# mees/hulc2

Measured on AMD Instinct MI355X. Metric: play-sequences/sec/node (seq_len=32, 200x200 RGB), higher is better.
Workload: dtype bf16; 1 GPU; BASELINE configs[1]: synthetic CALVIN-shaped batch, Hulc2.training_step fwd+bwd+allreduce+Adam, static CNN 200x200 + gripper CNN 84x84, lang = random (B,384) embeddings, dropout 0.1, gripper_control on; sequences_per_gpu_step=64, seq_len=32, parallelism=dp1, launch=hipGraph replay (fwd+bwd graph, all-reduce, optimizer graph), frames=fp32 NCHW, already transformed (the reference's dataloader output), gradient_allreduce=none (one rank, no process group), exact_forward_sites=encfc,goal,head,txl

## Files before the change

hulc2_amd/csrc/abi.hip:

```cpp
#include "hulc_abi_internal.h"
#include <stdarg.h>
#include <stdio.h>
#include <string.h>

static thread_local char g_err[512] = "";

int hulc_fail(int code, const char* msg) {
    snprintf(g_err, sizeof(g_err), "%s", msg);
    return code;
}

int hulc_check_launch(const char* where) {
    hipError_t e = hipGetLastError();
    if (e == hipSuccess) return 0;
    snprintf(g_err, sizeof(g_err), "%s: launch failed: %s", where, hipGetErrorString(e));
    return -100;
}

extern "C" const char* hulc_last_error(void) { return g_err; }

static thread_local char g_conv_path[256] = "";

void hulc_conv_path_clear(void) { g_conv_path[0] = 0; }
void hulc_conv_path_set(const char* fmt, ...) {
    va_list ap;
    va_start(ap, fmt);
    vsnprintf(g_conv_path, sizeof(g_conv_path), fmt, ap);
    va_end(ap);
}
void hulc_conv_path_append(const char* suffix) {
    const size_t n = strlen(g_conv_path);
    snprintf(g_conv_path + n, sizeof(g_conv_path) - n, "%s", suffix);
}

extern "C" const char* hulc_conv_last_path(void) { return g_conv_path; }
extern "C" int hulc_abi_version(void) { return 7; }

extern "C" int hulc_stream_create(void** out) {
    if (!out) return hulc_fail(-1, "hulc_stream_create: null pointer");
    hipStream_t s = nullptr;
    if (hipStreamCreateWithFlags(&s, hipStreamNonBlocking) != hipSuccess) { *out = nullptr; return hulc_fail(-100, "hulc_stream_create: hipStreamCreateWithFlags failed"); }
    *out = (void*)s;
    return 0;
}
```

hulc2_amd/csrc/hulc_abi_internal.h:

```cpp
#pragma once
#include <hip/hip_runtime.h>
#include "../../include/hulc2_amd.h"

int hulc_fail(int code, const char* msg);
int hulc_check_launch(const char* where);

void hulc_conv_path_clear(void);
void hulc_conv_path_set(const char* fmt, ...) __attribute__((format(printf, 1, 2)));
void hulc_conv_path_append(const char* suffix);

int hulc_wgrad_taps_takes(const hulc_wgrad_item* d);
long hulc_wgrad_taps_workspace(const hulc_wgrad_item* const* items, int n);
int hulc_wgrad_taps_launch(const hulc_wgrad_item* const* items, int n, void* slabs, hipStream_t s);

int hulc_gemm_tn128_try(const hulc_gemm_desc* d, hipStream_t s);
int hulc_gemm_nt128_try(const hulc_gemm_desc* d, hipStream_t s);
```

hulc2_amd/csrc/hulc_common.h:

```cpp
#pragma once
#include <hip/hip_runtime.h>
#include <stdint.h>

#define HULC_F32 0
#define HULC_BF16 1
#define HULC_F16 2

typedef __bf16 bf16_t;
typedef bf16_t bf16x8_t __attribute__((ext_vector_type(8)));
typedef float f32x16_t __attribute__((ext_vector_type(16)));
typedef float f32x4_t __attribute__((ext_vector_type(4)));
typedef float f32x2_t __attribute__((ext_vector_type(2)));

#define HULC_DEVICE __device__ __forceinline__

HULC_DEVICE float bf16_bits_to_f32(uint16_t b) { return __uint_as_float(((uint32_t)b) << 16); }

typedef bf16_t bf16x2_t __attribute__((ext_vector_type(2)));

HULC_DEVICE uint32_t pack_bf16x2(float lo, float hi) {
    f32x2_t f = {lo, hi};
    union { bf16x2_t b; uint32_t u; } x;
    x.b = __builtin_convertvector(f, bf16x2_t);
    return x.u;
// ... 25 lines not shown
}
HULC_DEVICE void store_elem(void* p, int dtype, long idx, float v) {
    if (dtype == HULC_F32) ((float*)p)[idx] = v;
    else ((uint16_t*)p)[idx] = f32_to_bf16_bits(v);
}

struct Chunk8 {
    float v[8];
};

HULC_DEVICE void chunk_zero(Chunk8& c) {
#pragma unroll
    for (int j = 0; j < 8; ++j) c.v[j] = 0.f;
}

HULC_DEVICE void chunk_keep_if(Chunk8& c, bool keep) {
#pragma unroll
    for (int j = 0; j < 8; ++j) c.v[j] = keep ? c.v[j] : 0.f;
}

HULC_DEVICE void chunk_load_contig(Chunk8& c, const void* base, int dtype, long off) {
    if (dtype == HULC_F32) {
        const float4* p = (const float4*)((const float*)base + off);
        float4 a = p[0], b = p[1];
        c.v[0] = a.x; c.v[1] = a.y; c.v[2] = a.z; c.v[3] = a.w;
        c.v[4] = b.x; c.v[5] = b.y; c.v[6] = b.z; c.v[7] = b.w;
    } else if (dtype == HULC_F16) {
        union { uint4 u; _Float16 h[8]; } r; r.u = *(const uint4*)((const uint16_t*)base + off);
#pragma unroll
        for (int j = 0; j < 8; ++j) c.v[j] = (float)r.h[j];
    } else {
        uint4 r = *(const uint4*)((const uint16_t*)base + off);
        c.v[0] = __uint_as_float(r.x << 16); c.v[1] = __uint_as_float(r.x & 0xffff0000u);
        c.v[2] = __uint_as_float(r.y << 16); c.v[3] = __uint_as_float(r.y & 0xffff0000u);
        c.v[4] = __uint_as_float(r.z << 16); c.v[5] = __uint_as_float(r.z & 0xffff0000u);
        c.v[6] = __uint_as_float(r.w << 16); c.v[7] = __uint_as_float(r.w & 0xffff0000u);
    }
}

HULC_DEVICE void chunk_load_strided(Chunk8& c, const void* base, int dtype, long off, long ld, int nvalid) {
#pragma unroll
    for (int j = 0; j < 8; ++j) c.v[j] = (j < nvalid) ? load_elem(base, dtype, off + (long)j * ld) : 0.f;
}

template <typename CT>
HULC_DEVICE void chunk_store_lds(char* dst, const Chunk8& c);

template <>
HULC_DEVICE void chunk_store_lds<bf16_t>(char* dst, const Chunk8& c) {
    uint4 r;
    r.x = pack_bf16x2(c.v[0], c.v[1]);
    r.y = pack_bf16x2(c.v[2], c.v[3]);
    r.z = pack_bf16x2(c.v[4], c.v[5]);
    r.w = pack_bf16x2(c.v[6], c.v[7]);
    *(uint4*)dst = r;
}
template <>
HULC_DEVICE void chunk_store_lds<float>(char* dst, const Chunk8& c) {
    ((float4*)dst)[0] = make_float4(c.v[0], c.v[1], c.v[2], c.v[3]);
    ((float4*)dst)[1] = make_float4(c.v[4], c.v[5], c.v[6], c.v[7]);
}

#define HULC_ROWB 80

template <typename CT> struct MmaTraits;
template <> struct MmaTraits<bf16_t> {
    static constexpr int KT = 32;
    static constexpr int NCH = 4;
    static constexpr int CHB = 16;
};
template <> struct MmaTraits<float> {
    static constexpr int KT = 16;
    static constexpr int NCH = 2;
    static constexpr int CHB = 32;
};

template <typename CT, int TM, int TN>
HULC_DEVICE void mma_tile(const char* a_rows, const char* b_rows, f32x16_t (&acc)[TM][TN], int lane);

template <int TM, int TN>
HULC_DEVICE void mma_tile_bf16(const char* a_rows, const char* b_rows, f32x16_t (&acc)[TM][TN], int lane) {
    const int r = lane & 31, h = lane >> 5;
#pragma unroll
    for (int ks = 0; ks < 2; ++ks) {
        bf16x8_t a[TM], b[TN];
#pragma unroll
        for (int i = 0; i < TM; ++i) a[i] = *(const bf16x8_t*)(a_rows + (i * 32 + r) * HULC_ROWB + (ks * 2 + h) * 16);
#pragma unroll
        for (int j = 0; j < TN; ++j) b[j] = *(const bf16x8_t*)(b_rows + (j * 32 + r) * HULC_ROWB + (ks * 2 + h) * 16);
#pragma unroll
        for (int i = 0; i < TM; ++i)
#pragma unroll
            for (int j = 0; j < TN; ++j)
                acc[i][j] = __builtin_amdgcn_mfma_f32_32x32x16_bf16(a[i], b[j], acc[i][j], 0, 0, 0);
    }
}

template <int TM, int TN>
HULC_DEVICE void mma_tile_f32(const char* a_rows, const char* b_rows, f32x16_t (&acc)[TM][TN], int lane) {
    const int r = lane & 31, h = lane >> 5;
    float a[TM][8], b[TN][8];
#pragma unroll
    for (int i = 0; i < TM; ++i) {
        const float4* p = (const float4*)(a_rows + (i * 32 + r) * HULC_ROWB + h * 32);
        float4 x = p[0], y = p[1];
        a[i][0] = x.x; a[i][1] = x.y; a[i][2] = x.z; a[i][3] = x.w;
        a[i][4] = y.x; a[i][5] = y.y; a[i][6] = y.z; a[i][7] = y.w;
    }
#pragma unroll
    for (int j = 0; j < TN; ++j) {
        const float4* p = (const float4*)(b_rows + (j * 32 + r) * HULC_ROWB + h * 32);
        float4 x = p[0], y = p[1];
        b[j][0] = x.x; b[j][1] = x.y; b[j][2] = x.z; b[j][3] = x.w;
        b[j][4] = y.x; b[j][5] = y.y; b[j][6] = y.z; b[j][7] = y.w;
    }
#pragma unroll
    for (int e = 0; e < 8; ++e)
#pragma unroll
        for (int i = 0; i < TM; ++i)
#pragma unroll
            for (int j = 0; j < TN; ++j)
                acc[i][j] = __builtin_amdgcn_mfma_f32_32x32x2f32(a[i][e], b[j][e], acc[i][j], 0, 0, 0);
}

template <typename CT, int TM, int TN> struct MmaTile;
template <int TM, int TN> struct MmaTile<bf16_t, TM, TN> {
    static HULC_DEVICE void run(const char* a, const char* b, f32x16_t (&acc)[TM][TN], int lane) {
        mma_tile_bf16<TM, TN>(a, b, acc, lane);
    }
};
template <int TM, int TN> struct MmaTile<float, TM, TN> {
    static HULC_DEVICE void run(const char* a, const char* b, f32x16_t (&acc)[TM][TN], int lane) {
        mma_tile_f32<TM, TN>(a, b, acc, lane);
    }
};

HULC_DEVICE int fast_div(int x, float inv) { return (int)(((float)x + 0.5f) * inv); }

HULC_DEVICE float fast_rcp(int d) { return __builtin_amdgcn_rcpf((float)d); }

HULC_DEVICE int acc_row(int reg, int lane) { return (reg & 3) + 8 * (reg >> 2) + 4 * (lane >> 5); }

HULC_DEVICE float wave_sum(float v) {
#pragma unroll
    for (int o = 32; o > 0; o >>= 1) v += __shfl_xor(v, o, 64);
    return v;
}
HULC_DEVICE float wave_max(float v) {
#pragma unroll
    for (int o = 32; o > 0; o >>= 1) v = fmaxf(v, __shfl_xor(v, o, 64));
    return v;
}

HULC_DEVICE uint64_t hulc_rand64(uint64_t seed, uint64_t idx) {
    uint64_t z = idx * 0x9E3779B97F4A7C15ull + seed;
    z = (z ^ (z >> 30)) * 0xBF58476D1CE4E5B9ull;
    z = (z ^ (z >> 27)) * 0x94D049BB133111EBull;
    return z ^ (z >> 31);
}
HULC_DEVICE uint32_t hulc_rand32(uint64_t seed, uint64_t idx) { return (uint32_t)(hulc_rand64(seed, idx) >> 32); }
HULC_DEVICE float dropout_scale(uint64_t seed, uint64_t idx, float p) {
    const uint32_t thr = (uint32_t)(p * 65536.0f);
    const uint32_t u = (uint32_t)(hulc_rand64(seed, idx >> 2) >> (16 * (uint32_t)(idx & 3))) & 0xffffu;
    return u >= thr ? 1.0f / (1.0f - p) : 0.0f;
}
HULC_DEVICE void dropout_scale4(uint64_t seed, uint64_t idx0, float p, float (&s)[4]) {
    const uint32_t thr = (uint32_t)(p * 65536.0f);
    const float keep = 1.0f / (1.0f - p);
    const uint64_t z = hulc_rand64(seed, idx0 >> 2);
    const uint32_t lo = (uint32_t)z, hi = (uint32_t)(z >> 32);
    s[0] = (lo & 0xffffu) >= thr ? keep : 0.f; s[1] = (lo >> 16) >= thr ? keep : 0.f;
    s[2] = (hi & 0xffffu) >= thr ? keep : 0.f; s[3] = (hi >> 16) >= thr ? keep : 0.f;
}
HULC_DEVICE void dropout_scale_acc16(uint64_t seed, uint64_t base, int hf, float p, float (&s)[16]) {
    if ((base & 3) == 0) {
#pragma unroll
        for (int g = 0; g < 4; ++g) {
            float t[4];
            dropout_scale4(seed, base + 8 * g + 4 * hf, p, t);
            s[4 * g] = t[0]; s[4 * g + 1] = t[1]; s[4 * g + 2] = t[2]; s[4 * g + 3] = t[3];
        }
    } else {
#pragma unroll
        for (int e = 0; e < 16; ++e) s[e] = dropout_scale(seed, base + (e & 3) + 8 * (e >> 2) + 4 * hf, p);
    }
}
HULC_DEVICE float hulc_uniform01(uint64_t seed, uint64_t idx) {
    return (hulc_rand32(seed, idx) >> 8) * (1.0f / 16777216.0f);
}
```

hulc2_amd/csrc/losses.hip:

```cpp
#include "hulc_common.h"
#include "hulc_abi_internal.h"
#include <stdio.h>

namespace {

HULC_DEVICE float softplus_t(float x) { return x > 20.f ? x : log1pf(expf(x)); }
HULC_DEVICE float sigmoid_f(float x) { return 1.f / (1.f + expf(-x)); }

HULC_DEVICE float block_sum(float v, float* sh) {
    const int lane = threadIdx.x & 63, wave = threadIdx.x >> 6, nw = (blockDim.x + 63) >> 6;
    v = wave_sum(v);
    __syncthreads();
    if (lane == 0) sh[wave] = v;
    __syncthreads();
    float t = 0.f;
    for (int w = 0; w < nw; ++w) t += sh[w];
    return t;
}

struct MixP {
    const float* y; long ld;
    const float* act;
    const float* amin; const float* amax;
    int T, A, NM, num_classes;
    float log_scale_min, gripper_alpha;
    int tm_B, nseg;
};

HULC_DEVICE int mix_row(const MixP& p, int seg, int j, int seg_tokens) {
    if (p.tm_B == 0) return seg * seg_tokens + j;
    const int bs = p.tm_B / p.nseg;
    return (j / bs) * p.tm_B + seg * bs + j % bs;
}
HULC_DEVICE int mix_seg_of_row(const MixP& p, int t, int seg_tokens) { return p.tm_B == 0 ? t / seg_tokens : (t % p.tm_B) / (p.tm_B / p.nseg); }

HULC_DEVICE float grp16_max(float v) {
#pragma unroll
    for (int o = 8; o > 0; o >>= 1) v = fmaxf(v, __shfl_xor(v, o, 64));
    return v;
}
HULC_DEVICE float grp16_sum(float v) {
#pragma unroll
    for (int o = 8; o > 0; o >>= 1) v += __shfl_xor(v, o, 64);
    return v;
}
template <bool GRAD>
HULC_DEVICE float mix_nll_lanes(const MixP& p, int t, int d, int i, float gscale, float* dy_row) {
    const float* row = p.y + (long)t * p.ld;
    const int NM = p.NM;
    const bool on = i < NM;
    const int ii = on ? i : 0;
    const float a = p.act[(long)t * (p.A + 1) + d];
    const float lo = p.amin[d], hi = p.amax[d];
    const float half = (hi - lo) * 0.5f / (float)(p.num_classes - 1);
    const float logc = logf((float)(p.num_classes - 1) * 0.5f);
    const float logit = row[d * NM + ii];
    const float lmax = grp16_max(on ? logit : -INFINITY);
    const float llse = lmax + logf(grp16_sum(on ? expf(logit - lmax) : 0.f));
    const float mu = row[p.A * NM + d * NM + ii];
    const float raw = row[2 * p.A * NM + d * NM + ii];
    const float ls = fmaxf(raw, p.log_scale_min);
    const float inv = expf(-ls), c = a - mu;
    const float plus = inv * (c + half), minn = inv * (c - half), mid = inv * c;
    float v, gmu, gls;
    if (a < lo + 1e-3f) {
        v = plus - softplus_t(plus);
        const float k = 1.f - sigmoid_f(plus);
        gmu = -inv * k; gls = -plus * k;
    } else if (a > hi - 1e-3f) {
        v = -softplus_t(minn);
        const float k = -sigmoid_f(minn);
        gmu = -inv * k; gls = -minn * k;
    } else {
        const float sp = sigmoid_f(plus), sm = sigmoid_f(minn), delta = sp - sm;
        if (delta > 1e-5f) {
            v = logf(fmaxf(delta, 1e-12f));
            const float dp = sp * (1.f - sp), dm = sm * (1.f - sm);
            gmu = (-inv * dp + inv * dm) / delta;
            gls = (-plus * dp + minn * dm) / delta;
        } else {
            v = mid - ls - 2.f * softplus_t(mid) - logc;
            const float k = 1.f - 2.f * sigmoid_f(mid);
            gmu = -inv * k; gls = -mid * k - 1.f;
        }
    }
    if (raw < p.log_scale_min) gls = 0.f;
    const float lp = v + (logit - llse);
    const float m = grp16_max(on ? lp : -INFINITY);
    const float lse = m + logf(grp16_sum(on ? expf(lp - m) : 0.f));
    if (GRAD && on) {
        const float w = expf(lp - lse), pi = expf(logit - llse);
        dy_row[d * NM + i] = -gscale * (w - pi);
        dy_row[p.A * NM + d * NM + i] = -gscale * w * gmu;
        dy_row[2 * p.A * NM + d * NM + i] = -gscale * w * gls;
    }
    return -lse;
}

__global__ __launch_bounds__(256) void mix_loss_partial_kernel(MixP p, int seg_tokens, int blocks_per_seg, float* __restrict__ partial) {
    __shared__ float sh[16];
    const int seg = blockIdx.x / blocks_per_seg, bl = blockIdx.x % blocks_per_seg;
    const int w = bl * 16 + (threadIdx.x >> 4), i = threadIdx.x & 15;
    float nll = 0.f, ce = 0.f;
    if (w < seg_tokens * (p.A + 1)) {
        const int t = mix_row(p, seg, w / (p.A + 1), seg_tokens), d = w % (p.A + 1);
        if (d < p.A) {
            const float v = mix_nll_lanes<false>(p, t, d, i, 0.f, nullptr);
            nll = i == 0 ? v : 0.f;
        } else if (i == 0) {
            const float* g = p.y + (long)t * p.ld + 3 * p.A * p.NM;
            const float a = p.act[(long)t * (p.A + 1) + p.A];
            const int lbl = (a == -1.f) ? 0 : (int)a;
            const float mx = fmaxf(g[0], g[1]);
            ce = mx + logf(expf(g[0] - mx) + expf(g[1] - mx)) - g[lbl];
        }
    }
    nll = block_sum(nll, sh);
    ce = block_sum(ce, sh);
    if (threadIdx.x == 0) { partial[2 * blockIdx.x] = nll; partial[2 * blockIdx.x + 1] = ce; }
}

__global__ __launch_bounds__(64) void mix_loss_final_kernel(const float* __restrict__ partial, int blocks_per_seg, int seg_tokens,
                                                            float gripper_alpha, float* __restrict__ out) {
    const int seg = blockIdx.x;
    float nll = 0.f, ce = 0.f;
    for (int b = threadIdx.x; b < blocks_per_seg; b += 64) { nll += partial[2 * (seg * blocks_per_seg + b)]; ce += partial[2 * (seg * blocks_per_seg + b) + 1]; }
    nll = wave_sum(nll); ce = wave_sum(ce);
    if (threadIdx.x != 0) return;
    nll /= seg_tokens; ce /= seg_tokens;
    out[seg] = nll + gripper_alpha * ce; out[gridDim.x + seg] = nll; out[2 * gridDim.x + seg] = ce;
}

__global__ __launch_bounds__(256) void mix_loss_bwd_kernel(MixP p, int seg_tokens, const float* __restrict__ gout, float* __restrict__ dy, long ld_dy) {
    const int w = blockIdx.x * 16 + (threadIdx.x >> 4), i = threadIdx.x & 15;
    if (w >= p.T * (p.A + 1)) return;
    const int t = w / (p.A + 1), d = w % (p.A + 1);
    const float g = gout[mix_seg_of_row(p, t, seg_tokens)] / seg_tokens;
    float* drow = dy + (long)t * ld_dy;
    if (d < p.A) mix_nll_lanes<true>(p, t, d, i, g, drow);
    else if (i == 0) {
        for (int c = 3 * p.A * p.NM + 2; c < ld_dy; ++c) drow[c] = 0.f;
        const float* gl = p.y + (long)t * p.ld + 3 * p.A * p.NM;
        const float a = p.act[(long)t * (p.A + 1) + p.A];
        const int lbl = (a == -1.f) ? 0 : (int)a;
        const float mx = fmaxf(gl[0], gl[1]);
        const float e0 = expf(gl[0] - mx), e1 = expf(gl[1] - mx), inv = 1.f / (e0 + e1);
        drow[3 * p.A * p.NM + 0] = g * p.gripper_alpha * (e0 * inv - (lbl == 0 ? 1.f : 0.f));
        drow[3 * p.A * p.NM + 1] = g * p.gripper_alpha * (e1 * inv - (lbl == 1 ? 1.f : 0.f));
    }
}

HULC_DEVICE float sub32_sum(float v) {
#pragma unroll
    for (int o = 16; o > 0; o >>= 1) v += __shfl_xor(v, o, 64);
    return v;
}
HULC_DEVICE float sub32_max(float v) {
#pragma unroll
    for (int o = 16; o > 0; o >>= 1) v = fmaxf(v, __shfl_xor(v, o, 64));
    return v;
}

__global__ __launch_bounds__(256) void cat_kl_group_kernel(const float* __restrict__ pp, const float* __restrict__ pr, int NG,
                                                           float* __restrict__ kl_group) {
    const int lane = threadIdx.x & 31;
    const int g = blockIdx.x * (blockDim.x >> 5) + (threadIdx.x >> 5);
    if (g >= NG) return;
    const float a = pr[(long)g * 32 + lane], b = pp[(long)g * 32 + lane];
    const float ma = sub32_max(a), mb = sub32_max(b);
    const float lp = a - (ma + logf(sub32_sum(expf(a - ma))));
    const float lq = b - (mb + logf(sub32_sum(expf(b - mb))));
    const float kl = sub32_sum(expf(lp) * (lp - lq));
    if (lane == 0) kl_group[g] = kl;
}
__global__ __launch_bounds__(1024) void cat_kl_sum_kernel(const float* __restrict__ kl_group, int NG_seg, int B_seg, float beta,
                                                          const float* __restrict__ beta_dev, float* __restrict__ out) {
    __shared__ float sh[16];
    if (beta_dev) beta = *beta_dev;
    const float* kg = kl_group + (long)blockIdx.x * NG_seg;
    float acc = 0.f;
    for (int g = threadIdx.x; g < NG_seg; g += blockDim.x) acc += kg[g];
    acc = block_sum(acc, sh);
    if (threadIdx.x == 0) out[blockIdx.x] = beta * acc / B_seg;
}

__global__ __launch_bounds__(256) void cat_kl_bwd_kernel(const float* __restrict__ pp, const float* __restrict__ pr,
                                                         const float* __restrict__ kl_group, int B, int G, float beta,
                                                         const float* __restrict__ beta_dev, float mix, const float* __restrict__ gout,
                                                         int nseg, float* __restrict__ dpp, float* __restrict__ dpr) {
    const int lane = threadIdx.x & 31;
    const int g = blockIdx.x * (blockDim.x >> 5) + (threadIdx.x >> 5);
    if (g >= B * G) return;
    if (beta_dev) beta = *beta_dev;
    const int Bs = B / nseg;
    gout += (g / G) / Bs;
    B = Bs;
    const float a = pr[(long)g * 32 + lane], b = pp[(long)g * 32 + lane];
    const float ma = sub32_max(a), mb = sub32_max(b);
    const float lp = a - (ma + logf(sub32_sum(expf(a - ma))));
    const float lq = b - (mb + logf(sub32_sum(expf(b - mb))));
    const float p = expf(lp), q = expf(lq);
    const float s = gout[0] * beta / B;
    dpp[(long)g * 32 + lane] = s * mix * (q - p);
    dpr[(long)g * 32 + lane] = s * (1.f - mix) * p * (lp - lq - kl_group[g]);
}

__global__ __launch_bounds__(256) void plan_sample_kernel(const float* __restrict__ logits, const long* __restrict__ idx_in,
                                                          unsigned long long seed, const unsigned long long* __restrict__ seed_dev, int NG,
                                                          long* __restrict__ idx_out, float* __restrict__ plan) {
    const int lane = threadIdx.x & 31;
    if (seed_dev) seed ^= seed_dev[0];
    const int g = blockIdx.x * (blockDim.x >> 5) + (threadIdx.x >> 5);
    if (g >= NG) return;
    int idx;
    if (idx_in) idx = (int)idx_in[g];
    else {
        const float a = logits[(long)g * 32 + lane];
        const float e = expf(a - sub32_max(a));
        float c = e;
#pragma unroll
        for (int o = 1; o < 32; o <<= 1) { const float n = __shfl_up(c, o, 32); if (lane >= o) c += n; }
        const float total = __shfl(c, 31, 32);
        const float u = hulc_uniform01(seed, (uint64_t)g) * total;
        const unsigned long long ball = __ballot(c > u);
        const unsigned int mine = (unsigned int)(ball >> (threadIdx.x & 32));
        idx = mine ? __ffs((int)mine) - 1 : 31;
    }
    if (lane == 0 && idx_out) idx_out[g] = idx;
    plan[(long)g * 32 + lane] = lane == idx ? 1.f : 0.f;
}

__global__ __launch_bounds__(256) void plan_sample_bwd_kernel(const float* __restrict__ logits, const float* __restrict__ dplan, int NG,
                                                              float* __restrict__ dlogits, int accumulate) {
    const int lane = threadIdx.x & 31;
    const int g = blockIdx.x * (blockDim.x >> 5) + (threadIdx.x >> 5);
    if (g >= NG) return;
    const float a = logits[(long)g * 32 + lane];
    const float e = expf(a - sub32_max(a));
    const float p = e / sub32_sum(e);
    const float gd = dplan[(long)g * 32 + lane];
    const float dot = sub32_sum(p * gd);
    const float v = p * (gd - dot);
    const long i = (long)g * 32 + lane;
    dlogits[i] = accumulate ? dlogits[i] + v : v;
}

HULC_DEVICE float softplus_grad(float r) { return r > 20.f ? 1.f : sigmoid_f(r); }
HULC_DEVICE void gauss_pair(uint64_t seed, uint64_t pair, float& z0, float& z1) {
    const float u1 = hulc_uniform01(seed, 2 * pair), u2 = hulc_uniform01(seed, 2 * pair + 1);
    const float rad = sqrtf(-2.f * logf(1.f - u1));
    float sn, cs;
    sincospif(2.f * u2, &sn, &cs);
    z0 = rad * cs; z1 = rad * sn;
}

__global__ __launch_bounds__(128) void gauss_plan_row_kernel(const float* __restrict__ pp, const float* __restrict__ pr,
                                                             const float* __restrict__ eps_in, unsigned long long seed,
                                                             const unsigned long long* __restrict__ seed_dev, int P, float min_std,
                                                             float* __restrict__ plan, float* __restrict__ eps_out, float* __restrict__ kl_row) {
    __shared__ float sh[16];
    const int b = blockIdx.x, NP = (P + 1) >> 1;
    if (seed_dev) seed ^= seed_dev[0];
    const float* q = pr + (long)b * 2 * P;
    const float* p = kl_row ? pp + (long)b * 2 * P : nullptr;
    const bool sample = plan || eps_out;
    float acc = 0.f;
    for (int k = threadIdx.x; k < NP; k += blockDim.x) {
        float z[2] = {0.f, 0.f};
        if (sample && !eps_in) gauss_pair(seed, (uint64_t)b * NP + k, z[0], z[1]);
#pragma unroll
        for (int e = 0; e < 2; ++e) {
            const int j = 2 * k + e;
            if (j >= P) break;
            const float mq = q[j], sq = softplus_t(q[P + j]) + min_std;
            if (sample) {
                const float eps = eps_in ? eps_in[(long)b * P + j] : z[e];
                if (plan) plan[(long)b * P + j] = mq + sq * eps;
                if (eps_out) eps_out[(long)b * P + j] = eps;
            }
            if (kl_row) {
                const float mp = p[j], sp = softplus_t(p[P + j]) + min_std;
                const float ratio = sq / sp, t = (mq - mp) / sp, r2 = ratio * ratio;
                acc += 0.5f * (r2 + t * t - 1.f - logf(r2));
            }
        }
    }
    if (kl_row) {
        acc = block_sum(acc, sh);
        if (threadIdx.x == 0) kl_row[b] = acc;
    }
}

__global__ __launch_bounds__(256) void gauss_plan_bwd_kernel(const float* __restrict__ pp, const float* __restrict__ pr,
                                                             const float* __restrict__ eps_in, unsigned long long seed,
                                                             const unsigned long long* __restrict__ seed_dev, int B, int P, float min_std,
                                                             float beta, const float* __restrict__ beta_dev, float mix, int nseg,
                                                             const float* __restrict__ dplan, const float* __restrict__ gout,
                                                             float* __restrict__ dpp, float* __restrict__ dpr) {
    const int NP = (P + 1) >> 1;
    const long i = (long)blockIdx.x * blockDim.x + threadIdx.x;
    if (i >= (long)B * NP) return;
    if (beta_dev) beta = *beta_dev;
    const int b = (int)(i / NP), k = (int)(i % NP);
    if (seed_dev) seed ^= seed_dev[0];
    float z[2] = {0.f, 0.f};
    if (dplan && !eps_in) gauss_pair(seed, (uint64_t)i, z[0], z[1]);
    const int Bs = B / nseg;
    const float s = gout ? gout[b / Bs] * beta / Bs : 0.f;
    const long row = (long)b * 2 * P;
#pragma unroll
    for (int e = 0; e < 2; ++e) {
        const int j = 2 * k + e;
        if (j >= P) break;
        const float rq = pr[row + P + j], gq = softplus_grad(rq);
        float dm = 0.f, dr = 0.f;
        if (gout) {
            const float mq = pr[row + j], sq = softplus_t(rq) + min_std;
            const float mp = pp[row + j], rp = pp[row + P + j], sp = softplus_t(rp) + min_std;
            const float ratio = sq / sp, t = (mq - mp) / sp, r2 = ratio * ratio;
            dm = s * (1.f - mix) * t / sp;
            dr = s * (1.f - mix) * (r2 - 1.f) / sq * gq;
            dpp[row + j] = -s * mix * t / sp;
            dpp[row + P + j] = s * mix * (1.f - r2 - t * t) / sp * softplus_grad(rp);
        }
        if (dplan) {
            const float g = dplan[(long)b * P + j];
            const float eps = eps_in ? eps_in[(long)b * P + j] : z[e];
            dm += g;
            dr += g * eps * gq;
        }
        dpr[row + j] = dm;
        dpr[row + P + j] = dr;
    }
}

#define CLIP_MAXM 128
#define CLIP_D 32
template <bool GRAD>
__global__ __launch_bounds__(256) void clip_loss_kernel(const float* __restrict__ im, const float* __restrict__ tx,
                                                        const unsigned char* __restrict__ use, int row0, const float* __restrict__ logit_scale, int M,
                                                        float* __restrict__ out, const float* __restrict__ gout, float* __restrict__ dim_,
                                                        float* __restrict__ dtx, float* __restrict__ dscale) {
    constexpr int DP = CLIP_D + 1;
    const int LP = M + 1;
    extern __shared__ __attribute__((aligned(16))) float sm[];
    float* n = sm;
    float* t = n + M * DP;
    float* L = t + M * DP;
    float* ni = L + M * LP;
    float* ti = ni + M;
    float* rl = ti + M;
    float* cl = rl + M;
    float* uf = cl + M;
    float* dn = uf + M;
    float* dt = dn + M * DP;
    __shared__ float sh[16];
    const int tid = threadIdx.x;
    const float s = expf(logit_scale[0]);
    if (GRAD) for (int i = tid; i < row0 * CLIP_D; i += blockDim.x) { dim_[i] = 0.f; dtx[i] = 0.f; }
    im += (long)row0 * CLIP_D; tx += (long)row0 * CLIP_D;
    if (GRAD) { dim_ += (long)row0 * CLIP_D; dtx += (long)row0 * CLIP_D; }
    for (int i = tid; i < M * CLIP_D; i += blockDim.x) { const int r = i / CLIP_D, d = i % CLIP_D; n[r * DP + d] = im[i]; t[r * DP + d] = tx[i]; }
    for (int r = tid; r < M; r += blockDim.x) uf[r] = use[r] ? 1.f : 0.f;
    __syncthreads();
    for (int r = tid; r < M; r += blockDim.x) {
        float a = 0.f, b = 0.f;
        for (int d = 0; d < CLIP_D; ++d) { a += n[r * DP + d] * n[r * DP + d]; b += t[r * DP + d] * t[r * DP + d]; }
        ni[r] = sqrtf(a); ti[r] = sqrtf(b);
    }
    __syncthreads();
    for (int i = tid; i < M * CLIP_D; i += blockDim.x) { const int r = i / CLIP_D, q = r * DP + i % CLIP_D; n[q] = n[q] / ni[r]; t[q] = t[q] / ti[r]; }
    __syncthreads();
    for (int i = tid; i < M * M; i += blockDim.x) {
        const int r = i / M, c = i % M;
        float a = 0.f;
        for (int d = 0; d < CLIP_D; ++d) a += n[r * DP + d] * t[c * DP + d];
        L[r * LP + c] = s * a;
    }
    __syncthreads();
    float cnt = 0.f;
    for (int r = 0; r < M; ++r) cnt += uf[r];
    for (int q = tid; q < 2 * M; q += blockDim.x) {
        const bool col = q >= M;
        const int r = col ? q - M : q;
        float m1 = -INFINITY;
        for (int c = 0; c < M; ++c) if (uf[c] != 0.f) m1 = fmaxf(m1, col ? L[c * LP + r] : L[r * LP + c]);
        float s1 = 0.f;
        for (int c = 0; c < M; ++c) if (uf[c] != 0.f) s1 += expf((col ? L[c * LP + r] : L[r * LP + c]) - m1);
        (col ? cl : rl)[r] = m1 + logf(s1);
    }
    __syncthreads();
    if (!GRAD) {
        float acc = 0.f;
        for (int r = tid; r < M; r += blockDim.x) if (uf[r] != 0.f) acc += (rl[r] - L[r * LP + r]) + (cl[r] - L[r * LP + r]);
        acc = block_sum(acc, sh);
        if (tid == 0) {
            out[0] = cnt > 0.f ? acc / (2.f * cnt) : 0.f;
            out[1] = cnt > 0.f ? cnt : 1.f;
        }
        return;
    }
    const float g = cnt > 0.f ? gout[0] / (2.f * cnt) : 0.f;
    float ds = 0.f;
    for (int i = tid; i < M * M; i += blockDim.x) {
        const int r = i / M, c = i % M;
        float dl = 0.f;
        if (uf[r] != 0.f && uf[c] != 0.f) {
            const float lv = L[r * LP + c];
            dl = g * (expf(lv - rl[r]) + expf(lv - cl[c]) - (r == c ? 2.f : 0.f));
            ds += dl * lv;
        }
        L[r * LP + c] = dl;
    }
    ds = block_sum(ds, sh);
    if (tid == 0) dscale[0] = ds;
    for (int i = tid; i < M * CLIP_D; i += blockDim.x) {
        const int r = i / CLIP_D, d = i % CLIP_D;
        float a = 0.f, b = 0.f;
        for (int c = 0; c < M; ++c) { a += L[r * LP + c] * t[c * DP + d]; b += L[c * LP + r] * n[c * DP + d]; }
        dn[r * DP + d] = s * a;
        dt[r * DP + d] = s * b;
    }
    __syncthreads();
    for (int i = tid; i < M * CLIP_D; i += blockDim.x) {
        const int r = i / CLIP_D, q = r * DP + i % CLIP_D;
        float pa = 0.f, pb = 0.f;
        for (int d = 0; d < CLIP_D; ++d) { pa += dn[r * DP + d] * n[r * DP + d]; pb += dt[r * DP + d] * t[r * DP + d]; }
        dim_[i] = (dn[q] - n[q] * pa) / ni[r];
        dtx[i] = (dt[q] - t[q] * pb) / ti[r];
    }
}

HULC_DEVICE void euler_xyz(float a, float b, float c, float (&R)[3][3]) {
    const float ca = cosf(a), sa = sinf(a), cb = cosf(b), sb = sinf(b), cc = cosf(c), sc = sinf(c);
    R[0][0] = cb * cc;                R[0][1] = -cb * sc;               R[0][2] = sb;
    R[1][0] = sa * sb * cc + ca * sc; R[1][1] = -sa * sb * sc + ca * cc; R[1][2] = -sa * cb;
    R[2][0] = -ca * sb * cc + sa * sc; R[2][1] = ca * sb * sc + sa * cc; R[2][2] = ca * cb;
}
HULC_DEVICE void world_to_tcp_row(const float* a, const float* o, float* y) {
    float R[3][3], Rn[3][3];
    euler_xyz(o[3], o[4], o[5], R);
    euler_xyz(o[3] + 0.01f * a[3], o[4] + 0.01f * a[4], o[5] + 0.01f * a[5], Rn);
    for (int r = 0; r < 3; ++r) y[r] = R[0][r] * a[0] + R[1][r] * a[1] + R[2][r] * a[2];
    float M[3][3];
    for (int r = 0; r < 3; ++r)
        for (int c = 0; c < 3; ++c) M[r][c] = Rn[0][r] * R[0][c] + Rn[1][r] * R[1][c] + Rn[2][r] * R[2][c];
    float e[3] = {atan2f(-M[1][2], M[2][2]), asinf(fminf(fmaxf(M[0][2], -1.f), 1.f)), atan2f(-M[0][1], M[0][0])};
    const float pi = 3.14159265358979323846f;
    for (int r = 0; r < 3; ++r) {
        if (e[r] < -pi) e[r] += 2 * pi;
        if (e[r] > pi) e[r] -= 2 * pi;
        y[3 + r] = e[r] * 100.f;
    }
    y[6] = a[6];
}
__global__ void world_to_tcp_kernel(const float* __restrict__ act, const float* __restrict__ obs, int n, int obs_dim, float* __restrict__ out) {
    const int i = blockIdx.x * blockDim.x + threadIdx.x;
    if (i >= n) return;
    world_to_tcp_row(act + (long)i * 7, obs + (long)i * obs_dim, out + (long)i * 7);
}
struct ActSegP { const float* act[4]; const float* obs[4]; };
__global__ void actions_time_major_kernel(ActSegP p, int nseg, int B, int S, int obs_dim, int to_tcp, float* __restrict__ out) {
    const int i = blockIdx.x * blockDim.x + threadIdx.x;
    if (i >= nseg * B * S) return;
    const int st = i / (nseg * B), rem = i % (nseg * B), seg = rem / B, b = rem % B;
    const float* a = p.act[seg] + ((long)b * S + st) * 7;
    float* y = out + (long)i * 7;
    if (to_tcp) world_to_tcp_row(a, p.obs[seg] + ((long)b * S + st) * obs_dim, y);
    else for (int r = 0; r < 7; ++r) y[r] = a[r];
}

__global__ void tcp_to_world_kernel(const float* __restrict__ act, const float* __restrict__ obs, int n, int obs_dim, float* __restrict__ out) {
    const int i = blockIdx.x * blockDim.x + threadIdx.x;
    if (i >= n) return;
    const float* a = act + (long)i * 7;
    const float* o = obs + (long)i * obs_dim;
    float R[3][3], Q[3][3];
    euler_xyz(o[3], o[4], o[5], R);
    euler_xyz(0.01f * a[3], 0.01f * a[4], 0.01f * a[5], Q);
    float* y = out + (long)i * 7;
    for (int r = 0; r < 3; ++r) y[r] = R[r][0] * a[0] + R[r][1] * a[1] + R[r][2] * a[2];
    float M[3][3];
    for (int r = 0; r < 3; ++r)
        for (int c = 0; c < 3; ++c) M[r][c] = R[r][0] * Q[c][0] + R[r][1] * Q[c][1] + R[r][2] * Q[c][2];
    float e[3] = {atan2f(-M[1][2], M[2][2]), asinf(fminf(fmaxf(M[0][2], -1.f), 1.f)), atan2f(-M[0][1], M[0][0])};
    const float pi = 3.14159265358979323846f;
    for (int r = 0; r < 3; ++r) {
        float d = e[r] - o[3 + r];
        if (d < -pi) d += 2 * pi;
        if (d > pi) d -= 2 * pi;
        y[3 + r] = d * 100.f;
    }
    y[6] = a[6];
}

__global__ __launch_bounds__(256) void mix_sample_kernel(MixP p, const float* __restrict__ u_mix, const float* __restrict__ u_inv,
                                                         unsigned long long seed, const unsigned long long* __restrict__ seed_dev,
                                                         const float* __restrict__ gripper_bounds, float* __restrict__ act_out,
                                                         long* __restrict__ idx_out) {
    const long i = (long)blockIdx.x * blockDim.x + threadIdx.x;
    if (i >= (long)p.T * (p.A + 1)) return;
    if (seed_dev) seed ^= seed_dev[0];
    const int t = (int)(i / (p.A + 1)), a = (int)(i % (p.A + 1));
    const float* row = p.y + (long)t * p.ld;
    const int n = p.A * p.NM;
    if (a == p.A) {
        const int g = row[3 * n + 1] > row[3 * n] ? 1 : 0;
        act_out[(long)t * (p.A + 1) + p.A] = gripper_bounds[g];
        return;
    }
    const float c = (float)(1e-5 - (1.0 - 1e-5)), r2 = (float)(1.0 - 1e-5);
    int best = 0; float best_v = -INFINITY;
    for (int k = 0; k < p.NM; ++k) {
        const float raw = u_mix ? u_mix[((long)t * p.A + a) * p.NM + k] : hulc_uniform01(seed, (uint64_t)(((long)t * p.A + a) * p.NM + k));
        const float u = __fadd_rn(__fmul_rn(c, raw), r2);
        const float v = row[a * p.NM + k] - logf(-logf(u));
        if (v > best_v) { best_v = v; best = k; }
    }
    const float mean = row[n + a * p.NM + best];
    const float ls = fmaxf(row[2 * n + a * p.NM + best], p.log_scale_min);
    const float raw = u_inv ? u_inv[(long)t * p.A + a] : hulc_uniform01(seed ^ 0x9E3779B97F4A7C15ull, (uint64_t)((long)t * p.A + a));
    const float u = __fadd_rn(__fmul_rn(c, raw), r2);
    act_out[(long)t * (p.A + 1) + a] = mean + expf(ls) * (logf(u) - logf(1.0f - u));
    if (idx_out) idx_out[(long)t * p.A + a] = best;
}

MixP make_mix(const hulc_mix_desc* d, const float* y, const float* act) {
    MixP p;
    p.y = y; p.ld = d->ld; p.act = act; p.amin = d->act_min; p.amax = d->act_max;
    p.T = d->T; p.A = d->A; p.NM = d->n_mix; p.num_classes = d->num_classes;
    p.log_scale_min = d->log_scale_min; p.gripper_alpha = d->gripper_alpha;
    p.tm_B = d->time_major_B; p.nseg = d->nseg < 1 ? 1 : d->nseg;
    return p;
}

}

static int mix_check(const hulc_mix_desc* d, const char* who) {
    if (d->n_mix > 16 || d->n_mix <= 0) return hulc_fail(-2, "hulc_mix_loss: n_mix must be in 1..16");
    if (d->nseg < 1 || d->T % d->nseg != 0) return hulc_fail(-3, "hulc_mix_loss: T must split into nseg equal segments");
    if (d->time_major_B < 0 || (d->time_major_B > 0 && (d->T % d->time_major_B || d->time_major_B % d->nseg)))
        return hulc_fail(-3, "hulc_mix_loss: time-major rows need T % B == 0 and B % nseg == 0");
    (void)who;
    return 0;
}
extern "C" long hulc_mix_loss_workspace(const hulc_mix_desc* d) {
    if (!d || d->nseg < 1) return -1;
    const int items = (d->T / d->nseg) * (d->A + 1);
    return (long)d->nseg * ((items + 15) / 16) * 2 * (long)sizeof(float);
}
extern "C" int hulc_mix_loss_fwd(const hulc_mix_desc* d, const float* y, const float* act, float* out, void* ws, void* stream) {
    if (!d || !y || !act || !out || !ws || !d->act_min || !d->act_max) return hulc_fail(-1, "hulc_mix_loss_fwd: null pointer");
    int rc = mix_check(d, "fwd"); if (rc) return rc;
    const int seg_tokens = d->T / d->nseg, bps = (seg_tokens * (d->A + 1) + 15) / 16;
    hipStream_t s = (hipStream_t)stream;
    mix_loss_partial_kernel<<<d->nseg * bps, 256, 0, s>>>(make_mix(d, y, act), seg_tokens, bps, (float*)ws);
    mix_loss_final_kernel<<<d->nseg, 64, 0, s>>>((const float*)ws, bps, seg_tokens, d->gripper_alpha, out);
    return hulc_check_launch("hulc_mix_loss_fwd");
}
extern "C" int hulc_mix_loss_bwd(const hulc_mix_desc* d, const float* y, const float* act, const float* gout, float* dy, long ld_dy,
                                 void* stream) {
    if (!d || !y || !act || !gout || !dy) return hulc_fail(-1, "hulc_mix_loss_bwd: null pointer");
    int rc = mix_check(d, "bwd"); if (rc) return rc;
    const int n = d->T * (d->A + 1);
    mix_loss_bwd_kernel<<<(n + 15) / 16, 256, 0, (hipStream_t)stream>>>(make_mix(d, y, act), d->T / d->nseg, gout, dy, ld_dy);
    return hulc_check_launch("hulc_mix_loss_bwd");
}

static int fail_named(int code, const char* name, const char* what) {
    char msg[256];
    snprintf(msg, sizeof(msg), "%s: %s", name, what);
    return hulc_fail(code, msg);
}
static int beta_dev_check(const float* beta_dev, const char* null_msg, const char* align_msg) {
    if (!beta_dev) return hulc_fail(-1, null_msg);
    if ((uintptr_t)beta_dev % 4) return hulc_fail(-4, align_msg);
    return 0;
}
static int cat_kl_fwd_impl(const char* name, const float* pp, const float* pr, int B, int G, int CLS, float beta, const float* beta_dev, int nseg,
                           float* out, float* kl_group, void* stream) {
    if (!pp || !pr || !out || !kl_group) return fail_named(-1, name, "null pointer");
    if (CLS != 32) return fail_named(-2, name, "class_size must be 32 (one 32-lane sub-wave per category)");
    if (nseg < 1 || B % nseg) return fail_named(-2, name, "the batch must split evenly into nseg segments");
    cat_kl_group_kernel<<<(B * G + 7) / 8, 256, 0, (hipStream_t)stream>>>(pp, pr, B * G, kl_group);
    cat_kl_sum_kernel<<<nseg, 1024, 0, (hipStream_t)stream>>>(kl_group, B / nseg * G, B / nseg, beta, beta_dev, out);
    return hulc_check_launch(name);
}
static int cat_kl_bwd_impl(const char* name, const float* pp, const float* pr, const float* kl_group, int B, int G, int CLS, float beta,
                           const float* beta_dev, float mix, const float* gout, int nseg, float* dpp, float* dpr, void* stream) {
    if (!pp || !pr || !kl_group || !gout || !dpp || !dpr) return fail_named(-1, name, "null pointer");
    if (CLS != 32) return fail_named(-2, name, "class_size must be 32");
    if (nseg < 1 || B % nseg) return fail_named(-2, name, "the batch must split evenly into nseg segments");
    cat_kl_bwd_kernel<<<(B * G + 7) / 8, 256, 0, (hipStream_t)stream>>>(pp, pr, kl_group, B, G, beta, beta_dev, mix, gout, nseg, dpp, dpr);
    return hulc_check_launch(name);
}
extern "C" int hulc_cat_kl_fwd(const float* pp, const float* pr, int B, int G, int CLS, float beta, int nseg, float* out, float* kl_group, void* stream) {
    return cat_kl_fwd_impl("hulc_cat_kl_fwd", pp, pr, B, G, CLS, beta, nullptr, nseg, out, kl_group, stream);
}
extern "C" int hulc_cat_kl_bwd(const float* pp, const float* pr, const float* kl_group, int B, int G, int CLS, float beta, float mix,
                               const float* gout, int nseg, float* dpp, float* dpr, void* stream) {
    return cat_kl_bwd_impl("hulc_cat_kl_bwd", pp, pr, kl_group, B, G, CLS, beta, nullptr, mix, gout, nseg, dpp, dpr, stream);
}
extern "C" int hulc_cat_kl_fwd_sched(const float* pp, const float* pr, int B, int G, int CLS, float beta, int nseg, float* out, float* kl_group,
                                     const float* beta_dev, void* stream) {
    int rc = beta_dev_check(beta_dev, "hulc_cat_kl_fwd_sched: null beta_dev", "hulc_cat_kl_fwd_sched: beta_dev must be 4-byte aligned");
    if (rc) return rc;
    return cat_kl_fwd_impl("hulc_cat_kl_fwd_sched", pp, pr, B, G, CLS, beta, beta_dev, nseg, out, kl_group, stream);
}
extern "C" int hulc_cat_kl_bwd_sched(const float* pp, const float* pr, const float* kl_group, int B, int G, int CLS, float beta, float mix,
                                     const float* gout, int nseg, float* dpp, float* dpr, const float* beta_dev, void* stream) {
    int rc = beta_dev_check(beta_dev, "hulc_cat_kl_bwd_sched: null beta_dev", "hulc_cat_kl_bwd_sched: beta_dev must be 4-byte aligned");
    if (rc) return rc;
    return cat_kl_bwd_impl("hulc_cat_kl_bwd_sched", pp, pr, kl_group, B, G, CLS, beta, beta_dev, mix, gout, nseg, dpp, dpr, stream);
}
extern "C" int hulc_plan_sample_fwd(const float* logits, const long* idx_in, unsigned long long seed, const unsigned long long* seed_dev,
                                    int NG, int CLS, long* idx_out, float* plan, void* stream) {
    if (!logits || !plan) return hulc_fail(-1, "hulc_plan_sample_fwd: null pointer");
    if (CLS != 32) return hulc_fail(-2, "hulc_plan_sample_fwd: class_size must be 32");
    plan_sample_kernel<<<(NG + 7) / 8, 256, 0, (hipStream_t)stream>>>(logits, idx_in, seed, seed_dev, NG, idx_out, plan);
    return hulc_check_launch("hulc_plan_sample_fwd");
}
extern "C" int hulc_plan_sample_bwd(const float* logits, const float* dplan, int NG, int CLS, float* dlogits, int accumulate, void* stream) {
    if (!logits || !dplan || !dlogits) return hulc_fail(-1, "hulc_plan_sample_bwd: null pointer");
    if (CLS != 32) return hulc_fail(-2, "hulc_plan_sample_bwd: class_size must be 32");
    plan_sample_bwd_kernel<<<(NG + 7) / 8, 256, 0, (hipStream_t)stream>>>(logits, dplan, NG, dlogits, accumulate);
    return hulc_check_launch("hulc_plan_sample_bwd");
}

static int gauss_plan_fwd_impl(const char* name, const float* pp, const float* pr, const float* eps_in, unsigned long long seed,
                               const unsigned long long* seed_dev, int B, int P, float min_std, float beta, const float* beta_dev, int nseg,
                               float* plan, float* eps_out, float* out, float* kl_row, void* stream) {
    if (!plan && !eps_out && !out) return fail_named(-1, name, "nothing to compute (plan, eps_out and out are all null)");
    if (!pr || (out && (!pp || !kl_row))) return fail_named(-1, name, "null pointer");
    if (B < 1 || P < 1) return fail_named(-2, name, "needs B >= 1 and plan_features >= 1");
    if (out && (nseg < 1 || B % nseg)) return fail_named(-2, name, "the batch must split evenly into nseg segments");
    gauss_plan_row_kernel<<<B, 128, 0, (hipStream_t)stream>>>(pp, pr, eps_in, seed, seed_dev, P, min_std, plan, eps_out, out ? kl_row : nullptr);
    if (out) cat_kl_sum_kernel<<<nseg, 1024, 0, (hipStream_t)stream>>>(kl_row, B / nseg, B / nseg, beta, beta_dev, out);
    return hulc_check_launch(name);
}
static int gauss_plan_bwd_impl(const char* name, const float* pp, const float* pr, const float* eps_in, unsigned long long seed,
                               const unsigned long long* seed_dev, int B, int P, float min_std, float beta, const float* beta_dev, float mix,
                               int nseg, const float* dplan, const float* gout, float* dpp, float* dpr, void* stream) {
    if (!dplan && !gout) return fail_named(-1, name, "nothing to compute (dplan and gout are both null)");
    if (!pr || !dpr || (gout && (!pp || !dpp))) return fail_named(-1, name, "null pointer");
    if (B < 1 || P < 1) return fail_named(-2, name, "needs B >= 1 and plan_features >= 1");
    if (gout && (nseg < 1 || B % nseg)) return fail_named(-2, name, "the batch must split evenly into nseg segments");
    const long n = (long)B * ((P + 1) / 2);
    gauss_plan_bwd_kernel<<<(unsigned)((n + 255) / 256), 256, 0, (hipStream_t)stream>>>(pp, pr, eps_in, seed, seed_dev, B, P, min_std, beta,
                                                                                        gout ? beta_dev : nullptr, mix, gout ? nseg : 1, dplan,
                                                                                        gout, dpp, dpr);
    return hulc_check_launch(name);
}
extern "C" int hulc_gauss_plan_fwd(const float* pp, const float* pr, const float* eps_in, unsigned long long seed,
                                   const unsigned long long* seed_dev, int B, int P, float min_std, float beta, int nseg, float* plan,
                                   float* eps_out, float* out, float* kl_row, void* stream) {
    return gauss_plan_fwd_impl("hulc_gauss_plan_fwd", pp, pr, eps_in, seed, seed_dev, B, P, min_std, beta, nullptr, nseg, plan, eps_out, out,
                               kl_row, stream);
}
extern "C" int hulc_gauss_plan_bwd(const float* pp, const float* pr, const float* eps_in, unsigned long long seed,
                                   const unsigned long long* seed_dev, int B, int P, float min_std, float beta, float mix, int nseg,
                                   const float* dplan, const float* gout, float* dpp, float* dpr, void* stream) {
    return gauss_plan_bwd_impl("hulc_gauss_plan_bwd", pp, pr, eps_in, seed, seed_dev, B, P, min_std, beta, nullptr, mix, nseg, dplan, gout, dpp,
                               dpr, stream);
}
extern "C" int hulc_gauss_plan_fwd_sched(const float* pp, const float* pr, const float* eps_in, unsigned long long seed,
                                         const unsigned long long* seed_dev, int B, int P, float min_std, float beta, int nseg, float* plan,
                                         float* eps_out, float* out, float* kl_row, const float* beta_dev, void* stream) {
    if (out) {
        int rc = beta_dev_check(beta_dev, "hulc_gauss_plan_fwd_sched: null beta_dev", "hulc_gauss_plan_fwd_sched: beta_dev must be 4-byte aligned");
        if (rc) return rc;
    }
    return gauss_plan_fwd_impl("hulc_gauss_plan_fwd_sched", pp, pr, eps_in, seed, seed_dev, B, P, min_std, beta, out ? beta_dev : nullptr, nseg,
                               plan, eps_out, out, kl_row, stream);
}
extern "C" int hulc_gauss_plan_bwd_sched(const float* pp, const float* pr, const float* eps_in, unsigned long long seed,
                                         const unsigned long long* seed_dev, int B, int P, float min_std, float beta, float mix, int nseg,
                                         const float* dplan, const float* gout, float* dpp, float* dpr, const float* beta_dev, void* stream) {
    if (gout) {
        int rc = beta_dev_check(beta_dev, "hulc_gauss_plan_bwd_sched: null beta_dev", "hulc_gauss_plan_bwd_sched: beta_dev must be 4-byte aligned");
        if (rc) return rc;
    }
    return gauss_plan_bwd_impl("hulc_gauss_plan_bwd_sched", pp, pr, eps_in, seed, seed_dev, B, P, min_std, beta, beta_dev, mix, nseg, dplan, gout,
                               dpp, dpr, stream);
}

static size_t clip_smem(int M) { return ((size_t)4 * M * (CLIP_D + 1) + (size_t)M * (M + 1) + 5 * (size_t)M) * sizeof(float); }
template <bool G> static int clip_lds_ok() {
    static int rc = hipFuncSetAttribute((const void*)clip_loss_kernel<G>, hipFuncAttributeMaxDynamicSharedMemorySize, (int)clip_smem(CLIP_MAXM)) == hipSuccess ? 0 : -8;
    return rc;
}

extern "C" int hulc_clip_loss_fwd(const float* im, const float* tx, const unsigned char* use, int row0, const float* logit_scale, int M, int D,
                                  float* out, void* stream) {
    if (!im || !tx || !use || !logit_scale || !out) return hulc_fail(-1, "hulc_clip_loss_fwd: null pointer");
    if (M > CLIP_MAXM || M <= 0 || D != CLIP_D || row0 < 0 || row0 >= M) return hulc_fail(-2, "hulc_clip_loss_fwd: needs M <= 128, D == 32, 0 <= row0 < M");
    if (clip_lds_ok<false>()) return hulc_fail(-8, "hulc_clip_loss_fwd: could not raise the dynamic LDS limit");
    clip_loss_kernel<false><<<1, 256, clip_smem(M - row0), (hipStream_t)stream>>>(im, tx, use, row0, logit_scale, M - row0, out, nullptr, nullptr, nullptr, nullptr);
    return hulc_check_launch("hulc_clip_loss_fwd");
}
extern "C" int hulc_clip_loss_bwd(const float* im, const float* tx, const unsigned char* use, int row0, const float* logit_scale, int M, int D,
                                  const float* gout, float* dim, float* dtx, float* dscale, void* stream) {
    if (!im || !tx || !use || !logit_scale || !gout || !dim || !dtx || !dscale) return hulc_fail(-1, "hulc_clip_loss_bwd: null pointer");
    if (M > CLIP_MAXM || M <= 0 || D != CLIP_D || row0 < 0 || row0 >= M) return hulc_fail(-2, "hulc_clip_loss_bwd: needs M <= 128, D == 32, 0 <= row0 < M");
    if (clip_lds_ok<true>()) return hulc_fail(-8, "hulc_clip_loss_bwd: could not raise the dynamic LDS limit");
    clip_loss_kernel<true><<<1, 256, clip_smem(M - row0), (hipStream_t)stream>>>(im, tx, use, row0, logit_scale, M - row0, nullptr, gout, dim, dtx, dscale);
    return hulc_check_launch("hulc_clip_loss_bwd");
}

__global__ void loss_combine_fwd_kernel(const float* __restrict__ kls, const float* __restrict__ acts, const float* __restrict__ clip, int n, float beta,
                                        float* __restrict__ out) {
    if (threadIdx.x != 0 || blockIdx.x != 0) return;
    float sk = 0.f, sa = 0.f, st = 0.f;
    for (int m = 0; m < n; ++m) { const float t = acts[m] + kls[m]; out[4 + m] = t; sk += kls[m]; sa += acts[m]; st += t; }
    float total = st / n;
    const float wc = clip ? beta * clip[0] : 0.f;
    if (clip) total = total + wc;
    out[0] = total; out[1] = sk / n; out[2] = sa / n; out[3] = wc;
}
__global__ void loss_combine_bwd_kernel(const float* __restrict__ g, int n, float beta, float* __restrict__ dkls, float* __restrict__ dacts,
                                        float* __restrict__ dclip) {
    const int m = threadIdx.x;
    if (m < n) { dkls[m] = g[0] / n; dacts[m] = g[0] / n; }
    if (m == 0 && dclip) dclip[0] = g[0] * beta;
}
extern "C" int hulc_loss_combine_fwd(const float* kls, const float* acts, const float* clip, int n, float beta, float* out, void* stream) {
    if (!kls || !acts || !out) return hulc_fail(-1, "hulc_loss_combine_fwd: null pointer");
    if (n < 1 || n > 64) return hulc_fail(-2, "hulc_loss_combine_fwd: 1..64 modalities");
    loss_combine_fwd_kernel<<<1, 64, 0, (hipStream_t)stream>>>(kls, acts, clip, n, beta, out);
    return hulc_check_launch("hulc_loss_combine_fwd");
}
extern "C" int hulc_loss_combine_bwd(const float* g, int n, float beta, float* dkls, float* dacts, float* dclip, void* stream) {
    if (!g || !dkls || !dacts) return hulc_fail(-1, "hulc_loss_combine_bwd: null pointer");
    if (n < 1 || n > 64) return hulc_fail(-2, "hulc_loss_combine_bwd: 1..64 modalities");
    loss_combine_bwd_kernel<<<1, 64, 0, (hipStream_t)stream>>>(g, n, beta, dkls, dacts, dclip);
    return hulc_check_launch("hulc_loss_combine_bwd");
}

extern "C" int hulc_actions_time_major(const float* const* act, const float* const* robot_obs, int nseg, int B, int S, int obs_dim, int to_tcp,
                                       float* out, void* stream) {
    if (!act || !out || (to_tcp && !robot_obs)) return hulc_fail(-1, "hulc_actions_time_major: null pointer");
    if (nseg < 1 || nseg > 4 || B < 1 || S < 1 || (to_tcp && obs_dim < 6)) return hulc_fail(-2, "hulc_actions_time_major: 1..4 segments, robot_obs with the euler angles in columns 3:6");
    ActSegP p{};
    for (int i = 0; i < nseg; ++i) {
        if (!act[i] || (to_tcp && !robot_obs[i])) return hulc_fail(-1, "hulc_actions_time_major: null segment pointer");
        p.act[i] = act[i];
        p.obs[i] = to_tcp ? robot_obs[i] : nullptr;
    }
    const int n = nseg * B * S;
    actions_time_major_kernel<<<(n + 255) / 256, 256, 0, (hipStream_t)stream>>>(p, nseg, B, S, obs_dim, to_tcp, out);
    return hulc_check_launch("hulc_actions_time_major");
}

extern "C" int hulc_world_to_tcp(const float* act, const float* robot_obs, int n, int obs_dim, float* out, void* stream) {
    if (!act || !robot_obs || !out) return hulc_fail(-1, "hulc_world_to_tcp: null pointer");
    if (obs_dim < 6) return hulc_fail(-2, "hulc_world_to_tcp: robot_obs needs the euler angles in columns 3:6");
    world_to_tcp_kernel<<<(n + 255) / 256, 256, 0, (hipStream_t)stream>>>(act, robot_obs, n, obs_dim, out);
    return hulc_check_launch("hulc_world_to_tcp");
}

extern "C" int hulc_tcp_to_world(const float* act, const float* robot_obs, int n, int obs_dim, float* out, void* stream) {
    if (!act || !robot_obs || !out) return hulc_fail(-1, "hulc_tcp_to_world: null pointer");
    if (obs_dim < 6) return hulc_fail(-2, "hulc_tcp_to_world: robot_obs needs the euler angles in columns 3:6");
    tcp_to_world_kernel<<<(n + 255) / 256, 256, 0, (hipStream_t)stream>>>(act, robot_obs, n, obs_dim, out);
    return hulc_check_launch("hulc_tcp_to_world");
}

extern "C" int hulc_mix_sample(const hulc_mix_desc* d, const float* y, const float* u_mix, const float* u_inv, unsigned long long seed,
                               const unsigned long long* seed_dev, const float* gripper_bounds, float* act_out, long* idx_out, void* stream) {
    if (!d || !y || !gripper_bounds || !act_out) return hulc_fail(-1, "hulc_mix_sample: null pointer");
    if (d->T <= 0 || d->A <= 0 || d->n_mix <= 0 || d->ld < 3L * d->A * d->n_mix + 2) return hulc_fail(-2, "hulc_mix_sample: bad geometry");
    MixP p = make_mix(d, y, nullptr);
    const long n = (long)d->T * (d->A + 1);
    mix_sample_kernel<<<(unsigned)((n + 255) / 256), 256, 0, (hipStream_t)stream>>>(p, u_mix, u_inv, seed, seed_dev, gripper_bounds, act_out, idx_out);
    return hulc_check_launch("hulc_mix_sample");
}
```

hulc2_amd/csrc/pointwise.hip:

```cpp
#include "hulc_common.h"
#include "hulc_abi_internal.h"
#include <stdlib.h>

namespace {

__global__ __launch_bounds__(256) void spatial_softmax_fwd_kernel(const void* __restrict__ x, int x_dtype, int N, int HW, int C,
                                                                  const float* __restrict__ xmap, const float* __restrict__ ymap,
                                                                  const float* __restrict__ temperature, float* __restrict__ out,
                                                                  float* __restrict__ stats) {
    __shared__ float red[4][4][64];
    const int lane = threadIdx.x & 63, wave = threadIdx.x >> 6;
    const int n = blockIdx.x;
    const bool act = lane < C;
    const float invT = 1.0f / temperature[0];
    const long base = (long)n * HW * C + lane;
    const int per = (HW + 3) / 4, p0 = wave * per, p1 = p0 + per < HW ? p0 + per : HW;
    float m = -INFINITY;
    if (act)
        for (int p = p0; p < p1; ++p) m = fmaxf(m, load_elem(x, x_dtype, base + (long)p * C) * invT);
    red[wave][0][lane] = m;
    __syncthreads();
    m = fmaxf(fmaxf(red[0][0][lane], red[1][0][lane]), fmaxf(red[2][0][lane], red[3][0][lane]));
    float s = 0.f, sx = 0.f, sy = 0.f;
    if (act)
// ... 44 lines not shown
    const float c1 = a.m == -INFINITY ? 0.f : __expf(a.m - mn), c2 = m2 == -INFINITY ? 0.f : __expf(m2 - mn);
    a.s = a.s * c1 + s2 * c2; a.sx = a.sx * c1 + sx2 * c2; a.sy = a.sy * c1 + sy2 * c2; a.m = mn;
}
__global__ __launch_bounds__(256) void spatial_softmax_fwd64_kernel(const void* __restrict__ x, int x_dtype, int HW,
                                                                    const float* __restrict__ xmap, const float* __restrict__ ymap,
                                                                    const float* __restrict__ temperature, float* __restrict__ out,
                                                                    float* __restrict__ stats) {
    __shared__ float red[4][4][64];
    const int lane = threadIdx.x & 63, wave = threadIdx.x >> 6;
    const int cg = lane & 7, pl = lane >> 3;
    const int n = blockIdx.x;
    const float invT = 1.0f / temperature[0];
    const long base = (long)n * HW * 64 + cg * 8;
    SsmAcc a[8];
#pragma unroll
    for (int j = 0; j < 8; ++j) { a[j].m = -INFINITY; a[j].s = 0.f; a[j].sx = 0.f; a[j].sy = 0.f; }
    for (int p = wave * 8 + pl; p < HW; p += 32) {
        Chunk8 c; chunk_load_contig(c, x, x_dtype, base + (long)p * 64);
        const float xm = xmap[p], ym = ymap[p];
#pragma unroll
        for (int j = 0; j < 8; ++j) {
            const float v = c.v[j] * invT;
            const float mn = fmaxf(a[j].m, v);
            const float sc = __expf(a[j].m - mn), e = __expf(v - mn);
            a[j].s = a[j].s * sc + e; a[j].sx = a[j].sx * sc + e * xm; a[j].sy = a[j].sy * sc + e * ym; a[j].m = mn;
        }
    }
#pragma unroll
    for (int j = 0; j < 8; ++j) {
#pragma unroll
        for (int o = 8; o < 64; o <<= 1)
            ssm_merge(a[j], __shfl_xor(a[j].m, o, 64), __shfl_xor(a[j].s, o, 64), __shfl_xor(a[j].sx, o, 64), __shfl_xor(a[j].sy, o, 64));
        if (pl == 0) { red[wave][0][cg * 8 + j] = a[j].m; red[wave][1][cg * 8 + j] = a[j].s; red[wave][2][cg * 8 + j] = a[j].sx; red[wave][3][cg * 8 + j] = a[j].sy; }
    }
    __syncthreads();
    if (wave == 0) {
        SsmAcc t; t.m = red[0][0][lane]; t.s = red[0][1][lane]; t.sx = red[0][2][lane]; t.sy = red[0][3][lane];
#pragma unroll
        for (int w = 1; w < 4; ++w) ssm_merge(t, red[w][0][lane], red[w][1][lane], red[w][2][lane], red[w][3][lane]);
        const float inv = 1.0f / t.s;
        out[(long)n * 128 + 2 * lane] = t.sx * inv;
        out[(long)n * 128 + 2 * lane + 1] = t.sy * inv;
        stats[((long)n * 64 + lane) * 2] = t.m;
        stats[((long)n * 64 + lane) * 2 + 1] = t.s;
    }
}
template <int DT>
__global__ __launch_bounds__(256) void spatial_softmax_fwd64_regs_kernel(const void* __restrict__ x, int HW, const float* __restrict__ xmap,
                                                                         const float* __restrict__ ymap, const float* __restrict__ temperature,
                                                                         float* __restrict__ out, float* __restrict__ stats) {
    constexpr int IT = 14;
    __shared__ float red[4][4][64];
    const int lane = threadIdx.x & 63, wave = threadIdx.x >> 6;
    const int cg = lane & 7, pl = lane >> 3;
    const int n = blockIdx.x;
    const float invT = 1.0f / temperature[0];
    const long base = (long)n * HW * 64 + cg * 8;
    float v[IT][8];
#pragma unroll
    for (int k = 0; k < IT; ++k) {
        const int p = wave * 8 + pl + 32 * k;
        const bool on = p < HW;
        const long off = base + (long)(on ? p : 0) * 64;
        float c[8];
        if (DT == HULC_BF16) {
            const uint4 r = *(const uint4*)((const uint16_t*)x + off);
            const uint32_t w[4] = {r.x, r.y, r.z, r.w};
#pragma unroll
            for (int j = 0; j < 4; ++j) { c[2 * j] = __uint_as_float(w[j] << 16); c[2 * j + 1] = __uint_as_float(w[j] & 0xffff0000u); }
        } else if (DT == HULC_F16) {
            union { uint4 u; _Float16 hh[8]; } r; r.u = *(const uint4*)((const uint16_t*)x + off);
#pragma unroll
            for (int j = 0; j < 8; ++j) c[j] = (float)r.hh[j];
        } else {
            const float4* q = (const float4*)((const float*)x + off);
            const float4 a0 = q[0], a1 = q[1];
            c[0] = a0.x; c[1] = a0.y; c[2] = a0.z; c[3] = a0.w; c[4] = a1.x; c[5] = a1.y; c[6] = a1.z; c[7] = a1.w;
        }
#pragma unroll
        for (int j = 0; j < 8; ++j) v[k][j] = on ? c[j] * invT : -INFINITY;
    }
    SsmAcc a[8];
#pragma unroll
    for (int j = 0; j < 8; ++j) {
        float m = v[0][j];
#pragma unroll
        for (int k = 1; k < IT; ++k) m = fmaxf(m, v[k][j]);
        a[j].m = m; a[j].s = 0.f; a[j].sx = 0.f; a[j].sy = 0.f;
    }
#pragma unroll
    for (int k = 0; k < IT; ++k) {
        const int p = wave * 8 + pl + 32 * k;
        const int pc = p < HW ? p : 0;
        const float xm = xmap[pc], ym = ymap[pc];
#pragma unroll
        for (int j = 0; j < 8; ++j) {
            const float e = __expf(v[k][j] - a[j].m);
            a[j].s += e; a[j].sx += e * xm; a[j].sy += e * ym;
        }
    }
#pragma unroll
    for (int j = 0; j < 8; ++j) {
#pragma unroll
        for (int o = 8; o < 64; o <<= 1)
            ssm_merge(a[j], __shfl_xor(a[j].m, o, 64), __shfl_xor(a[j].s, o, 64), __shfl_xor(a[j].sx, o, 64), __shfl_xor(a[j].sy, o, 64));
        if (pl == 0) { red[wave][0][cg * 8 + j] = a[j].m; red[wave][1][cg * 8 + j] = a[j].s; red[wave][2][cg * 8 + j] = a[j].sx; red[wave][3][cg * 8 + j] = a[j].sy; }
    }
    __syncthreads();
    if (wave == 0) {
        SsmAcc t; t.m = red[0][0][lane]; t.s = red[0][1][lane]; t.sx = red[0][2][lane]; t.sy = red[0][3][lane];
#pragma unroll
        for (int w = 1; w < 4; ++w) ssm_merge(t, red[w][0][lane], red[w][1][lane], red[w][2][lane], red[w][3][lane]);
        const float inv = 1.0f / t.s;
        out[(long)n * 128 + 2 * lane] = t.sx * inv;
        out[(long)n * 128 + 2 * lane + 1] = t.sy * inv;
        stats[((long)n * 64 + lane) * 2] = t.m;
        stats[((long)n * 64 + lane) * 2 + 1] = t.s;
    }
}
__global__ __launch_bounds__(256) void spatial_softmax_bwd64_kernel(const void* __restrict__ x, int x_dtype, int HW,
                                                                    const float* __restrict__ xmap, const float* __restrict__ ymap,
                                                                    const float* __restrict__ temperature, const float* __restrict__ out,
                                                                    const float* __restrict__ stats, const float* __restrict__ dout,
                                                                    void* __restrict__ dx, int dx_dtype, int relu_mask) {
    const int lane = threadIdx.x & 63, wave = threadIdx.x >> 6;
    const int cg = lane & 7, pl = lane >> 3;
    const int n = blockIdx.x;
    const float invT = 1.0f / temperature[0];
    const long base = (long)n * HW * 64 + cg * 8;
    float m[8], k[8], ex[8], ey[8], gx[8], gy[8];
#pragma unroll
    for (int j = 0; j < 8; ++j) {
        const int c = cg * 8 + j;
        m[j] = stats[((long)n * 64 + c) * 2]; k[j] = invT / stats[((long)n * 64 + c) * 2 + 1];
        ex[j] = out[(long)n * 128 + 2 * c]; ey[j] = out[(long)n * 128 + 2 * c + 1];
        gx[j] = dout[(long)n * 128 + 2 * c]; gy[j] = dout[(long)n * 128 + 2 * c + 1];
    }
    for (int p = wave * 8 + pl; p < HW; p += 32) {
        Chunk8 c; chunk_load_contig(c, x, x_dtype, base + (long)p * 64);
        const float xm = xmap[p], ym = ymap[p];
        float g[8];
#pragma unroll
        for (int j = 0; j < 8; ++j) {
            g[j] = k[j] * __expf(c.v[j] * invT - m[j]) * (gx[j] * (xm - ex[j]) + gy[j] * (ym - ey[j]));
            if (relu_mask && !(c.v[j] > 0.f)) g[j] = 0.f;
        }
        const long o = base + (long)p * 64;
        if (dx_dtype == HULC_BF16) *(uint4*)((uint16_t*)dx + o) = make_uint4(pack_bf16x2(g[0], g[1]), pack_bf16x2(g[2], g[3]), pack_bf16x2(g[4], g[5]), pack_bf16x2(g[6], g[7]));
        else { ((float4*)((float*)dx + o))[0] = make_float4(g[0], g[1], g[2], g[3]); ((float4*)((float*)dx + o))[1] = make_float4(g[4], g[5], g[6], g[7]); }
    }
}


__global__ __launch_bounds__(256) void layernorm_fwd_kernel(const float* __restrict__ x, const float* __restrict__ o, float drop_p,
                                                            unsigned long long seed, const unsigned long long* __restrict__ seed_dev,
                                                            const float* __restrict__ gamma,
                                                            const float* __restrict__ beta, float eps, int R, int D,
                                                            float* __restrict__ pre_out, float* __restrict__ y,
                                                            float* __restrict__ mean_out, float* __restrict__ rstd_out,
                                                            int n_o = 1, long o_stride = 0, long ld_y = 0) {
    const int lane = threadIdx.x & 63;
    const int r = blockIdx.x * 4 + (threadIdx.x >> 6);
    if (r >= R) return;
    if (seed_dev) seed ^= seed_dev[0];
    float v[4];
    float s = 0.f;
#pragma unroll
    for (int q = 0; q < 4; ++q) {
        const int c = lane + q * 64;
        v[q] = 0.f;
        if (c < D) {
            const long i = (long)r * D + c;
            float t = x[i];
            if (o) {
                float ov = o[i];
                {
                    int sl = 1;
                    for (; sl + 3 < n_o; sl += 4) {
                        const float a0 = o[(long)sl * o_stride + i], a1 = o[(long)(sl + 1) * o_stride + i], a2 = o[(long)(sl + 2) * o_stride + i],
                                    a3 = o[(long)(sl + 3) * o_stride + i];
                        ov += a0; ov += a1; ov += a2; ov += a3;
                    }
                    for (; sl < n_o; ++sl) ov += o[(long)sl * o_stride + i];
                }
                if (drop_p > 0.f) ov *= dropout_scale(seed, (uint64_t)i, drop_p);
                t += ov;
            }
            v[q] = t;
            if (pre_out) pre_out[i] = t;
            s += t;
        }
    }
    const float mean = wave_sum(s) / D;
    float ss = 0.f;
#pragma unroll
    for (int q = 0; q < 4; ++q) {
        const int c = lane + q * 64;
        if (c < D) { const float dlt = v[q] - mean; ss += dlt * dlt; }
    }
    const float rstd = rsqrtf(wave_sum(ss) / D + eps);
#pragma unroll
    for (int q = 0; q < 4; ++q) {
        const int c = lane + q * 64;
        if (c < D) y[(long)r * (ld_y ? ld_y : D) + c] = (v[q] - mean) * rstd * gamma[c] + beta[c];
    }
    if (lane == 0) { mean_out[r] = mean; rstd_out[r] = rstd; }
}

__global__ __launch_bounds__(256) void layernorm_bwd_kernel(const float* __restrict__ dy, const float* __restrict__ pre,
                                                            const float* __restrict__ mean_in, const float* __restrict__ rstd_in,
                                                            const float* __restrict__ gamma, int R, int D, int rows_per_block,
                                                            float* __restrict__ dpre, float* __restrict__ do_out, float drop_p,
                                                            unsigned long long seed, const unsigned long long* __restrict__ seed_dev,
                                                            float* __restrict__ partial, long ld_dy = 0) {
    __shared__ float red[4][2][256];
    if (seed_dev) seed ^= seed_dev[0];
    const int lane = threadIdx.x & 63, wave = threadIdx.x >> 6;
    float dg[4] = {0.f, 0.f, 0.f, 0.f}, db[4] = {0.f, 0.f, 0.f, 0.f};
    const int r0 = blockIdx.x * rows_per_block;
    for (int r = r0 + wave; r < r0 + rows_per_block && r < R; r += 4) {
        const float mean = mean_in[r], rstd = rstd_in[r];
        float g[4], xh[4], s1 = 0.f, s2 = 0.f;
#pragma unroll
        for (int q = 0; q < 4; ++q) {
            const int c = lane + q * 64;
            g[q] = 0.f; xh[q] = 0.f;
            if (c < D) {
                const long i = (long)r * D + c;
                const float d = dy[ld_dy ? (long)r * ld_dy + c : i];
                xh[q] = (pre[i] - mean) * rstd;
                g[q] = d * gamma[c];
                dg[q] += d * xh[q]; db[q] += d;
                s1 += g[q]; s2 += g[q] * xh[q];
            }
        }
        s1 = wave_sum(s1) / D; s2 = wave_sum(s2) / D;
#pragma unroll
        for (int q = 0; q < 4; ++q) {
            const int c = lane + q * 64;
            if (c < D) {
                const long i = (long)r * D + c;
                const float v = rstd * (g[q] - s1 - xh[q] * s2);
                dpre[i] = v;
                if (do_out) do_out[i] = drop_p > 0.f ? v * dropout_scale(seed, (uint64_t)i, drop_p) : v;
            }
        }
    }
#pragma unroll
    for (int q = 0; q < 4; ++q) { red[wave][0][lane + q * 64] = dg[q]; red[wave][1][lane + q * 64] = db[q]; }
    __syncthreads();
    for (int c = threadIdx.x; c < D; c += 256) {
        float a = 0.f, b = 0.f;
        for (int w = 0; w < 4; ++w) { a += red[w][0][c]; b += red[w][1][c]; }
        partial[(long)blockIdx.x * 2 * D + c] = a;
        partial[(long)blockIdx.x * 2 * D + D + c] = b;
    }
}

__device__ inline float4 load4(const void* x, int dt, long off) {
    if (dt == HULC_F32) return *(const float4*)((const float*)x + off);
    const uint2 v = *(const uint2*)((const uint16_t*)x + off);
    return make_float4(__uint_as_float(v.x << 16), __uint_as_float(v.x & 0xffff0000u), __uint_as_float(v.y << 16), __uint_as_float(v.y & 0xffff0000u));
}
__global__ __launch_bounds__(256) void colsum_kernel(const void* __restrict__ x, int x_dtype, long M, int N, long ld, long rows_per_block,
                                                     float* __restrict__ partial, float* __restrict__ direct_out, int accumulate, int vec) {
    __shared__ float4 red[4][64];
    const int lane = threadIdx.x & 63, wave = threadIdx.x >> 6;
    const int n = (blockIdx.x * 64 + lane) * 4;
    const long r0 = (long)blockIdx.y * rows_per_block;
    long r1 = r0 + rows_per_block; if (r1 > M) r1 = M;
    float4 s = make_float4(0.f, 0.f, 0.f, 0.f);
    if (vec) {
        if (n < N) {
            long r = r0 + wave;
            float4 a0 = s, a1 = s, a2 = s, a3 = s;
            for (; r + 12 < r1; r += 16) {
                const float4 v0 = load4(x, x_dtype, r * ld + n), v1 = load4(x, x_dtype, (r + 4) * ld + n);
                const float4 v2 = load4(x, x_dtype, (r + 8) * ld + n), v3 = load4(x, x_dtype, (r + 12) * ld + n);
                a0.x += v0.x; a0.y += v0.y; a0.z += v0.z; a0.w += v0.w;
                a1.x += v1.x; a1.y += v1.y; a1.z += v1.z; a1.w += v1.w;
                a2.x += v2.x; a2.y += v2.y; a2.z += v2.z; a2.w += v2.w;
                a3.x += v3.x; a3.y += v3.y; a3.z += v3.z; a3.w += v3.w;
            }
            for (; r < r1; r += 4) { const float4 v = load4(x, x_dtype, r * ld + n); a0.x += v.x; a0.y += v.y; a0.z += v.z; a0.w += v.w; }
            s.x = (a0.x + a1.x) + (a2.x + a3.x); s.y = (a0.y + a1.y) + (a2.y + a3.y);
            s.z = (a0.z + a1.z) + (a2.z + a3.z); s.w = (a0.w + a1.w) + (a2.w + a3.w);
        }
    } else {
        float* sp = (float*)&s;
        for (int j = 0; j < 4; ++j)
            if (n + j < N)
                for (long r = r0 + wave; r < r1; r += 4) sp[j] += load_elem(x, x_dtype, r * ld + n + j);
    }
    red[wave][lane] = s;
    __syncthreads();
    if (wave == 0) {
        const float4 a = red[0][lane], b = red[1][lane], c = red[2][lane], d = red[3][lane];
        const float v[4] = {(a.x + b.x) + (c.x + d.x), (a.y + b.y) + (c.y + d.y), (a.z + b.z) + (c.z + d.z), (a.w + b.w) + (c.w + d.w)};
        for (int j = 0; j < 4; ++j) {
            if (n + j >= N) break;
            if (direct_out) direct_out[n + j] = accumulate ? direct_out[n + j] + v[j] : v[j];
            else partial[(long)blockIdx.y * N + n + j] = v[j];
        }
    }
}
__global__ __launch_bounds__(1024) void reduce_rows_wide_kernel(const float* __restrict__ partial, float* __restrict__ out, int P, long R, long ld,
                                                                int accumulate, long off1 = 0, float* __restrict__ out1 = nullptr) {
    __shared__ float red[16][64];
    if (blockIdx.y == 1) { partial += off1; out = out1; }
    const int lane = threadIdx.x & 63, sl = threadIdx.x >> 6;
    const long rr = (long)blockIdx.x * 64 + lane;
    const int per = (P + 15) / 16;
    const int q0 = sl * per, q1 = q0 + per < P ? q0 + per : P;
    float s = 0.f;
    if (rr < R)
        for (int q = q0; q < q1; ++q) s += partial[(long)q * ld + rr];
    red[sl][lane] = s;
    __syncthreads();
    if (sl == 0 && rr < R) {
        float t = 0.f;
#pragma unroll
        for (int w = 0; w < 16; ++w) t += red[w][lane];
        out[rr] = accumulate ? out[rr] + t : t;
    }
}

__global__ void seq_mean_fwd_kernel(const float* __restrict__ x, float* __restrict__ y, int B, int S, int D, float scale) {
    const long i = (long)blockIdx.x * blockDim.x + threadIdx.x;
    if (i >= (long)B * D) return;
    const int b = (int)(i / D), d = (int)(i % D);
    float s0 = 0.f, s1 = 0.f, s2 = 0.f, s3 = 0.f;
    const float* xb = x + (long)b * S * D + d;
    int t = 0;
    for (; t + 3 < S; t += 4) {
        const float a = xb[(long)t * D], c = xb[(long)(t + 1) * D], e = xb[(long)(t + 2) * D], f = xb[(long)(t + 3) * D];
        s0 += a; s1 += c; s2 += e; s3 += f;
    }
    for (; t < S; ++t) s0 += xb[(long)t * D];
    const float s = (s0 + s1) + (s2 + s3);
    y[i] = scale * (s / S);
}
__global__ void strided_seq_sum_kernel(const void* __restrict__ x, int x_dtype, float* __restrict__ y, int B, int S, int D, long stride_b,
                                       long stride_s, long ldy, float scale) {
    const long i = (long)blockIdx.x * blockDim.x + threadIdx.x;
    if (i >= (long)B * D) return;
    const int b = (int)(i / D), d = (int)(i % D);
    float s0 = 0.f, s1 = 0.f, s2 = 0.f, s3 = 0.f;
    const long o = (long)b * stride_b + d;
    int t = 0;
    for (; t + 3 < S; t += 4) {
        const float a = load_elem(x, x_dtype, o + (long)t * stride_s), c = load_elem(x, x_dtype, o + (long)(t + 1) * stride_s),
                    e = load_elem(x, x_dtype, o + (long)(t + 2) * stride_s), f = load_elem(x, x_dtype, o + (long)(t + 3) * stride_s);
        s0 += a; s1 += c; s2 += e; s3 += f;
    }
    for (; t < S; ++t) s0 += load_elem(x, x_dtype, o + (long)t * stride_s);
    y[(long)b * ldy + d] = scale * ((s0 + s1) + (s2 + s3));
}

__global__ void seq_mean_bwd_kernel(const float* __restrict__ dy, float* __restrict__ dx, int B, int S, int D) {
    const long i = (long)blockIdx.x * blockDim.x + threadIdx.x;
    if (i >= (long)B * S * D) return;
    const int d = (int)(i % D); const long bs = i / D; const int b = (int)(bs / S);
    dx[i] = dy[(long)b * D + d] / S;
}
__global__ void add_pos_fwd_kernel(const float* __restrict__ x, const float* __restrict__ pos, const long* __restrict__ pos_ids,
                                   float* __restrict__ y, int B, int S, int D, float drop_p, unsigned long long seed,
                                   const unsigned long long* __restrict__ seed_dev) {
    const long i = (long)blockIdx.x * blockDim.x + threadIdx.x;
    if (i >= (long)B * S * D) return;
    if (seed_dev) seed ^= seed_dev[0];
    const int d = (int)(i % D); const int s = (int)((i / D) % S);
    float v = x[i] + pos[pos_ids[s] * D + d];
    if (drop_p > 0.f) v *= dropout_scale(seed, (uint64_t)i, drop_p);
    y[i] = v;
}
__global__ void dropout_bwd_kernel(const float* __restrict__ dy, float* __restrict__ dx, long n, float drop_p, unsigned long long seed,
                                   const unsigned long long* __restrict__ seed_dev) {
    const long i = (long)blockIdx.x * blockDim.x + threadIdx.x;
    if (i >= n) return;
    if (seed_dev) seed ^= seed_dev[0];
    dx[i] = dy[i] * dropout_scale(seed, (uint64_t)i, drop_p);
}

__global__ void relu_bwd_kernel(const float* __restrict__ dy, const void* __restrict__ y, int y_dtype, float* __restrict__ dx, long n, float scale) {
    const long i = (long)blockIdx.x * blockDim.x + threadIdx.x;
    if (i >= n) return;
    dx[i] = load_elem(y, y_dtype, i) > 0.f ? dy[i] * scale : 0.f;
}

#define ATT_DH 16
__global__ __launch_bounds__(64) void attention_fwd_kernel(const float* __restrict__ qkv, float* __restrict__ out, float* __restrict__ probs,
                                                           int B, int S, int H, float scale, float drop_p, unsigned long long seed,
                                                           const unsigned long long* __restrict__ seed_dev) {
    __shared__ float q[32][ATT_DH + 1], k[32][ATT_DH + 1], v[32][ATT_DH + 1];
    if (seed_dev) seed ^= seed_dev[0];
    const int lane = threadIdx.x, b = blockIdx.x / H, h = blockIdx.x % H, E = H * ATT_DH;
    for (int idx = lane; idx < S * ATT_DH; idx += 64) {
        const int s = idx / ATT_DH, d = idx % ATT_DH;
        const long row = ((long)b * S + s) * 3 * E + h * ATT_DH + d;
        q[s][d] = qkv[row]; k[s][d] = qkv[row + E]; v[s][d] = qkv[row + 2 * E];
    }
    __syncthreads();
    const int i = lane & 31, half = lane >> 5;
    float sc[16];
    float m = -INFINITY;
#pragma unroll
    for (int jj = 0; jj < 16; ++jj) {
        const int j = half * 16 + jj;
        float a = -INFINITY;
        if (i < S && j < S) {
            a = 0.f;
#pragma unroll
            for (int d = 0; d < ATT_DH; ++d) a += q[i][d] * k[j][d];
            a *= scale;
        }
        sc[jj] = a; m = fmaxf(m, a);
    }
    m = fmaxf(m, __shfl_xor(m, 32, 64));
    float sum = 0.f;
#pragma unroll
    for (int jj = 0; jj < 16; ++jj) { sc[jj] = (i < S && half * 16 + jj < S) ? __expf(sc[jj] - m) : 0.f; sum += sc[jj]; }
    sum += __shfl_xor(sum, 32, 64);
    const float inv = i < S ? 1.0f / sum : 0.f;
    float o[ATT_DH];
#pragma unroll
    for (int d = 0; d < ATT_DH; ++d) o[d] = 0.f;
    const long pbase = (((long)b * H + h) * S + i) * S;
#pragma unroll
    for (int jj = 0; jj < 16; ++jj) {
        const int j = half * 16 + jj;
        if (i < S && j < S) {
            float p = sc[jj] * inv;
            if (drop_p > 0.f) p *= dropout_scale(seed, (uint64_t)(pbase + j), drop_p);
            probs[pbase + j] = p;
#pragma unroll
            for (int d = 0; d < ATT_DH; ++d) o[d] += p * v[j][d];
        }
    }
#pragma unroll
    for (int d = 0; d < ATT_DH; ++d) o[d] += __shfl_xor(o[d], 32, 64);
    if (i < S) {
        float* dst = out + ((long)b * S + i) * E + h * ATT_DH + half * 8;
#pragma unroll
        for (int d = 0; d < 8; ++d) dst[d] = o[half * 8 + d];
    }
}

__global__ __launch_bounds__(64) void attention_bwd_kernel(const float* __restrict__ qkv, const float* __restrict__ probs,
                                                           const float* __restrict__ dout, float* __restrict__ dqkv, int B, int S, int H,
                                                           float scale, float drop_p, unsigned long long seed,
                                                           const unsigned long long* __restrict__ seed_dev) {
    __shared__ float q[32][ATT_DH + 1], k[32][ATT_DH + 1], v[32][ATT_DH + 1], go[32][ATT_DH + 1];
    if (seed_dev) seed ^= seed_dev[0];
    __shared__ float ds[32][33], pp[32][33];
    const int lane = threadIdx.x, b = blockIdx.x / H, h = blockIdx.x % H, E = H * ATT_DH;
    for (int idx = lane; idx < S * ATT_DH; idx += 64) {
        const int s = idx / ATT_DH, d = idx % ATT_DH;
// ... 13 lines not shown
        dp[jj] = 0.f; pr[jj] = 0.f;
        if (i < S && j < S) {
            const float pd = probs[pbase + j];
            float ks = 1.f;
            if (drop_p > 0.f) ks = dropout_scale(seed, (uint64_t)(pbase + j), drop_p);
            float a = 0.f;
#pragma unroll
            for (int d = 0; d < ATT_DH; ++d) a += go[i][d] * v[j][d];
            const float p = ks > 0.f ? pd / ks : 0.f;
            dp[jj] = a * ks;
            pr[jj] = p;
            dot += dp[jj] * p;
            pp[i][j] = pd;
        }
    }
    dot += __shfl_xor(dot, 32, 64);
    if (drop_p > 0.f) {
        float sc[16], m = -INFINITY, sum = 0.f;
#pragma unroll
        for (int jj = 0; jj < 16; ++jj) {
            const int j = half * 16 + jj;
            float a = -INFINITY;
            if (i < S && j < S) {
                a = 0.f;
#pragma unroll
                for (int d = 0; d < ATT_DH; ++d) a += q[i][d] * k[j][d];
                a *= scale;
            }
            sc[jj] = a; m = fmaxf(m, a);
        }
        m = fmaxf(m, __shfl_xor(m, 32, 64));
#pragma unroll
        for (int jj = 0; jj < 16; ++jj) { sc[jj] = (i < S && half * 16 + jj < S) ? __expf(sc[jj] - m) : 0.f; sum += sc[jj]; }
        sum += __shfl_xor(sum, 32, 64);
        dot = 0.f;
#pragma unroll
        for (int jj = 0; jj < 16; ++jj) { pr[jj] = i < S ? sc[jj] / sum : 0.f; dot += dp[jj] * pr[jj]; }
        dot += __shfl_xor(dot, 32, 64);
    }
    float dq[ATT_DH];
#pragma unroll
    for (int d = 0; d < ATT_DH; ++d) dq[d] = 0.f;
#pragma unroll
    for (int jj = 0; jj < 16; ++jj) {
        const int j = half * 16 + jj;
        if (i < S && j < S) {
            const float dsv = pr[jj] * (dp[jj] - dot) * scale;
            ds[i][j] = dsv;
#pragma unroll
            for (int d = 0; d < ATT_DH; ++d) dq[d] += dsv * k[j][d];
        }
    }
#pragma unroll
    for (int d = 0; d < ATT_DH; ++d) dq[d] += __shfl_xor(dq[d], 32, 64);
    if (i < S) {
        float* dst = dqkv + ((long)b * S + i) * 3 * E + h * ATT_DH + half * 8;
#pragma unroll
        for (int d = 0; d < 8; ++d) dst[d] = dq[half * 8 + d];
    }
    __syncthreads();
    const int j = i;
    if (j < S) {
        float dk[8], dv[8];
#pragma unroll
        for (int d = 0; d < 8; ++d) { dk[d] = 0.f; dv[d] = 0.f; }
        for (int ii = 0; ii < S; ++ii) {
            const float a = ds[ii][j], pv = pp[ii][j];
#pragma unroll
            for (int d = 0; d < 8; ++d) { dk[d] += a * q[ii][half * 8 + d]; dv[d] += pv * go[ii][half * 8 + d]; }
        }
        float* dst = dqkv + ((long)b * S + j) * 3 * E + h * ATT_DH + half * 8;
#pragma unroll
        for (int d = 0; d < 8; ++d) { dst[E + d] = dk[d]; dst[2 * E + d] = dv[d]; }
    }
}

}

extern "C" int hulc_spatial_softmax_fwd(const void* x, int x_dtype, int N, int HW, int C, const float* xmap, const float* ymap,
                                        const float* temperature, float* out, float* stats, void* stream) {
    if (!x || !xmap || !ymap || !temperature || !out || !stats) return hulc_fail(-1, "hulc_spatial_softmax_fwd: null pointer");
    if (C > 64 || C <= 0) return hulc_fail(-2, "hulc_spatial_softmax_fwd: C must be in 1..64 (lane = channel)");
    if (x_dtype == HULC_F16 && (C != 64 || ((uintptr_t)x % 16))) return hulc_fail(-4, "hulc_spatial_softmax_fwd: an fp16 map has 64 channels, 16-byte aligned");
    const int esz = x_dtype == HULC_F32 ? 4 : 2;
    if (C == 64 && ((uintptr_t)x % (8 * esz)) == 0 && HW >= 32 && HW <= 448) {
        if (x_dtype == HULC_BF16) spatial_softmax_fwd64_regs_kernel<HULC_BF16><<<N, 256, 0, (hipStream_t)stream>>>(x, HW, xmap, ymap, temperature, out, stats);
        else if (x_dtype == HULC_F16) spatial_softmax_fwd64_regs_kernel<HULC_F16><<<N, 256, 0, (hipStream_t)stream>>>(x, HW, xmap, ymap, temperature, out, stats);
        else spatial_softmax_fwd64_regs_kernel<HULC_F32><<<N, 256, 0, (hipStream_t)stream>>>(x, HW, xmap, ymap, temperature, out, stats);
    } else if (C == 64 && ((uintptr_t)x % (8 * esz)) == 0)
        spatial_softmax_fwd64_kernel<<<N, 256, 0, (hipStream_t)stream>>>(x, x_dtype, HW, xmap, ymap, temperature, out, stats);
    else
        spatial_softmax_fwd_kernel<<<N, 256, 0, (hipStream_t)stream>>>(x, x_dtype, N, HW, C, xmap, ymap, temperature, out, stats);
    return hulc_check_launch("hulc_spatial_softmax_fwd");
}

extern "C" int hulc_spatial_softmax_bwd(const void* x, int x_dtype, int N, int HW, int C, const float* xmap, const float* ymap,
                                        const float* temperature, const float* out, const float* stats, const float* dout,
                                        void* dx, int dx_dtype, int relu_mask, void* stream) {
    if (!x || !out || !stats || !dout || !dx) return hulc_fail(-1, "hulc_spatial_softmax_bwd: null pointer");
    if (C > 64 || C <= 0) return hulc_fail(-2, "hulc_spatial_softmax_bwd: C must be in 1..64");
    if (x_dtype == HULC_F16 && (C != 64 || ((uintptr_t)x % 16) || ((uintptr_t)dx % (dx_dtype == HULC_F32 ? 32 : 16))))
        return hulc_fail(-4, "hulc_spatial_softmax_bwd: an fp16 map has 64 channels, 16-byte aligned");
    const int esz = x_dtype == HULC_F32 ? 4 : 2, dsz = dx_dtype == HULC_F32 ? 4 : 2;
    if (C == 64 && ((uintptr_t)x % (8 * esz)) == 0 && ((uintptr_t)dx % (8 * dsz)) == 0)
        spatial_softmax_bwd64_kernel<<<N, 256, 0, (hipStream_t)stream>>>(x, x_dtype, HW, xmap, ymap, temperature, out, stats, dout, dx, dx_dtype,
                                                                      relu_mask);
    else
        spatial_softmax_bwd_kernel<<<N, 256, 0, (hipStream_t)stream>>>(x, x_dtype, N, HW, C, xmap, ymap, temperature, out, stats,
                                                                             dout, dx, dx_dtype, relu_mask);
    return hulc_check_launch("hulc_spatial_softmax_bwd");
}

extern "C" int hulc_layernorm_fwd(const float* x, const float* o, float drop_p, unsigned long long seed, const unsigned long long* seed_dev,
                                  const float* gamma, const float* beta, float eps, int R, int D, float* pre_out, float* y, float* mean,
                                  float* rstd, void* stream) {
    if (!x || !gamma || !beta || !y || !mean || !rstd) return hulc_fail(-1, "hulc_layernorm_fwd: null pointer");
    if (D > 256 || D <= 0) return hulc_fail(-2, "hulc_layernorm_fwd: D must be in 1..256");
    if (o && !pre_out) return hulc_fail(-3, "hulc_layernorm_fwd: pre_out required with a residual branch");
    layernorm_fwd_kernel<<<(R + 3) / 4, 256, 0, (hipStream_t)stream>>>(x, o, drop_p, seed, seed_dev, gamma, beta, eps, R, D, pre_out, y, mean, rstd);
    return hulc_check_launch("hulc_layernorm_fwd");
}

extern "C" int hulc_layernorm_slab_fwd(const float* x, const float* o, int n_o, long o_stride, float drop_p, unsigned long long seed,
                                       const unsigned long long* seed_dev, const float* gamma, const float* beta, float eps, int R, int D,
                                       float* pre_out, float* y, float* mean, float* rstd, void* stream) {
    if (!x || !o || !gamma || !beta || !y || !mean || !rstd || !pre_out) return hulc_fail(-1, "hulc_layernorm_slab_fwd: null pointer");
    if (D > 256 || D <= 0 || n_o < 1) return hulc_fail(-2, "hulc_layernorm_slab_fwd: D must be in 1..256, n_o >= 1");
    layernorm_fwd_kernel<<<(R + 3) / 4, 256, 0, (hipStream_t)stream>>>(x, o, drop_p, seed, seed_dev, gamma, beta, eps, R, D, pre_out, y, mean, rstd,
                                                                        n_o, o_stride);
    return hulc_check_launch("hulc_layernorm_slab_fwd");
}

extern "C" int hulc_layernorm_fwd_ld(const float* x, const float* gamma, const float* beta, float eps, int R, int D, float* y, long ld_y,
                                     float* mean, float* rstd, void* stream) {
    if (!x || !gamma || !beta || !y || !mean || !rstd) return hulc_fail(-1, "hulc_layernorm_fwd_ld: null pointer");
    if (D > 256 || D <= 0 || ld_y < D) return hulc_fail(-2, "hulc_layernorm_fwd_ld: D must be in 1..256, ld_y >= D");
    layernorm_fwd_kernel<<<(R + 3) / 4, 256, 0, (hipStream_t)stream>>>(x, nullptr, 0.f, 0ull, nullptr, gamma, beta, eps, R, D, nullptr, y, mean, rstd, 1, 0, ld_y);
    return hulc_check_launch("hulc_layernorm_fwd_ld");
}

static int ln_bwd_rows_per_block(int R) { const int r = (R + 255) / 256; return r < 4 ? 4 : r; }
extern "C" long hulc_layernorm_bwd_workspace(int R, int D) {
    const int rpb = ln_bwd_rows_per_block(R);
    return (long)((R + rpb - 1) / rpb) * 2 * D * (long)sizeof(float);
}

extern "C" int hulc_layernorm_bwd(const float* dy, const float* pre, const float* mean, const float* rstd, const float* gamma, int R,
                                  int D, float* dpre, float* do_out, float drop_p, unsigned long long seed, const unsigned long long* seed_dev,
                                  float* dgamma, float* dbeta, int accumulate_params, void* ws, void* stream) {
    if (!dy || !pre || !mean || !rstd || !gamma || !dpre || !dgamma || !dbeta || !ws) return hulc_fail(-1, "hulc_layernorm_bwd: null pointer");
    if (D > 256 || D <= 0) return hulc_fail(-2, "hulc_layernorm_bwd: D must be in 1..256");
    const int rpb = ln_bwd_rows_per_block(R), nb = (R + rpb - 1) / rpb;
    hipStream_t s = (hipStream_t)stream;
    layernorm_bwd_kernel<<<nb, 256, 0, s>>>(dy, pre, mean, rstd, gamma, R, D, rpb, dpre, do_out, drop_p, seed, seed_dev, (float*)ws);
    reduce_rows_wide_kernel<<<dim3((D + 63) / 64, 2), 1024, 0, s>>>((const float*)ws, dgamma, nb, D, 2 * D, accumulate_params, (long)D, dbeta);
    return hulc_check_launch("hulc_layernorm_bwd");
}

extern "C" int hulc_layernorm_bwd_ld(const float* dy, long ld_dy, const float* pre, const float* mean, const float* rstd, const float* gamma, int R,
                                     int D, float* dpre, float* dgamma, float* dbeta, int accumulate_params, void* ws, void* stream) {
    if (!dy || !pre || !mean || !rstd || !gamma || !dpre || !dgamma || !dbeta || !ws) return hulc_fail(-1, "hulc_layernorm_bwd_ld: null pointer");
    if (D > 256 || D <= 0 || ld_dy < D) return hulc_fail(-2, "hulc_layernorm_bwd_ld: D must be in 1..256, ld_dy >= D");
    const int rpb = ln_bwd_rows_per_block(R), nb = (R + rpb - 1) / rpb;
    hipStream_t s = (hipStream_t)stream;
    layernorm_bwd_kernel<<<nb, 256, 0, s>>>(dy, pre, mean, rstd, gamma, R, D, rpb, dpre, nullptr, 0.f, 0ull, nullptr, (float*)ws, ld_dy);
    reduce_rows_wide_kernel<<<dim3((D + 63) / 64, 2), 1024, 0, s>>>((const float*)ws, dgamma, nb, D, 2 * D, accumulate_params, (long)D, dbeta);
    return hulc_check_launch("hulc_layernorm_bwd_ld");
}

__global__ __launch_bounds__(256) void emb_fanout_fwd_kernel(const float* __restrict__ emb, int N, int S, int D, int n_last, int lo, int hi,
                                                             float* __restrict__ e0, float* __restrict__ elast, float* __restrict__ edec_t) {
    const long i = (long)blockIdx.x * blockDim.x + threadIdx.x;
    const int E = hi - lo;
    const long n_dec = (long)S * N * E, n0 = (long)N * D, nl = (long)n_last * D;
    if (i < n_dec) {
        const int c = (int)(i % E); const long sn = i / E; const int n = (int)(sn % N), st = (int)(sn / N);
        edec_t[i] = emb[((long)n * S + st) * D + lo + c];
    } else if (i < n_dec + n0) {
        const long j = i - n_dec; const int c = (int)(j % D), n = (int)(j / D);
        e0[j] = emb[((long)n * S) * D + c];
    } else if (i < n_dec + n0 + nl) {
        const long j = i - n_dec - n0; const int c = (int)(j % D), n = (int)(j / D);
        elast[j] = emb[((long)n * S + S - 1) * D + c];
    }
}
__global__ __launch_bounds__(256) void emb_fanin_bwd_kernel(const float* __restrict__ g_rec, const float* __restrict__ g0, const float* __restrict__ g_last,
                                                            const float* __restrict__ g_dec_t, int N, int S, int D, int n_last, int lo, int hi,
                                                            float* __restrict__ demb) {
    const long i = (long)blockIdx.x * blockDim.x + threadIdx.x;
    if (i >= (long)N * S * D) return;
    const int c = (int)(i % D); const long ns = i / D; const int st = (int)(ns % S), n = (int)(ns / S);
    float v = g_rec ? g_rec[i] : 0.f;
    if (g0 && st == 0) v += g0[(long)n * D + c];
    if (g_last && st == S - 1 && n < n_last) v += g_last[(long)n * D + c];
    if (g_dec_t && c >= lo && c < hi) v += g_dec_t[((long)st * N + n) * (hi - lo) + c - lo];
    demb[i] = v;
}

extern "C" int hulc_emb_fanout_fwd(const float* emb, int N, int S, int D, int n_last, int lo, int hi, float* e0, float* elast, float* edec_t,
                                   void* stream) {
    if (!emb || !e0 || !edec_t || (n_last > 0 && !elast)) return hulc_fail(-1, "hulc_emb_fanout_fwd: null pointer");
    if (N < 1 || S < 1 || lo < 0 || hi > D || lo >= hi || n_last < 0 || n_last > N) return hulc_fail(-2, "hulc_emb_fanout_fwd: bad geometry");
    const long n = (long)S * N * (hi - lo) + (long)N * D + (long)n_last * D;
    emb_fanout_fwd_kernel<<<(unsigned)((n + 255) / 256), 256, 0, (hipStream_t)stream>>>(emb, N, S, D, n_last, lo, hi, e0, elast, edec_t);
    return hulc_check_launch("hulc_emb_fanout_fwd");
}
extern "C" int hulc_emb_fanin_bwd(const float* g_rec, const float* g0, const float* g_last, const float* g_dec_t, int N, int S, int D, int n_last,
                                  int lo, int hi, float* demb, void* stream) {
    if (!demb) return hulc_fail(-1, "hulc_emb_fanin_bwd: null pointer");
    if (N < 1 || S < 1 || lo < 0 || hi > D || lo >= hi || n_last < 0 || n_last > N) return hulc_fail(-2, "hulc_emb_fanin_bwd: bad geometry");
    const long n = (long)N * S * D;
    emb_fanin_bwd_kernel<<<(unsigned)((n + 255) / 256), 256, 0, (hipStream_t)stream>>>(g_rec, g0, g_last, g_dec_t, N, S, D, n_last, lo, hi, demb);
    return hulc_check_launch("hulc_emb_fanin_bwd");
}

extern "C" int hulc_ln_partial_reduce(const float* partial, int P, int D, float* dgamma, float* dbeta, int accumulate, void* stream) {
    if (!partial || !dgamma || !dbeta) return hulc_fail(-1, "hulc_ln_partial_reduce: null pointer");
    if (P < 1 || D < 1) return hulc_fail(-2, "hulc_ln_partial_reduce: bad geometry");
    reduce_rows_wide_kernel<<<dim3((D + 63) / 64, 2), 1024, 0, (hipStream_t)stream>>>(partial, dgamma, P, D, 2 * D, accumulate, (long)D, dbeta);
    return hulc_check_launch("hulc_ln_partial_reduce");
}

namespace {
struct LnMultiP { float* dg[8]; float* db[8]; int acc[8]; };
__global__ __launch_bounds__(1024) void ln_partial_multi_kernel(const float* __restrict__ partial, int P, int D, LnMultiP t) {
    __shared__ float red[16][64];
    const int which = blockIdx.z;
    const float* src = partial + (long)which * P * 2 * D + (blockIdx.y ? D : 0);
    float* out = blockIdx.y ? t.db[which] : t.dg[which];
    const int lane = threadIdx.x & 63, sl = threadIdx.x >> 6;
    const int rr = blockIdx.x * 64 + lane;
    const int per = (P + 15) / 16;
    const int q0 = sl * per, q1 = q0 + per < P ? q0 + per : P;
    float s = 0.f;
    if (rr < D)
        for (int q = q0; q < q1; ++q) s += src[(long)q * 2 * D + rr];
    red[sl][lane] = s;
    __syncthreads();
    if (sl == 0 && rr < D) {
        float v = 0.f;
#pragma unroll
        for (int w = 0; w < 16; ++w) v += red[w][lane];
        out[rr] = t.acc[which] ? out[rr] + v : v;
    }
}
}

extern "C" int hulc_ln_partial_reduce_multi(const float* partial, int n, int P, int D, float* const* dgamma, float* const* dbeta, const int* accumulate,
                                            void* stream) {
    if (!partial || !dgamma || !dbeta || !accumulate) return hulc_fail(-1, "hulc_ln_partial_reduce_multi: null pointer");
    if (n < 1 || n > 8 || P < 1 || D < 1) return hulc_fail(-2, "hulc_ln_partial_reduce_multi: 1..8 LayerNorms");
    LnMultiP t = {};
    for (int i = 0; i < n; ++i) {
        if (!dgamma[i] || !dbeta[i]) return hulc_fail(-1, "hulc_ln_partial_reduce_multi: null destination");
        t.dg[i] = dgamma[i]; t.db[i] = dbeta[i]; t.acc[i] = accumulate[i];
    }
    ln_partial_multi_kernel<<<dim3((D + 63) / 64, 2, n), 1024, 0, (hipStream_t)stream>>>(partial, P, D, t);
    return hulc_check_launch("hulc_ln_partial_reduce_multi");
}

static long colsum_row_blocks(long M, int N) {
    const long gx = (N + 255) / 256;
    long rb = (1024 + gx - 1) / gx;
    const long cap = (M + 31) / 32;
    if (rb > cap) rb = cap;
    if (rb > 512) rb = 512;
    if (rb < 1) rb = 1;
    return rb;
}
extern "C" long hulc_colsum_workspace(long M, int N) { return colsum_row_blocks(M, N) * N * (long)sizeof(float); }

extern "C" int hulc_colsum(const void* x, int x_dtype, long M, int N, long ld, float* out, int accumulate, void* ws, void* stream) {
    if (!x || !out || !ws) return hulc_fail(-1, "hulc_colsum: null pointer");
    long rb = colsum_row_blocks(M, N);
    const long rpb = (M + rb - 1) / rb;
    rb = (M + rpb - 1) / rpb;
    const int esz = x_dtype == HULC_F32 ? 4 : 2;
    const int vec = (N % 4 == 0) && (ld % 4 == 0) && (((uintptr_t)x) % (4 * esz) == 0);
    hipStream_t s = (hipStream_t)stream;
    dim3 grid((N + 255) / 256, (unsigned)rb);
    colsum_kernel<<<grid, 256, 0, s>>>(x, x_dtype, M, N, ld, rpb, (float*)ws, rb == 1 ? out : nullptr, accumulate, vec);
    if (rb > 1) reduce_rows_wide_kernel<<<(N + 63) / 64, 1024, 0, s>>>((const float*)ws, out, (int)rb, N, N, accumulate);
    return hulc_check_launch("hulc_colsum");
}

extern "C" int hulc_seq_mean_fwd(const float* x, float* y, int B, int S, int D, float scale, void* stream) {
    if (!x || !y) return hulc_fail(-1, "hulc_seq_mean_fwd: null pointer");
    const long n = (long)B * D;
    seq_mean_fwd_kernel<<<(unsigned)((n + 255) / 256), 256, 0, (hipStream_t)stream>>>(x, y, B, S, D, scale);
    return hulc_check_launch("hulc_seq_mean_fwd");
}
extern "C" int hulc_strided_seq_sum(const void* x, int x_dtype, float* y, int B, int S, int D, long stride_b, long stride_s, long ldy,
                                    float scale, void* stream) {
    if (!x || !y) return hulc_fail(-1, "hulc_strided_seq_sum: null pointer");
    const long n = (long)B * D;
    strided_seq_sum_kernel<<<(unsigned)((n + 255) / 256), 256, 0, (hipStream_t)stream>>>(x, x_dtype, y, B, S, D, stride_b, stride_s, ldy, scale);
    return hulc_check_launch("hulc_strided_seq_sum");
}

extern "C" int hulc_seq_mean_bwd(const float* dy, float* dx, int B, int S, int D, void* stream) {
    if (!dy || !dx) return hulc_fail(-1, "hulc_seq_mean_bwd: null pointer");
    const long n = (long)B * S * D;
    seq_mean_bwd_kernel<<<(unsigned)((n + 255) / 256), 256, 0, (hipStream_t)stream>>>(dy, dx, B, S, D);
    return hulc_check_launch("hulc_seq_mean_bwd");
}
extern "C" int hulc_add_pos_fwd(const float* x, const float* pos, const long* pos_ids, float* y, int B, int S, int D, float drop_p,
                                unsigned long long seed, const unsigned long long* seed_dev, void* stream) {
    if (!x || !pos || !pos_ids || !y) return hulc_fail(-1, "hulc_add_pos_fwd: null pointer");
    const long n = (long)B * S * D;
    add_pos_fwd_kernel<<<(unsigned)((n + 255) / 256), 256, 0, (hipStream_t)stream>>>(x, pos, pos_ids, y, B, S, D, drop_p, seed, seed_dev);
    return hulc_check_launch("hulc_add_pos_fwd");
}
extern "C" int hulc_dropout_bwd(const float* dy, float* dx, long n, float drop_p, unsigned long long seed, const unsigned long long* seed_dev,
                                void* stream) {
    if (!dy || !dx) return hulc_fail(-1, "hulc_dropout_bwd: null pointer");
    dropout_bwd_kernel<<<(unsigned)((n + 255) / 256), 256, 0, (hipStream_t)stream>>>(dy, dx, n, drop_p, seed, seed_dev);
    return hulc_check_launch("hulc_dropout_bwd");
}

extern "C" int hulc_relu_bwd(const float* dy, const void* y, int y_dtype, float* dx, long n, float scale, void* stream) {
    if (!dy || !y || !dx) return hulc_fail(-1, "hulc_relu_bwd: null pointer");
    relu_bwd_kernel<<<(unsigned)((n + 255) / 256), 256, 0, (hipStream_t)stream>>>(dy, y, y_dtype, dx, n, scale);
    return hulc_check_launch("hulc_relu_bwd");
}

extern "C" int hulc_attention_fwd(const float* qkv, float* out, float* probs, int B, int S, int H, int head_dim, float drop_p,
                                  unsigned long long seed, const unsigned long long* seed_dev, void* stream) {
    if (!qkv || !out || !probs) return hulc_fail(-1, "hulc_attention_fwd: null pointer");
    if (S > 32 || S <= 0 || head_dim != ATT_DH) return hulc_fail(-2, "hulc_attention_fwd: needs S <= 32 and head_dim == 16");
    attention_fwd_kernel<<<B * H, 64, 0, (hipStream_t)stream>>>(qkv, out, probs, B, S, H, 1.0f / sqrtf((float)head_dim), drop_p, seed, seed_dev);
    return hulc_check_launch("hulc_attention_fwd");
}
extern "C" int hulc_attention_bwd(const float* qkv, const float* probs, const float* dout, float* dqkv, int B, int S, int H, int head_dim,
                                  float drop_p, unsigned long long seed, const unsigned long long* seed_dev, void* stream) {
    if (!qkv || !probs || !dout || !dqkv) return hulc_fail(-1, "hulc_attention_bwd: null pointer");
    if (S > 32 || S <= 0 || head_dim != ATT_DH) return hulc_fail(-2, "hulc_attention_bwd: needs S <= 32 and head_dim == 16");
    attention_bwd_kernel<<<B * H, 64, 0, (hipStream_t)stream>>>(qkv, probs, dout, dqkv, B, S, H, 1.0f / sqrtf((float)head_dim), drop_p, seed, seed_dev);
    return hulc_check_launch("hulc_attention_bwd");
}
```

hulc2_amd/functional.py:

```python
from typing import List, Optional, Sequence, Tuple

import os

import torch

from . import gradsink
from . import kernels as kn
from .shadow import weight_operand


def _scoped(cls):
    fwd, bwd = cls.forward, cls.backward

    def forward(ctx, *args):
        ctx._compute = kn.backward_compute()
        return fwd(ctx, *args)

    def backward(ctx, *grads):
        if ctx._compute == kn.get_compute():
            return bwd(ctx, *grads)
        with kn.compute_scope(ctx._compute):
            return bwd(ctx, *grads)

    forward.__doc__, backward.__doc__ = fwd.__doc__, bwd.__doc__
# ... 415 lines not shown
            gz = torch.empty(g.shape, dtype=torch.float32, device=g.device)
            kn.relu_bwd(g.float() if g.dtype != torch.float32 else g, a3, gz, g.numel())
            g = gz
        inputs = (None, a1, a2)
        weights = (None, w2, w3)
        grads_w, grads_b = [None] * 3, [None] * 3
        for li in (2, 1, 0):
            h, w_, cin, cout, k, s, nchw = dims[li]
            (dw, db), acc, (rw, grads_b[li]) = gradsink.joint((ctx.conv_w[li], ctx.conv_b[li]), ((cout, cin * k * k), None), g)
            if li == 0:
                off = 0
                pad, shifts, indices = ctx.aug
                paired = False
                if _conv1_pair_ok(xs, xs[0].dtype == torch.uint8, None, cout, shifts, indices) and g.dtype == torch.bfloat16:
                    pair_shift, pair_index = getattr(ctx, "pair_aug", (None, None))
                    try:
                        kn.conv2d_bwd_weight(xs[0], g, dw, db, N, h, w_, cin, cout, k, k, s, nchw, dw_oihw=True, accumulate=acc,
                                             x2=None if pair_index is not None else xs[1], aug_shift=pair_shift, aug_pad=pad, frame_index=pair_index)
                        paired = True
                    except kn._L.HulcKernelError as e:
                        if not _pair_not_covered(e):
                            raise
                if not paired:
                    for j, (x, n, sh, ix) in enumerate(zip(xs, Ns, shifts, indices)):
                        kn.conv2d_bwd_weight(x, g[off:off + n], dw, db, n, h, w_, cin, cout, k, k, s, nchw, dw_oihw=True, accumulate=acc or j > 0,
                                             aug_shift=sh, aug_pad=pad, frame_index=ix)
                        off += n
            else:
                kn.conv2d_bwd_weight(inputs[li], g, dw, db, N, h, w_, cin, cout, k, k, s, nchw, dw_oihw=True, accumulate=acc)
            grads_w[li] = None if rw is None else rw.view(cout, cin, k, k)
            if li > 0:
                inp = inputs[li]
                wt = weight_operand(weights[li], "ihwo")
                dx = torch.empty(N, h, w_, cin, dtype=inp.dtype, device=g.device)
                kn.conv2d_bwd_data(g, wt, dx, inp, N, h, w_, cin, cout, k, k, s, relu_bits=ctx.relu_bits[li - 1])
                g = dx
        return (None, None, grads_w[0], grads_b[0], grads_w[1], grads_b[1], grads_w[2], grads_b[2], *([None] * len(xs)))


def conv_stack(x, params, grad_premasked=False, aug_pad=0, aug_shifts=None, frame_index=None, exact_out=False):
    xs = list(x) if isinstance(x, (list, tuple)) else [x]
    aug = None
    if xs[0].dtype == torch.uint8:
        sh = list(aug_shifts) if isinstance(aug_shifts, (list, tuple)) else [aug_shifts] * len(xs)
        ix = list(frame_index) if isinstance(frame_index, (list, tuple)) else [frame_index] * len(xs)
        aug = (int(aug_pad), [None if t is None else _c(t.reshape(-1, 2).to(torch.int32)) for t in sh],
               [None if t is None else _c(t.reshape(-1).to(torch.int32)) for t in ix])
    out = ConvStackFn.apply((bool(grad_premasked), True) if exact_out else grad_premasked, aug, *params, *xs)
    if isinstance(out, tuple):
        out[0]._hulc_f32 = out[1]
        return out[0]
    return out


def exact_map(a: torch.Tensor):
    t = getattr(a, "_hulc_f32", None)
    return t if (t is not None and t.shape == a.shape) else None


@_scoped
class SpatialSoftmaxFn(torch.autograd.Function):

    @staticmethod
    def forward(ctx, a, xmap, ymap, temperature, a_exact=None):
        N, H, W, C = a.shape
        out = _f32(N, 2 * C, like=a)
        stats = _f32(N, C, 2, like=a)
        kn.spatial_softmax_fwd(a_exact if a_exact is not None else a, N, H * W, C, xmap, ymap, temperature, out, stats)
        ctx.save_for_backward(a, xmap, ymap, temperature, out, stats)
        return out

    @staticmethod
    def backward(ctx, dout):
        a, xmap, ymap, temperature, out, stats = ctx.saved_tensors
        N, H, W, C = a.shape
        gdt = torch.bfloat16 if (a.dtype == torch.float32 and kn.base_mode() == "bf16" and kn.get_compute() == "bf16") else a.dtype
        dx = torch.empty(a.shape, dtype=gdt, device=a.device)
        kn.spatial_softmax_bwd(a, N, H * W, C, xmap, ymap, temperature, out, stats, _c(dout), dx, relu_mask=True)
        return dx, None, None, None, None


def spatial_softmax(a, xmap, ymap, temperature):
    return SpatialSoftmaxFn.apply(a, xmap, ymap, temperature, exact_map(a))


@_scoped
class LayerNormFn(torch.autograd.Function):
    @staticmethod
    def forward(ctx, x, o, gamma, beta, eps: float, drop_p: float, seed: int):
        D = x.shape[-1]
        x2 = _c(x.reshape(-1, D))
        o2 = _c(o.reshape(-1, D)) if o is not None else None
        R = x2.shape[0]
        y = _f32(R, D, like=x2)
        mean, rstd = _f32(R, like=x2), _f32(R, like=x2)
        pre = _f32(R, D, like=x2) if o2 is not None else None
        kn.layernorm_fwd(x2, o2, drop_p, seed, gamma, beta, eps, R, D, pre, y, mean, rstd)
        ctx.save_for_backward(pre if pre is not None else x2, mean, rstd, gamma)
        ctx.beta = beta
        ctx.meta = (x.shape, o is not None, drop_p, seed)
        return y.reshape(x.shape)

    @staticmethod
    def backward(ctx, dy):
        pre, mean, rstd, gamma = ctx.saved_tensors
        shape, has_o, drop_p, seed = ctx.meta
        R, D = pre.shape
        dy2 = _c(dy.reshape(R, D))
        dpre = _f32(R, D, like=dy2)
        do = _f32(R, D, like=dy2) if (has_o and drop_p > 0) else None
        (dg, db), acc, (rg, rb) = gradsink.joint((gamma, ctx.beta), None, dy2)
        kn.layernorm_bwd(dy2, pre, mean, rstd, gamma, R, D, dpre, do, drop_p, seed, dg, db, accumulate_params=acc)
        dx = dpre.reshape(shape)
        d_o = None
        if has_o:
            d_o = (do if do is not None else dpre).reshape(shape)
        return dx, d_o, rg, rb, None, None, None


def layer_norm(x, gamma, beta, eps=1e-5):
    return LayerNormFn.apply(x, None, gamma, beta, eps, 0.0, 0)


def add_layer_norm(x, o, gamma, beta, eps=1e-5, drop_p=0.0, seed=0):
    return LayerNormFn.apply(x, o, gamma, beta, eps, drop_p, seed)


@_scoped
class LayerNormCatFn(torch.autograd.Function):

    @staticmethod
    def forward(ctx, dim: int, eps: float, n: int, *args):
        xs = [_c(x.reshape(-1, x.shape[-1])) for x in args[:n]]
        params = args[n:]
        if dim == 0:
            D = xs[0].shape[1]
            R = sum(x.shape[0] for x in xs)
            offs, acc = [], 0
            for x in xs:
                offs.append(acc * D)
                acc += x.shape[0]
            ld = D
        else:
            R = xs[0].shape[0]
            D = sum(x.shape[1] for x in xs)
            offs, acc = [], 0
            for x in xs:
                offs.append(acc)
                acc += x.shape[1]
            ld = D
        y = _f32(R, D, like=xs[0])
        flat = y.view(-1)
        stats = []
        for i, x in enumerate(xs):
            r, d = x.shape
            mean, rstd = _f32(r, like=x), _f32(r, like=x)
            kn.layernorm_fwd_ld(x, params[2 * i], params[2 * i + 1], eps, r, d, flat[offs[i]:], ld, mean, rstd)
            stats += [mean, rstd]
        ctx.save_for_backward(*xs, *stats, *[params[2 * i] for i in range(n)])
        ctx.betas = [params[2 * i + 1] for i in range(n)]
        ctx.meta = (n, offs, ld, [tuple(a.shape) for a in args[:n]])
        return y

    @staticmethod
    def backward(ctx, dy):
        n, offs, ld, shapes = ctx.meta
        sv = ctx.saved_tensors
        xs, stats, gammas = sv[:n], sv[n:3 * n], sv[3 * n:]
        dyf = _c(dy).view(-1)
        dxs, dps = [], []
        for i in range(n):
            x, gamma, beta = xs[i], gammas[i], ctx.betas[i]
            r, d = x.shape
            dx = _f32(r, d, like=dyf)
            (dg, db), acc, rets = gradsink.joint((gamma, beta), None, dyf)
            kn.layernorm_bwd_ld(dyf[offs[i]:], ld, x, stats[2 * i], stats[2 * i + 1], gamma, r, d, dx, dg, db, accumulate_params=acc)
            dxs.append(dx.reshape(shapes[i]))
            dps += rets
        return (None, None, None, *dxs, *dps)


def layer_norm_cat(xs, norms, dim: int):
    params = [t for m in norms for t in (m.weight, m.bias)]
    return LayerNormCatFn.apply(int(dim), float(norms[0].eps), len(xs), *xs, *params)


@_scoped
class PlanSampleKLFn(torch.autograd.Function):

    @staticmethod
    def forward(ctx, pp, pr, idx_in, G: int, CLS: int, seed: int, beta, mix: float, nseg: int):
        beta, beta_dev = _kl_beta(beta)
        pp, pr = _c(pp), _c(pr)
        B = pr.shape[0]
        plan = _f32(B, G * CLS, like=pr)
        idx = torch.empty(B, G, dtype=torch.long, device=pr.device)
        kn.plan_sample_fwd(pr, _c(idx_in) if idx_in is not None else None, seed, B * G, CLS, idx, plan)
        out = _f32(nseg, like=pp)
        klg = _f32(B * G, like=pp)
        kn.cat_kl_fwd(pp, pr, B, G, CLS, beta, out, klg, nseg, beta_dev=beta_dev)
        ctx.save_for_backward(pp, pr, klg)
        ctx.meta = (B, G, CLS, beta, beta_dev, mix, nseg)
        ctx.mark_non_differentiable(idx)
        ctx.set_materialize_grads(False)
        return plan, idx, out

    @staticmethod
    def backward(ctx, dplan, _didx=None, gkl=None):
        pp, pr, klg = ctx.saved_tensors
        B, G, CLS, beta, beta_dev, mix, nseg = ctx.meta
        dpp = dpr = None
        if gkl is not None:
            dpp, dpr = torch.empty_like(pp), torch.empty_like(pr)
            kn.cat_kl_bwd(pp, pr, klg, B, G, CLS, beta, mix, _c(gkl.reshape(nseg)), dpp, dpr, nseg, beta_dev=beta_dev)
        if dplan is not None:
            if dpr is None:
                dpr = torch.empty_like(pr)
                kn.plan_sample_bwd(pr, _c(dplan), B * G, CLS, dpr)
            else:
                kn.plan_sample_bwd(pr, _c(dplan), B * G, CLS, dpr, accumulate=True)
        return dpp, dpr, None, None, None, None, None, None, None


@_scoped
class GaussPlanKLFn(torch.autograd.Function):

    @staticmethod
    def forward(ctx, pp, pr, eps_in, seed: int, beta, mix: float, nseg: int):
        beta, beta_dev = _kl_beta(beta)
        pp, pr = _c(pp), _c(pr)
        B, P = pr.shape[0], pr.shape[1] // 2
        eps_in = _c(eps_in) if eps_in is not None else None
        plan = _f32(B, P, like=pr)
        out = _f32(nseg, like=pp)
        klr = _f32(B, like=pp)
        kn.gauss_plan_fwd(pp, pr, eps_in, seed, B, P, beta, nseg, plan, None, out, klr, beta_dev=beta_dev)
        ctx.save_for_backward(pp, pr, eps_in)
        ctx.meta = (B, P, seed, beta, beta_dev, mix, nseg)
        ctx.set_materialize_grads(False)
        return plan, out

    @staticmethod
    def backward(ctx, dplan, gkl=None):
        pp, pr, eps_in = ctx.saved_tensors
        B, P, seed, beta, beta_dev, mix, nseg = ctx.meta
        if dplan is None and gkl is None:
            return None, None, None, None, None, None, None
        dpr = torch.empty_like(pr)
        dpp = torch.empty_like(pp) if gkl is not None else None
        kn.gauss_plan_bwd(pp, pr, eps_in, seed, B, P, beta, mix, nseg, _c(dplan) if dplan is not None else None,
                          _c(gkl.reshape(nseg)) if gkl is not None else None, dpp, dpr, beta_dev=beta_dev if gkl is not None else None)
        return dpp, dpr, None, None, None, None, None


@_scoped
class GaussPlanSampleFn(torch.autograd.Function):

    @staticmethod
    def forward(ctx, raw, eps_in, seed: int):
        raw = _c(raw)
        B, P = raw.shape[0], raw.shape[1] // 2
        eps_in = _c(eps_in) if eps_in is not None else None
        plan = _f32(B, P, like=raw)
        kn.gauss_plan_fwd(None, raw, eps_in, seed, B, P, 0.0, 1, plan, None, None, None)
        ctx.save_for_backward(raw, eps_in)
        ctx.meta = (B, P, seed)
        return plan

    @staticmethod
    def backward(ctx, dplan):
        raw, eps_in = ctx.saved_tensors
        B, P, seed = ctx.meta
        draw = torch.empty_like(raw)
        kn.gauss_plan_bwd(None, raw, eps_in, seed, B, P, 0.0, 0.0, 1, _c(dplan), None, None, draw)
        return draw, None, None


@_scoped
class GaussKLFn(torch.autograd.Function):

    @staticmethod
    def forward(ctx, pp, pr, beta, mix: float, nseg: int = 1):
        beta, beta_dev = _kl_beta(beta)
        pp, pr = _c(pp), _c(pr)
        B, P = pr.shape[0], pr.shape[1] // 2
        out = _f32(nseg, like=pp)
        klr = _f32(B, like=pp)
        kn.gauss_plan_fwd(pp, pr, None, 0, B, P, beta, nseg, None, None, out, klr, beta_dev=beta_dev)
        ctx.save_for_backward(pp, pr)
        ctx.meta = (B, P, beta, beta_dev, mix, nseg)
        return out[0] if nseg == 1 else out

    @staticmethod
    def backward(ctx, g):
        pp, pr = ctx.saved_tensors
        B, P, beta, beta_dev, mix, nseg = ctx.meta
        dpp, dpr = torch.empty_like(pp), torch.empty_like(pr)
        kn.gauss_plan_bwd(pp, pr, None, 0, B, P, beta, mix, nseg, None, _c(g.reshape(nseg)), dpp, dpr, beta_dev=beta_dev)
        return dpp, dpr, None, None, None


def _pos_table_grad(demb, pos, pshape, pos_ids):
    B, S, D = demb.shape
    if pos is not None and gradsink.get(pos) is not None:
        sink, acc, _ = gradsink.dest(pos, None, demb)
        kn.colsum(demb, B, S * D, S * D, sink[:S].view(-1), accumulate=acc)
        if not acc and pshape[0] > S:
            sink[S:].zero_()
        return None
    dsum = _f32(S, D, like=demb)
    kn.colsum(demb, B, S * D, S * D, dsum)
    dpos = torch.zeros(pshape, dtype=torch.float32, device=demb.device)
    dpos.index_copy_(0, pos_ids, dsum)
    return dpos


@_scoped
class AddPosFn(torch.autograd.Function):

    @staticmethod
    def forward(ctx, x, pos, pos_ids, drop_p: float, seed: int, identity: bool = False):
        B, S, D = x.shape
        y = _f32(B, S, D, like=x)
        kn.add_pos_fwd(_c(x), pos, pos_ids, y, B, S, D, drop_p, seed)
        ctx.save_for_backward(pos_ids)
        ctx.meta = (B, S, D, drop_p, seed, pos.shape)
        ctx.pos = pos if identity else None
        return y

    @staticmethod
    def backward(ctx, dy):
        (pos_ids,) = ctx.saved_tensors
        B, S, D, drop_p, seed, pshape = ctx.meta
        dy = _c(dy)
        if drop_p > 0:
            dx = torch.empty_like(dy)
            kn.dropout_bwd(dy, dx, dy.numel(), drop_p, seed)
        else:
            dx = dy
        return dx, _pos_table_grad(dx, ctx.pos if dx.dtype == torch.float32 else None, pshape, pos_ids), None, None, None, None


@_scoped
class SeqMeanFn(torch.autograd.Function):
    @staticmethod
    def forward(ctx, x):
        B, S, D = x.shape
        y = _f32(B, D, like=x)
        kn.seq_mean_fwd(_c(x), y, B, S, D)
        ctx.meta = (B, S, D)
        return y

    @staticmethod
    def backward(ctx, dy):
        B, S, D = ctx.meta
        dx = _f32(B, S, D, like=dy)
        kn.seq_mean_bwd(_c(dy), dx, B, S, D)
        return dx


@_scoped
class AttentionFn(torch.autograd.Function):

    @staticmethod
    def forward(ctx, qkv, B: int, S: int, H: int, drop_p: float, seed: int):
        E = qkv.shape[-1] // 3
        dh = E // H
        qkv = _c(qkv)
        out = _f32(B * S, E, like=qkv)
        probs = _f32(B, H, S, S, like=qkv)
        kn.attention_fwd(qkv, out, probs, B, S, H, dh, drop_p, seed)
        ctx.save_for_backward(qkv, probs)
        ctx.meta = (B, S, H, dh, drop_p, seed)
# ... 612 lines not shown
```

hulc2_amd/kernels.py:

```python
import ctypes

import torch

from . import lib as _L

F32, BF16, F16 = (_L.DEFINES["HULC_" + n] for n in ("F32", "BF16", "F16"))
_COMPUTE = {"bf16": BF16, "fp32": F32, "f32": F32}
_compute_mode = BF16


_base_mode = "bf16"
_bwd_mode = None


def set_compute(mode: str) -> None:
    global _compute_mode, _base_mode, _bwd_mode
    if mode not in ("bf16", "fp32", "mixed"):
        raise ValueError(mode)
    _base_mode, _bwd_mode = mode, None
    _compute_mode = _COMPUTE["bf16" if mode == "mixed" else mode]


def get_compute() -> str:
    return "bf16" if _compute_mode == BF16 else "fp32"
# ... 963 lines not shown
    T, H, OUT = x.shape[0], W1.shape[0], W2T.shape[1]
    _call("hulc_mlp2_rows_bwd", x, dy, W1, b1, W1T, W2T, T, 128, H, OUT, dx, h, dh, key=("mlp2_rows_bwd", T, H, OUT),
          flops=2.0 * T * H * (2 * 128 + OUT), nbytes=_nbytes(x, dy, W1, W1T, W2T, dx, h, dh))


def txl_block_desc(emb, pos, pos_ids, B, S, H, FF, drop_p, seed_pos, eps, layers, pooled=None, dpooled=None, demb=None, share=None):
    d = _L.TxlBlockDesc()
    _require_cuda(emb, pos, pos_ids, pooled, dpooled, demb)
    _require_contiguous(emb=emb, pos=pos)
    if len(layers) > _L.TXL_MAX_LAYERS:
        raise _L.HulcKernelError("txl_block: at most %d layers" % _L.TXL_MAX_LAYERS)
    d.L, d.B, d.S, d.H, d.E, d.FF = len(layers), int(B), int(S), int(H), int(emb.shape[-1]), int(FF)
    d.eps, d.drop_p, d.seed_pos = float(eps), float(drop_p), int(seed_pos) & 0xFFFFFFFFFFFFFFFF
    d.seed_dev = step_state(emb.device).data_ptr() if drop_p > 0.0 else None
    d.emb, d.pos, d.pos_ids = emb.data_ptr(), pos.data_ptr(), pos_ids.data_ptr()
    d.pooled, d.dpooled, d.demb = [t.data_ptr() if t is not None else None for t in (pooled, dpooled, demb)]
    import os
    d.exclusive = int(not concurrent_streams() and not os.environ.get("HULC_TXL_NO_SHARE"))
    d.coop_share = int(_coop_share if share is None else share)
    if d.exclusive:
        need = _L.load().hulc_txl_block_workspace(B, len(layers))
        ws = _cached_ws(_chain_ws, (emb.device, _stream(), "txl"), need, need // 4 + 1)
        d._ws = ws
        d.ws, d.err_sticky = ws.data_ptr(), fault_word(emb.device).data_ptr()
    for i, rec in enumerate(layers):
        e = d.layers[i]
        for name, v in rec.items():
            if name.startswith("seed_"):
                setattr(e, name, int(v) & 0xFFFFFFFFFFFFFFFF)
            elif v is not None:
                _require_cuda(v)
                if not v.is_contiguous():
                    raise _L.HulcKernelError("txl_block: %s must be contiguous" % name)
                if name[0] == "W" and v.dtype != torch.bfloat16:
                    raise _L.HulcKernelError("txl_block: weights are the bf16 shadows (bf16 compute mode)")
                setattr(e, name, v.data_ptr())
    return d


def _txl_block_flops(B, S, H, E, FF, L, bwd):
    T = B * S
    attn = 2.0 * T * E * 4 * E + 2.0 * 2 * B * H * S * S * (E // H)
    ffn = 2.0 * T * E * FF * 2
    return L * ((2.5 * attn + 2.5 * ffn) if bwd else (attn + ffn))


def txl_block_fwd(d, B, S, H, E, FF, L):
    _call("hulc_txl_block_fwd", _c.byref(d), key=("txl_block_fwd", B, S, L), flops=_txl_block_flops(B, S, H, E, FF, L, False))


def txl_block_bwd(d, B, S, H, E, FF, L):
    _call("hulc_txl_block_bwd", _c.byref(d), key=("txl_block_bwd", B, S, L), flops=_txl_block_flops(B, S, H, E, FF, L, True))


def residual_bf16(p32, hi, lo, segments):
    _call("hulc_residual_bf16", p32, hi, lo, segments, segments.shape[0])


def gather_chunks(src0, src1, dst, idx):
    _call("hulc_gather_chunks", src0, src1, dst, idx, idx.numel())


def ffn_frag_perm(layout: int, FF: int):
    import numpy as np
    out = np.empty(FF * 128, dtype=np.int32)
    _L.check(_L.load().hulc_ffn_frag_perm(layout, FF, out.ctypes.data), "hulc_ffn_frag_perm")
    return out


def repack_conv_weights(src_f32, dst_bf16, table):
    _call("hulc_repack_conv_weights", src_f32, dst_bf16, table, table.shape[0])


def transpose_bf16_tiles(src, dst, tiles):
    _call("hulc_transpose_bf16_tiles", src, dst, tiles, tiles.shape[0])


def rnn_wavefront(z0, z_step, S, B, H, wA, wB1, wB2, transposed, add1=None, add1_step=0, ld_add1=0, bias1=(None, None), bias2=(None, None),
                  mask1=None, mask1_step=0, ld_mask1=0, mask2=None, mask2_step=0, ld_mask2=0, relu=False, mirror_t=False, add1c=None, zero_edges=False):
    for w in (wA, wB1, wB2):
        if w.dtype != torch.bfloat16:
            raise _L.HulcKernelError("rnn_wavefront: weights must be bf16 shadows (bf16 compute mode)")
    d = _L.RnnWaveDesc()
    d.z, d.z_step = z0.data_ptr(), int(z_step)
    d.wA, d.wB1, d.wB2 = wA.data_ptr(), wB1.data_ptr(), wB2.data_ptr()
    d.ldA, d.ldB1, d.ldB2 = wA.stride(0), wB1.stride(0), wB2.stride(0)
    if isinstance(transposed, (tuple, list)):
        d.tA, d.tB1, d.tB2 = (int(bool(t)) for t in transposed)
        transposed = d.tA
    else:
        d.tA = d.tB1 = d.tB2 = int(bool(transposed))
    d.add1, d.add1_step, d.ld_add1 = (add1.data_ptr() if add1 is not None else None), int(add1_step), int(ld_add1)
    d.bias1a, d.bias1b = [b.data_ptr() if b is not None else None for b in bias1]
    d.bias2a, d.bias2b = [b.data_ptr() if b is not None else None for b in bias2]
    d.mask1, d.mask1_step, d.ld_mask1 = (mask1.data_ptr() if mask1 is not None else None), int(mask1_step), int(ld_mask1)
    d.mask2, d.mask2_step, d.ld_mask2 = (mask2.data_ptr() if mask2 is not None else None), int(mask2_step), int(ld_mask2)
    d.relu, d.S, d.B, d.H = int(relu), int(S), int(B), int(H)
    d.mirror_t = int(bool(mirror_t))
    d.err_sticky = fault_word(z0.device).data_ptr()
    d.add1c, d.ld_add1c = (add1c.data_ptr(), add1c.stride(0)) if add1c is not None else (None, 0)
    d.zero_edges = int(bool(zero_edges))
    import os
    dbg = os.environ.get("HULC_RNN_DBG", "")
    d.inject_timeout = int(dbg) & 4 if dbg.isdigit() else 0
    lib = _L.load()
    ws = _ws(lib.hulc_rnn_wavefront_workspace(S, B, H), z0.device)
    flops = 2.0 * B * 3 * H * H * S
    nbytes = 3.0 * H * H * 2 + S * B * (2 * H * 4 + 2 * 2 * H * 2 + (H * 4 if add1 is not None else 0)
                                        + (H * 4 if mask1 is not None else 0) + (H * 4 if mask2 is not None else 0))
    _call("hulc_rnn_wavefront", _c.byref(d), ws, key=("rnn_wavefront", S, B, H, int(bool(transposed))), flops=flops, nbytes=nbytes)
    off = lib.hulc_rnn_wavefront_mirror_offset() // 2
    w16 = ws.view(torch.bfloat16)
    z16 = w16[off:off + (S + 2) * B * 2 * H].view(S + 2, B, 2 * H)
    offt = lib.hulc_rnn_wavefront_mirror_t_offset(S, B, H) // 2
    z16t = w16[offt:offt + (S + 2) * B * 2 * H].view(2 * H, (S + 2) * B) if (offt and mirror_t) else None
    return z16, z16t


def mix_loss_fwd(y, act, out, T, A, n_mix, num_classes, ld, log_scale_min, gripper_alpha, act_min, act_max, nseg=1, time_major_B=0):
    d = _mix_desc(T, A, n_mix, num_classes, ld, log_scale_min, gripper_alpha, act_min, act_max, nseg, time_major_B)
    ws = _ws(_L.load().hulc_mix_loss_workspace(_c.byref(d)), y.device)
    _call("hulc_mix_loss_fwd", _c.byref(d), y, act, out, ws)


def mix_loss_bwd(y, act, gout, dy, ld_dy, T, A, n_mix, num_classes, ld, log_scale_min, gripper_alpha, act_min, act_max, nseg=1, time_major_B=0):
    d = _mix_desc(T, A, n_mix, num_classes, ld, log_scale_min, gripper_alpha, act_min, act_max, nseg, time_major_B)
    _call("hulc_mix_loss_bwd", _c.byref(d), y, act, gout, dy, ld_dy)


def _beta_dev_ok(name, beta_dev, device):
    if not isinstance(beta_dev, torch.Tensor) or beta_dev.dtype != torch.float32 or beta_dev.numel() != 1 or beta_dev.device != device:
        raise _L.HulcKernelError(f"{name}: beta_dev is a one-element fp32 tensor on the operands' device")


def cat_kl_fwd(pp, pr, B, G, CLS, beta, out, kl_group, nseg=1, beta_dev=None):
    if beta_dev is None:
        return _call("hulc_cat_kl_fwd", pp, pr, B, G, CLS, beta, nseg, out, kl_group)
    _beta_dev_ok("cat_kl_fwd", beta_dev, _first_device(pp, pr, out))
    _call("hulc_cat_kl_fwd_sched", pp, pr, B, G, CLS, beta, nseg, out, kl_group, beta_dev)


def cat_kl_bwd(pp, pr, kl_group, B, G, CLS, beta, mix, gout, dpp, dpr, nseg=1, beta_dev=None):
    if beta_dev is None:
        return _call("hulc_cat_kl_bwd", pp, pr, kl_group, B, G, CLS, beta, mix, gout, nseg, dpp, dpr)
    _beta_dev_ok("cat_kl_bwd", beta_dev, _first_device(pp, pr, dpp))
    _call("hulc_cat_kl_bwd_sched", pp, pr, kl_group, B, G, CLS, beta, mix, gout, nseg, dpp, dpr, beta_dev)


def plan_sample_fwd(logits, idx_in, seed, NG, CLS, idx_out, plan):
    _call("hulc_plan_sample_fwd", logits, idx_in, seed, step_state(logits.device) if idx_in is None else None, NG, CLS,
          idx_out, plan)


def plan_sample_bwd(logits, dplan, NG, CLS, dlogits, accumulate=False):
    _call("hulc_plan_sample_bwd", logits, dplan, NG, CLS, dlogits, accumulate)


GAUSS_MIN_STD = 1e-4


def _first_device(*ts):
    for t in ts:
        if t is not None:
            _require_cuda(t)
            return t.device
    raise _L.HulcKernelError("no tensor operand")


def gauss_plan_fwd(pp, pr, eps_in, seed, B, P, beta, nseg, plan, eps_out, out, kl_row, min_std=GAUSS_MIN_STD, beta_dev=None):
    dev = _first_device(pr, pp, plan, eps_out, out)
    word = step_state(dev) if eps_in is None else None
    if beta_dev is None:
        return _call("hulc_gauss_plan_fwd", pp, pr, eps_in, seed, word, B, P, min_std, beta, nseg, plan, eps_out, out, kl_row)
    _beta_dev_ok("gauss_plan_fwd", beta_dev, dev)
    _call("hulc_gauss_plan_fwd_sched", pp, pr, eps_in, seed, word, B, P, min_std, beta, nseg, plan, eps_out, out, kl_row, beta_dev)


def gauss_plan_bwd(pp, pr, eps_in, seed, B, P, beta, mix, nseg, dplan, gout, dpp, dpr, min_std=GAUSS_MIN_STD, beta_dev=None):
    dev = _first_device(pr, pp, dplan, gout, dpr)
    word = step_state(dev) if eps_in is None else None
    if beta_dev is None:
        return _call("hulc_gauss_plan_bwd", pp, pr, eps_in, seed, word, B, P, min_std, beta, mix, nseg, dplan, gout, dpp, dpr)
    _beta_dev_ok("gauss_plan_bwd", beta_dev, dev)
    _call("hulc_gauss_plan_bwd_sched", pp, pr, eps_in, seed, word, B, P, min_std, beta, mix, nseg, dplan, gout, dpp, dpr, beta_dev)


def clip_loss_fwd(im, tx, use, logit_scale, M, D, out, row0=0):
    _call("hulc_clip_loss_fwd", im, tx, use, row0, logit_scale, M, D, out)


def clip_loss_bwd(im, tx, use, logit_scale, M, D, gout, dim, dtx, dscale, row0=0):
    _call("hulc_clip_loss_bwd", im, tx, use, row0, logit_scale, M, D, gout, dim, dtx, dscale)


def loss_combine_fwd(kls, acts, clip, n, beta, out):
    _call("hulc_loss_combine_fwd", kls, acts, clip, n, beta, out)


def loss_combine_bwd(g, n, beta, dkls, dacts, dclip):
    _call("hulc_loss_combine_bwd", g, n, beta, dkls, dacts, dclip)


def emb_fanout_fwd(emb, N, S, D, n_last, lo, hi, e0, elast, edec_t):
    _call("hulc_emb_fanout_fwd", emb, N, S, D, n_last, lo, hi, e0, elast, edec_t)


def emb_fanin_bwd(g_rec, g0, g_last, g_dec_t, N, S, D, n_last, lo, hi, demb):
    _call("hulc_emb_fanin_bwd", g_rec, g0, g_last, g_dec_t, N, S, D, n_last, lo, hi, demb)


def actions_time_major(acts, obss, B, S, obs_dim, to_tcp, out):
    n = len(acts)
    _require_cuda(*acts, out)
    A = (_c.c_void_p * n)(*[a.data_ptr() for a in acts])
    O = (_c.c_void_p * n)(*[o.data_ptr() for o in obss]) if to_tcp else None
    if to_tcp:
        _require_cuda(*obss)
    _call("hulc_actions_time_major", A, O, n, B, S, obs_dim, int(bool(to_tcp)), out)


def layernorm_fwd_ld(x, gamma, beta, eps, R, D, y, ld_y, mean, rstd):
    _call("hulc_layernorm_fwd_ld", x, gamma, beta, eps, R, D, y, ld_y, mean, rstd)


def layernorm_bwd_ld(dy, ld_dy, pre, mean, rstd, gamma, R, D, dpre, dgamma, dbeta, accumulate_params=False):
    ws = _ws(_L.load().hulc_layernorm_bwd_workspace(R, D), dy.device)
    _call("hulc_layernorm_bwd_ld", dy, ld_dy, pre, mean, rstd, gamma, R, D, dpre, dgamma, dbeta, accumulate_params, ws)


def world_to_tcp(act, robot_obs, n, obs_dim, out):
    _call("hulc_world_to_tcp", act, robot_obs, n, obs_dim, out)


def embed_ln_fwd(ids, word, pos, type0, gamma, beta, eps, T, S, D, out):
    if ids.dtype != torch.int64 or not ids.is_contiguous():
        raise TypeError("embed_ln_fwd: token ids are a contiguous int64 tensor")
    for name, t in (("word", word), ("pos", pos)):
        if t.dtype != torch.float32 or t.dim() != 2 or t.shape[1] != D or not t.is_contiguous():
            raise TypeError(f"embed_ln_fwd: {name} is a contiguous fp32 (rows, {D}) table")
    for name, t, n in (("type0", type0, D), ("gamma", gamma, D), ("beta", beta, D), ("out", out, T * D)):
        if t.dtype != torch.float32 or t.numel() != n or not t.is_contiguous():
            raise TypeError(f"embed_ln_fwd: {name} is a contiguous fp32 tensor of {n} elements")
    if ids.numel() != T:
        raise ValueError(f"embed_ln_fwd: {ids.numel()} token ids for T = {T}")
    if S > pos.shape[0]:
        raise ValueError(f"embed_ln_fwd: S = {S} exceeds the position table's {pos.shape[0]} rows")
    if T > 0 and not (ids.is_cuda and torch.cuda.is_current_stream_capturing()):
        lo, hi = (int(v) for v in torch.aminmax(ids))
        if lo < 0 or hi >= word.shape[0]:
            raise ValueError(f"embed_ln_fwd: token ids span [{lo}, {hi}], the vocabulary has {word.shape[0]} rows")
    _call("hulc_embed_ln_fwd", ids, word, pos, type0, gamma, beta, eps, T, S, D, out)
    return out


def ln_wide_fwd(x, add, gamma, beta, eps, R, D, y):
    _call("hulc_ln_wide_fwd", x, add, gamma, beta, eps, R, D, y)
    return y


def mha_masked_fwd(qkv, mask, B, S, nhead, hd, out):
    if mask.dtype != torch.int32 or not mask.is_contiguous():
        raise TypeError("mha_masked_fwd: the padding mask is a contiguous int32 (B, S) tensor")
    _call("hulc_mha_masked_fwd", qkv, mask, B, S, nhead, hd, out)
    return out


def masked_mean_fwd(x, mask, B, S, D, out):
    _call("hulc_masked_mean_fwd", x, mask, B, S, D, out)
    return out


def tcp_to_world(act, robot_obs, n, obs_dim, out):
    _call("hulc_tcp_to_world", act, robot_obs, n, obs_dim, out)


def mix_sample(y, ld, T, A, n_mix, log_scale_min, gripper_bounds, act_out, seed, u_mix=None, u_inv=None, idx_out=None):
    d = _mix_desc(T, A, n_mix, 0, ld, log_scale_min, 0.0, gripper_bounds, gripper_bounds)
    _call("hulc_mix_sample", _c.byref(d), y, u_mix, u_inv, seed, None, gripper_bounds, act_out, idx_out)


def window_index(starts, sizes, B, S, out):
    for t in (starts, sizes, out):
        if t.dtype != torch.int32 or not t.is_contiguous():
            raise TypeError("window_index: starts / sizes / out are contiguous int32 tensors")
    _call("hulc_window_index", starts, sizes, B, S, out)
    return out


def window_rows(store, starts, sizes, B, S, out, zero_cols=(0, 0)):
    if store.dtype != torch.float32 or out.dtype != torch.float32 or starts.dtype != torch.int32 or sizes.dtype != torch.int32:
        raise TypeError("window_rows: fp32 store / out, int32 starts / sizes")
    _require_contiguous(store=store, out=out, starts=starts, sizes=sizes)
    _call("hulc_window_rows", store, store.shape[-1], starts, sizes, B, S, zero_cols[0], zero_cols[1], out)
    return out


def adam_step(p, g, m, v, shadow, n, lr, beta1, beta2, eps, weight_decay, step, grad_scale=1.0, step_state_dev=None, lo=None, lo_ranges=(),
              loss_scale_dev=None, found_inf_dev=None, lr_dev=None, clip_coef_dev=None, clip_value=0.0):
    n_lo = sum(int(e) - int(b) for b, e in lo_ranges) if (lo is not None and lo_ranges) else 0
    nbytes = float(n) * (16 + 12 + (2 if shadow is not None else 0)) + 2.0 * n_lo
    if clip_coef_dev is not None or clip_value:
        _call("hulc_adam_step_clip", p, g, m, v, shadow, n, lr, beta1, beta2, eps, weight_decay, step, step_state_dev, grad_scale,
              *_rule_tail("adam_step", p, lo, lo_ranges, loss_scale_dev, found_inf_dev, lr_dev, (), clip_coef_dev)[:7], clip_coef_dev,
              float(clip_value), nbytes=nbytes)
        return
    if lr_dev is not None or loss_scale_dev is not None or found_inf_dev is not None:
        for t in (lr_dev, loss_scale_dev, found_inf_dev):
            if t is not None and (not isinstance(t, torch.Tensor) or t.dtype != torch.float32 or t.numel() != 1 or t.device != p.device):
                raise _L.HulcKernelError("adam_step: lr_dev / loss_scale / found_inf are one-element fp32 tensors on the parameters' device")
        has_lo = lo is not None and bool(lo_ranges)
        flat = [int(x) for r in lo_ranges for x in r] if has_lo else [0, 0]
        arr = (_c.c_long * len(flat))(*flat)
        args = (p, g, m, v, shadow, n, lr, beta1, beta2, eps, weight_decay, step, step_state_dev, grad_scale, fault_word(p.device),
                lo if has_lo else None, arr if has_lo else None, len(lo_ranges) if has_lo else 0, loss_scale_dev, found_inf_dev)
        if lr_dev is not None:
            _call("hulc_adam_step_sched", *args, lr_dev, nbytes=nbytes)
        else:
            _call("hulc_adam_step_amp", *args, nbytes=nbytes)
        return
    if lo is None or not lo_ranges:
        _call("hulc_adam_step", p, g, m, v, shadow, n, lr, beta1, beta2, eps, weight_decay, step,
              step_state_dev, grad_scale, fault_word(p.device), nbytes=nbytes)
        return
    flat = [int(x) for r in lo_ranges for x in r]
    arr = (_c.c_long * len(flat))(*flat)
    _call("hulc_adam_step_lo", p, g, m, v, shadow, n, lr, beta1, beta2, eps, weight_decay, step,
          step_state_dev, grad_scale, fault_word(p.device), lo, arr, len(lo_ranges), nbytes=nbytes)


def _rule_tail(name, p, lo, lo_ranges, loss_scale_dev, found_inf_dev, lr_dev, skip_ranges, clip_coef_dev=None):
    for t in (lr_dev, loss_scale_dev, found_inf_dev, clip_coef_dev):
        if t is not None and (not isinstance(t, torch.Tensor) or t.dtype != torch.float32 or t.numel() != 1 or t.device != p.device):
            raise _L.HulcKernelError(f"{name}: lr_dev / loss_scale / found_inf / clip_coef are one-element fp32 tensors on the parameters' device")
    has_lo = lo is not None and bool(lo_ranges)
    flat = [int(x) for r in lo_ranges for x in r] if has_lo else [0, 0]
    arr = (_c.c_long * len(flat))(*flat)
    skip = [int(x) for r in skip_ranges for x in r]
    sarr = (_c.c_long * max(len(skip), 2))(*skip)
    return (fault_word(p.device), lo if has_lo else None, arr if has_lo else None, len(lo_ranges) if has_lo else 0, loss_scale_dev,
            found_inf_dev, lr_dev, sarr if skip else None, len(skip) // 2)


def adamw_step(p, g, m, v, shadow, n, lr, beta1, beta2, eps, weight_decay, step, grad_scale=1.0, step_state_dev=None, lo=None, lo_ranges=(),
               loss_scale_dev=None, found_inf_dev=None, lr_dev=None, skip_ranges=(), clip_coef_dev=None, clip_value=0.0):
    n_lo = sum(int(e) - int(b) for b, e in lo_ranges) if (lo is not None and lo_ranges) else 0
    nbytes = float(n) * (16 + 12 + (2 if shadow is not None else 0)) + 2.0 * n_lo
    tail = _rule_tail("adamw_step", p, lo, lo_ranges, loss_scale_dev, found_inf_dev, lr_dev, skip_ranges, clip_coef_dev)
    clip = (clip_coef_dev, float(clip_value)) if (clip_coef_dev is not None or clip_value) else ()
    _call("hulc_adamw_step_clip" if clip else "hulc_adamw_step", p, g, m, v, shadow, n, lr, beta1, beta2, eps, weight_decay, step, step_state_dev,
          grad_scale, *tail, *clip, nbytes=nbytes)


def sgd_step(p, g, buf, shadow, n, lr, momentum, dampening, nesterov, weight_decay, step, grad_scale=1.0, step_state_dev=None, lo=None,
             lo_ranges=(), loss_scale_dev=None, found_inf_dev=None, lr_dev=None, skip_ranges=(), clip_coef_dev=None, clip_value=0.0):
    n_lo = sum(int(e) - int(b) for b, e in lo_ranges) if (lo is not None and lo_ranges) else 0
    nbytes = float(n) * (12 + (8 if (buf is not None and momentum != 0) else 0) + (2 if shadow is not None else 0)) + 2.0 * n_lo
    tail = _rule_tail("sgd_step", p, lo, lo_ranges, loss_scale_dev, found_inf_dev, lr_dev, skip_ranges, clip_coef_dev)
    clip = (clip_coef_dev, float(clip_value)) if (clip_coef_dev is not None or clip_value) else ()
    _call("hulc_sgd_step_clip" if clip else "hulc_sgd_step", p, g, buf, shadow, n, lr, momentum, dampening, int(bool(nesterov)), weight_decay, step,
          step_state_dev, grad_scale, *tail, *clip, nbytes=nbytes)


_grad_norm_ws = {}


def grad_norm_clip(g, n, grad_scale, loss_scale_dev, max_norm, out):
    for t, k in ((out, 2), (loss_scale_dev, 1)):
        if t is not None and (not isinstance(t, torch.Tensor) or t.dtype != torch.float32 or t.numel() != k or t.device != g.device or not t.is_contiguous()):
            raise _L.HulcKernelError("grad_norm_clip: out is two fp32 elements, loss_scale one, contiguous on the gradients' device")
    if g.dtype != torch.float32 or not g.is_contiguous() or g.numel() < n:
        raise _L.HulcKernelError("grad_norm_clip: g is a contiguous fp32 tensor of at least n elements")
    need = int(_L.load().hulc_grad_norm_ws_bytes(int(n)))
    ws = _grad_norm_ws.get(g.device)
    if ws is None or ws.numel() * 8 < need:
        ws = _grad_norm_ws[g.device] = torch.empty(max(need // 8, 2048), dtype=torch.float64, device=g.device)
    _call("hulc_grad_norm_clip", g, int(n), float(grad_scale), loss_scale_dev, float(max_norm), out, ws, nbytes=4.0 * n)


def step_count_advance_if(state, found_inf_dev=None) -> None:
    _call("hulc_step_count_advance_if", state, found_inf_dev)
# ... 217 lines not shown
```

include/hulc2_amd.h:

```cpp
#ifndef HULC2_AMD_H
#define HULC2_AMD_H

#ifdef __cplusplus
extern "C" {
#endif

#define HULC_F32 0
#define HULC_BF16 1
#define HULC_F16 2

const char* hulc_last_error(void);
const char* hulc_conv_last_path(void);
int hulc_abi_version(void);
int hulc_stream_create(void** out);

typedef struct {
    const void* A; const void* B; void* C;
    const float* bias; const void* add; const void* mask;
    int M, N, K;
    long lda, ldb, ldc, ld_add, ld_mask;
    int a_dtype, b_dtype, c_dtype, add_dtype, mask_dtype;
    int a_kmajor, b_kmajor;
    int relu, accumulate;
    float alpha, mask_scale, drop_p;
    unsigned long long drop_seed;
    int compute;
    int generic_only;
    void* ws; long ws_bytes;
    const unsigned long long* seed_dev;
    float* rowsum_a; int rowsum_accumulate;
} hulc_gemm_desc;
int hulc_gemm(const hulc_gemm_desc* d, void* stream);


typedef struct {
    int N, H, W, Cin, Cout, KH, KW, stride;
    int x_nchw;
    int x_dtype, y_dtype, w_dtype;
    int relu;
    int compute;
    int dw_oihw;
    int dw_accumulate;
    int x_u8_nhwc;
    int aug_pad;
    const int* aug_shift;
    const int* frame_index;
    void* relu_bits;
    const void* w_lo;
    const void* x2;
    int n_split;
    int conv1_slots;
    const void* x_slot;
    const void* x2_slot;
    void* y_bf16;
} hulc_conv_desc;
int hulc_conv2d_fwd(const hulc_conv_desc* d, const void* x, const void* w, const float* bias, void* y, void* stream);
int hulc_conv2d_bwd_data(const hulc_conv_desc* d, const void* dy, const void* wt, void* dx, const void* relu_src, void* stream);
long hulc_conv2d_bwd_weight_workspace(const hulc_conv_desc* d);
int hulc_conv2d_bwd_weight(const hulc_conv_desc* d, const void* x, const void* dy, float* dw, float* db, void* ws, void* stream);

int hulc_spatial_softmax_fwd(const void* x, int x_dtype, int N, int HW, int C, const float* xmap, const float* ymap,
                             const float* temperature, float* out, float* stats, void* stream);
int hulc_spatial_softmax_bwd(const void* x, int x_dtype, int N, int HW, int C, const float* xmap, const float* ymap,
                             const float* temperature, const float* out, const float* stats, const float* dout,
                             void* dx, int dx_dtype, int relu_mask, void* stream);
int hulc_layernorm_fwd(const float* x, const float* o, float drop_p, unsigned long long seed, const unsigned long long* seed_dev,
                       const float* gamma, const float* beta, float eps, int R, int D, float* pre_out, float* y, float* mean,
                       float* rstd, void* stream);
int hulc_layernorm_slab_fwd(const float* x, const float* o, int n_o, long o_stride, float drop_p, unsigned long long seed,
                            const unsigned long long* seed_dev, const float* gamma, const float* beta, float eps, int R, int D,
                            float* pre_out, float* y, float* mean, float* rstd, void* stream);
int hulc_layernorm_fwd_ld(const float* x, const float* gamma, const float* beta, float eps, int R, int D, float* y, long ld_y, float* mean,
                          float* rstd, void* stream);
int hulc_layernorm_bwd_ld(const float* dy, long ld_dy, const float* pre, const float* mean, const float* rstd, const float* gamma, int R, int D,
                          float* dpre, float* dgamma, float* dbeta, int accumulate_params, void* ws, void* stream);
long hulc_layernorm_bwd_workspace(int R, int D);
int hulc_layernorm_bwd(const float* dy, const float* pre, const float* mean, const float* rstd, const float* gamma, int R, int D,
                       float* dpre, float* do_out, float drop_p, unsigned long long seed, const unsigned long long* seed_dev,
                       float* dgamma, float* dbeta, int accumulate_params, void* ws, void* stream);
long hulc_colsum_workspace(long M, int N);
int hulc_colsum(const void* x, int x_dtype, long M, int N, long ld, float* out, int accumulate, void* ws, void* stream);
int hulc_seq_mean_fwd(const float* x, float* y, int B, int S, int D, float scale, void* stream);
int hulc_seq_mean_bwd(const float* dy, float* dx, int B, int S, int D, void* stream);
int hulc_strided_seq_sum(const void* x, int x_dtype, float* y, int B, int S, int D, long stride_b, long stride_s, long ldy,
                         float scale, void* stream);
int hulc_add_pos_fwd(const float* x, const float* pos, const long* pos_ids, float* y, int B, int S, int D, float drop_p,
                     unsigned long long seed, const unsigned long long* seed_dev, void* stream);
int hulc_dropout_bwd(const float* dy, float* dx, long n, float drop_p, unsigned long long seed, const unsigned long long* seed_dev,
                     void* stream);
int hulc_relu_bwd(const float* dy, const void* y, int y_dtype, float* dx, long n, float scale, void* stream);
int hulc_attention_fwd(const float* qkv, float* out, float* probs, int B, int S, int H, int head_dim, float drop_p,
                       unsigned long long seed, const unsigned long long* seed_dev, void* stream);
int hulc_attention_bwd(const float* qkv, const float* probs, const float* dout, float* dqkv, int B, int S, int H, int head_dim,
                       float drop_p, unsigned long long seed, const unsigned long long* seed_dev, void* stream);

typedef struct {
    int T, A, n_mix, num_classes, nseg;
    long ld;
    float log_scale_min, gripper_alpha;
    const float* act_min; const float* act_max;
    int time_major_B;
} hulc_mix_desc;
long hulc_mix_loss_workspace(const hulc_mix_desc* d);
int hulc_mix_loss_fwd(const hulc_mix_desc* d, const float* y, const float* act, float* out, void* ws, void* stream);
int hulc_mix_loss_bwd(const hulc_mix_desc* d, const float* y, const float* act, const float* gout, float* dy, long ld_dy, void* stream);
int hulc_cat_kl_fwd(const float* pp, const float* pr, int B, int G, int CLS, float beta, int nseg, float* out, float* kl_group, void* stream);
int hulc_cat_kl_bwd(const float* pp, const float* pr, const float* kl_group, int B, int G, int CLS, float beta, float mix,
                    const float* gout, int nseg, float* dpp, float* dpr, void* stream);
int hulc_plan_sample_fwd(const float* logits, const long* idx_in, unsigned long long seed, const unsigned long long* seed_dev,
                         int NG, int CLS, long* idx_out, float* plan, void* stream);
int hulc_plan_sample_bwd(const float* logits, const float* dplan, int NG, int CLS, float* dlogits, int accumulate, void* stream);
int hulc_gauss_plan_fwd(const float* pp, const float* pr, const float* eps_in, unsigned long long seed, const unsigned long long* seed_dev,
                        int B, int P, float min_std, float beta, int nseg, float* plan, float* eps_out, float* out, float* kl_row,
                        void* stream);
int hulc_gauss_plan_bwd(const float* pp, const float* pr, const float* eps_in, unsigned long long seed, const unsigned long long* seed_dev,
                        int B, int P, float min_std, float beta, float mix, int nseg, const float* dplan, const float* gout, float* dpp,
                        float* dpr, void* stream);
int hulc_cat_kl_fwd_sched(const float* pp, const float* pr, int B, int G, int CLS, float beta, int nseg, float* out, float* kl_group,
                          const float* beta_dev, void* stream);
int hulc_cat_kl_bwd_sched(const float* pp, const float* pr, const float* kl_group, int B, int G, int CLS, float beta, float mix,
                          const float* gout, int nseg, float* dpp, float* dpr, const float* beta_dev, void* stream);
int hulc_gauss_plan_fwd_sched(const float* pp, const float* pr, const float* eps_in, unsigned long long seed,
                              const unsigned long long* seed_dev, int B, int P, float min_std, float beta, int nseg, float* plan,
                              float* eps_out, float* out, float* kl_row, const float* beta_dev, void* stream);
int hulc_gauss_plan_bwd_sched(const float* pp, const float* pr, const float* eps_in, unsigned long long seed,
                              const unsigned long long* seed_dev, int B, int P, float min_std, float beta, float mix, int nseg,
                              const float* dplan, const float* gout, float* dpp, float* dpr, const float* beta_dev, void* stream);
int hulc_clip_loss_fwd(const float* im, const float* tx, const unsigned char* use, int row0, const float* logit_scale, int M, int D,
                       float* out, void* stream);
int hulc_clip_loss_bwd(const float* im, const float* tx, const unsigned char* use, int row0, const float* logit_scale, int M, int D,
                       const float* gout, float* dim, float* dtx, float* dscale, void* stream);
int hulc_loss_combine_fwd(const float* kls, const float* acts, const float* clip, int n, float beta, float* out, void* stream);
int hulc_loss_combine_bwd(const float* g, int n, float beta, float* dkls, float* dacts, float* dclip, void* stream);
int hulc_emb_fanout_fwd(const float* emb, int N, int S, int D, int n_last, int lo, int hi, float* e0, float* elast, float* edec_t, void* stream);
int hulc_emb_fanin_bwd(const float* g_rec, const float* g0, const float* g_last, const float* g_dec_t, int N, int S, int D, int n_last, int lo, int hi,
                       float* demb, void* stream);
int hulc_world_to_tcp(const float* act, const float* robot_obs, int n, int obs_dim, float* out, void* stream);
int hulc_actions_time_major(const float* const* act, const float* const* robot_obs, int nseg, int B, int S, int obs_dim, int to_tcp, float* out,
                            void* stream);
int hulc_tcp_to_world(const float* act, const float* robot_obs, int n, int obs_dim, float* out, void* stream);
int hulc_mix_sample(const hulc_mix_desc* d, const float* y, const float* u_mix, const float* u_inv, unsigned long long seed,
                    const unsigned long long* seed_dev, const float* gripper_bounds, float* act_out, long* idx_out, void* stream);

int hulc_window_index(const int* starts, const int* sizes, int B, int S, int* index_out, void* stream);
int hulc_window_rows(const float* store, int D, const int* starts, const int* sizes, int B, int S, int zero_lo, int zero_hi,
                     float* out, void* stream);

int hulc_embed_ln_fwd(const long* ids, const float* word, const float* pos, const float* type0, const float* gamma, const float* beta,
                      float eps, int T, int S, int D, float* out, void* stream);
int hulc_ln_wide_fwd(const float* x, const float* add, const float* gamma, const float* beta, float eps, int R, int D, float* y, void* stream);
int hulc_mha_masked_fwd(const float* qkv, const int* mask, int B, int S, int nhead, int hd, float* out, void* stream);
int hulc_masked_mean_fwd(const float* x, const int* mask, int B, int S, int D, float* out, void* stream);

int hulc_r3m_normalize(const float* x, int N, int H, int W, const float* mean3, const float* std3, void* y, int y_dtype, void* stream);
int hulc_conv2d_padded_fwd(const hulc_conv_desc* d, int pad, const void* x, const void* w, const float* bias, const void* add, void* y,
                           void* stream);
int hulc_maxpool_nhwc(const void* x, int dtype, int N, int H, int W, int C, int k, int stride, int pad, void* y, void* stream);
long hulc_nhwc_bn_train_workspace(long M, int C);
int hulc_nhwc_bn_train_fwd(const void* z, int z_dtype, long M, int C, const float* gamma, const float* beta, float eps, float momentum,
                           float* run_mean, float* run_var, const void* add, int add_dtype, int relu, void* y, int y_dtype, void* ws, void* stream);
int hulc_nhwc_bn_train_fwd_saved(const void* z, int z_dtype, long M, int C, const float* gamma, const float* beta, float eps, float momentum,
                                 float* run_mean, float* run_var, const void* add, int add_dtype, int relu, void* y, int y_dtype, float* saved, void* ws,
                                 void* stream);
int hulc_nhwc_bn_train_bwd(const void* dy, int dy_dtype, const void* y, int y_dtype, const float* z, long M, int C, const float* gamma,
                           const float* saved, void* dz, void* g_out, int o_dtype, float* dgamma, float* dbeta, int accumulate_params, void* ws,
                           void* stream);
int hulc_maxpool_nhwc_bwd(const void* x, const void* dy, int dtype, int N, int H, int W, int C, int k, int stride, int pad, void* dx, void* stream);
int hulc_nhwc_scatter(const void* x, int dtype, int N, int H, int W, int C, int Hy, int Wy, int step, int off, void* y, void* stream);
int hulc_r3m_packed_width(int W);
int hulc_r3m_normalize_packed(const float* x, int N, int H, int W, const float* mean3, const float* std3, void* xp, void* stream);
int hulc_r3m_stem_fwd(const void* xp, const void* w, const float* bias, void* y, int y_dtype, int N, int H, int W, int Cout, int relu, void* stream);

long hulc_ffn_workspace(int T, int FF);
int hulc_ffn_fwd(const float* x, const void* W1, const float* b1, const void* W2, const float* b2, int T, int D, int FF, float drop_p,
                 unsigned long long seed, const unsigned long long* seed_dev, float* f, void* ws, void* stream);
int hulc_ffn_bwd(const float* x, const float* df, const void* W1, const float* b1, const void* W1T, const void* W2T, int T, int D, int FF,
                 float drop_p, unsigned long long seed, const unsigned long long* seed_dev, float* dx, int dx_accumulate,
                 float* dW1, float* db1, float* dW2, int accumulate_params, void* ws, void* stream);

typedef struct hulc_txl_attn_desc {
    const float* x;
    const void *Wqkv, *Wo, *WqkvT, *WoT;
    const float *bqkv, *bo, *gamma, *beta;
    float eps;
    int B, S, H, E;
    float drop_p;
    unsigned long long seed_attn, seed_ln;
    const unsigned long long* seed_dev;
    float *y, *pre, *mean, *rstd;
    void* ctx;
    const float *dy, *dy_slab;
    int n_slab;
    long slab_stride;
    float* dx;
    void *d_o, *dqkv;
    float* ln_partial;
} hulc_txl_attn_desc;
int hulc_ln_partial_reduce(const float* partial, int P, int D, float* dgamma, float* dbeta, int accumulate, void* stream);
int hulc_ln_partial_reduce_multi(const float* partial, int n, int P, int D, float* const* dgamma, float* const* dbeta, const int* accumulate,
                                 void* stream);
int hulc_txl_attn_fwd(const hulc_txl_attn_desc* d, void* stream);
int hulc_txl_attn_bwd(const hulc_txl_attn_desc* d, void* stream);

int hulc_mlp2_rows_fwd(const float* x, const void* W1, const float* b1, const void* W2, const float* b2, const void* W1_lo, const void* W2_lo,
                       int T, int K, int H, int OUT, float* y, void* stream);
int hulc_mlp2_rows_bwd(const float* x, const float* dy, const void* W1, const float* b1, const void* W1T, const void* W2T, int T, int K, int H, int OUT,
                       float* dx, void* h, void* dh, void* stream);

#define HULC_TXL_MAX_LAYERS 4
typedef struct hulc_txl_block_layer {
    const void *Wqkv, *Wo, *W1, *W2;
    const void *WqkvT, *WoT, *W1T, *W2T;
    const void *W1p, *W2p, *W2Tp, *W1Tp;
    const void *Wqkv_lo, *Wo_lo, *W1p_lo, *W2p_lo;
    const float *bqkv, *bo, *b1, *b2, *g1, *be1, *g2, *be2;
    unsigned long long seed_attn, seed_ln1, seed_ffn, seed_ln2;
    float* x;
    float *y1, *pre1, *mean1, *rstd1;
    void* ctx;
    float *y2, *pre2, *mean2, *rstd2;
    void *d_o, *dqkv, *df, *h, *dh;
    float *lnp1, *lnp2;
} hulc_txl_block_layer;
typedef struct hulc_txl_block_desc {
    int L, B, S, H, E, FF;
    float eps, drop_p;
    unsigned long long seed_pos;
    const unsigned long long* seed_dev;
    const float* emb;
    const float* pos;
    const long* pos_ids;
    float* pooled;
    const float* dpooled;
    float* demb;
    void* ws;
    int exclusive;
    int coop_share;
    int* err_sticky;
    hulc_txl_block_layer layers[HULC_TXL_MAX_LAYERS];
} hulc_txl_block_desc;
long hulc_txl_block_workspace(int B, int L);
int hulc_txl_block_fwd(const hulc_txl_block_desc* d, void* stream);
int hulc_txl_block_bwd(const hulc_txl_block_desc* d, void* stream);

typedef struct hulc_mlp_chain_layer {
    const void* W; long ldw;
    const void* W_lo;
    const float* bias;
    const float* mask; long ld_mask; float mask_scale;
    float* out; long ld_out;
    int N, relu;
} hulc_mlp_chain_layer;
typedef struct hulc_mlp_chain_desc {
    int nl, M, K0;
    int coop_share;
    const float* x0; long ld_x0;
    hulc_mlp_chain_layer layers[8];
} hulc_mlp_chain_desc;
long hulc_mlp_chain_workspace(const hulc_mlp_chain_desc* d);
int hulc_mlp_chain(const hulc_mlp_chain_desc* d, void* ws, int* err_sticky, void* stream);
int hulc_mlp_chain2(const hulc_mlp_chain_desc* a, const hulc_mlp_chain_desc* b, void* ws, int* err_sticky, void* stream);

typedef struct hulc_wgrad_item {
    const void* A; const void* B; float* C; float* rowsum;
    int M, N, K;
    int lda, ldb, ldc;
    int a_dtype, b_dtype;
    int accumulate, rowsum_accumulate;
    int col_perm;
    int col_mul;
    int store_rows;
    int conv_taps_wp;
} hulc_wgrad_item;
long hulc_wgrad_group_workspace(const hulc_wgrad_item* items, int n);
int hulc_wgrad_group(const hulc_wgrad_item* items, int n, void* ws, long ws_bytes, void* stream);

int hulc_gridconv3x3_fused(const void* x, long ldx, const void* wt, void* y, long ldy, int N, int H, int W, int Cin, int Cout, const float* bias,
                           const void* add, long ldadd, int relu, void* stream);
int hulc_grid_from_nhwc(const void* x, int N, int H, int W, int C, void* y, long ldy, void* stream);
long hulc_gridconv_stats_bytes(int N, int H, int W, int Cout);
// ... 101 lines not shown
```

Baseline: 20740 play-sequences/s.

## Fuse reduction tails via last-block counters, batch layernorms, merge KL sample backward

Adds a per-device pool of device-side finish counters. Small-grid reductions (mix loss, categorical KL, gaussian plan KL, colsum) now finish their final reduction in the last-arriving block instead of launching a second kernel. Layernorm forward and backward over several inputs are batched into one multi-tensor launch, and the categorical KL backward and the plan-sample backward are merged into a single kernel. Together these cut kernel launch count and intermediate traffic in the graph, at the cost of atomic counter state that must be created outside a capture first, plus extra synchronisation inside the reducing kernels.

```diff
diff --git a/hulc2_amd/csrc/abi.hip b/hulc2_amd/csrc/abi.hip
--- a/hulc2_amd/csrc/abi.hip
+++ b/hulc2_amd/csrc/abi.hip
@@ -2,6 +2,7 @@
 #include <stdarg.h>
 #include <stdio.h>
 #include <string.h>
+#include <mutex>
 
 static thread_local char g_err[512] = "";
 
@@ -34,6 +35,51 @@
 }
 
 extern "C" const char* hulc_conv_last_path(void) { return g_conv_path; }
+
+namespace {
+constexpr unsigned FIN_EAGER = 4096, FIN_CAPTURED = 61440, FIN_DEVICES = 64;
+struct FinPool { unsigned* base; unsigned eager, captured; };
+FinPool g_fin[FIN_DEVICES];
+std::mutex g_fin_mu;
+}
+
+unsigned* hulc_finish_counters(unsigned n, hipStream_t s, const char* who) {
+    char msg[256];
+    int dev = -1;
+    hipStreamCaptureStatus st = hipStreamCaptureStatusNone;
+    if (n < 1 || n > HULC_FINISH_MAX || hipGetDevice(&dev) != hipSuccess || dev < 0 || dev >= (int)FIN_DEVICES ||
+        hipStreamIsCapturing(s, &st) != hipSuccess) {
+        snprintf(msg, sizeof(msg), "%s: no finish counters (count, device or stream state)", who);
+        hulc_fail(-100, msg);
+        return nullptr;
+    }
+    const bool capturing = st != hipStreamCaptureStatusNone;
+    std::lock_guard<std::mutex> lock(g_fin_mu);
+    FinPool& p = g_fin[dev];
+    if (!p.base) {
+        if (capturing) {
+            snprintf(msg, sizeof(msg), "%s: first call on this device is inside a stream capture; run it once outside a capture first "
+                     "(the finish counters are created, and zeroed, there)", who);
+            hulc_fail(-100, msg);
+            return nullptr;
+        }
+        unsigned* b = nullptr;
+        const size_t bytes = (size_t)(FIN_EAGER + FIN_CAPTURED) * sizeof(unsigned);
+        if (hipMalloc((void**)&b, bytes) != hipSuccess || hipMemset(b, 0, bytes) != hipSuccess || hipDeviceSynchronize() != hipSuccess) {
+            if (b) (void)hipFree(b);
+            snprintf(msg, sizeof(msg), "%s: could not create the finish counters", who);
+            hulc_fail(-100, msg);
+            return nullptr;
+        }
+        p.base = b;
+    }
+    unsigned& cur = capturing ? p.captured : p.eager;
+    const unsigned size = capturing ? FIN_CAPTURED : FIN_EAGER;
+    if (cur + n > size) cur = 0;
+    unsigned* out = p.base + (capturing ? FIN_EAGER : 0u) + cur;
+    cur += n;
+    return out;
+}
 extern "C" int hulc_abi_version(void) { return 7; }
 
 extern "C" int hulc_stream_create(void** out) {
diff --git a/hulc2_amd/csrc/hulc_abi_internal.h b/hulc2_amd/csrc/hulc_abi_internal.h
--- a/hulc2_amd/csrc/hulc_abi_internal.h
+++ b/hulc2_amd/csrc/hulc_abi_internal.h
@@ -4,6 +4,10 @@
 
 int hulc_fail(int code, const char* msg);
 int hulc_check_launch(const char* where);
+
+#define HULC_FINISH_MAX 1024u
+constexpr int FIN_MAX_ARRIVALS = 64;
+unsigned* hulc_finish_counters(unsigned n, hipStream_t s, const char* who);
 
 void hulc_conv_path_clear(void);
 void hulc_conv_path_set(const char* fmt, ...) __attribute__((format(printf, 1, 2)));
diff --git a/hulc2_amd/csrc/hulc_common.h b/hulc2_amd/csrc/hulc_common.h
--- a/hulc2_amd/csrc/hulc_common.h
+++ b/hulc2_amd/csrc/hulc_common.h
@@ -201,6 +201,21 @@
     return v;
 }
 
+HULC_DEVICE void fin_store(float* p, float v) { __hip_atomic_store(p, v, __ATOMIC_RELAXED, __HIP_MEMORY_SCOPE_AGENT); }
+HULC_DEVICE float fin_load(const float* p) { return __hip_atomic_load(p, __ATOMIC_RELAXED, __HIP_MEMORY_SCOPE_AGENT); }
+HULC_DEVICE bool fin_last_arriver(unsigned* ctr, unsigned expected, int* s_last) {
+    asm volatile("s_waitcnt vmcnt(0)" ::: "memory");
+    __syncthreads();
+    if (threadIdx.x == 0) {
+        const unsigned old = __hip_atomic_fetch_add(ctr, 1u, __ATOMIC_RELAXED, __HIP_MEMORY_SCOPE_AGENT);
+        const int last = old == expected - 1u;
+        if (last) __hip_atomic_store(ctr, 0u, __ATOMIC_RELAXED, __HIP_MEMORY_SCOPE_AGENT);
+        *s_last = last;
+    }
+    __syncthreads();
+    return *s_last != 0;
+}
+
 HULC_DEVICE uint64_t hulc_rand64(uint64_t seed, uint64_t idx) {
     uint64_t z = idx * 0x9E3779B97F4A7C15ull + seed;
     z = (z ^ (z >> 30)) * 0xBF58476D1CE4E5B9ull;
diff --git a/hulc2_amd/csrc/losses.hip b/hulc2_amd/csrc/losses.hip
--- a/hulc2_amd/csrc/losses.hip
+++ b/hulc2_amd/csrc/losses.hip
@@ -97,8 +97,28 @@
     return -lse;
 }
 
-__global__ __launch_bounds__(256) void mix_loss_partial_kernel(MixP p, int seg_tokens, int blocks_per_seg, float* __restrict__ partial) {
+HULC_DEVICE void mix_loss_segment(const float* partial, int seg, int nseg, int blocks_per_seg, int seg_tokens, float gripper_alpha,
+                                  float* __restrict__ out) {
+    const int lane = threadIdx.x & 63;
+    float nll = 0.f, ce = 0.f;
+    const float* ps = partial + 2 * (long)seg * blocks_per_seg;
+    for (int b = lane; b < blocks_per_seg; b += 256) {
+        float vn[4], vc[4];
+#pragma unroll
+        for (int k = 0; k < 4; ++k)
+            if (b + 64 * k < blocks_per_seg) { vn[k] = fin_load(ps + 2 * (b + 64 * k)); vc[k] = fin_load(ps + 2 * (b + 64 * k) + 1); }
+#pragma unroll
+        for (int k = 0; k < 4; ++k)
+            if (b + 64 * k < blocks_per_seg) { nll += vn[k]; ce += vc[k]; }
+    }
+    nll = wave_sum(nll); ce = wave_sum(ce);
+    nll /= seg_tokens; ce /= seg_tokens;
+    if (lane == 0) { out[seg] = nll + gripper_alpha * ce; out[nseg + seg] = nll; out[2 * nseg + seg] = ce; }
+}
+__global__ __launch_bounds__(256) void mix_loss_partial_kernel(MixP p, int seg_tokens, int blocks_per_seg, float* __restrict__ partial, int nseg,
+                                                               unsigned* fin_ctr, float* __restrict__ out) {
     __shared__ float sh[16];
+    __shared__ int s_last;
     const int seg = blockIdx.x / blocks_per_seg, bl = blockIdx.x % blocks_per_seg;
     const int w = bl * 16 + (threadIdx.x >> 4), i = threadIdx.x & 15;
     float nll = 0.f, ce = 0.f;
@@ -117,18 +137,16 @@
     }
     nll = block_sum(nll, sh);
     ce = block_sum(ce, sh);
-    if (threadIdx.x == 0) { partial[2 * blockIdx.x] = nll; partial[2 * blockIdx.x + 1] = ce; }
-}
-
+    if (threadIdx.x == 0) {
+        if (fin_ctr) { fin_store(partial + 2 * blockIdx.x, nll); fin_store(partial + 2 * blockIdx.x + 1, ce); }
+        else { partial[2 * blockIdx.x] = nll; partial[2 * blockIdx.x + 1] = ce; }
+    }
+    if (!fin_ctr || !fin_last_arriver(fin_ctr, gridDim.x, &s_last)) return;
+    for (int seg = threadIdx.x >> 6; seg < nseg; seg += 4) mix_loss_segment(partial, seg, nseg, blocks_per_seg, seg_tokens, p.gripper_alpha, out);
+}
 __global__ __launch_bounds__(64) void mix_loss_final_kernel(const float* __restrict__ partial, int blocks_per_seg, int seg_tokens,
                                                             float gripper_alpha, float* __restrict__ out) {
-    const int seg = blockIdx.x;
-    float nll = 0.f, ce = 0.f;
-    for (int b = threadIdx.x; b < blocks_per_seg; b += 64) { nll += partial[2 * (seg * blocks_per_seg + b)]; ce += partial[2 * (seg * blocks_per_seg + b) + 1]; }
-    nll = wave_sum(nll); ce = wave_sum(ce);
-    if (threadIdx.x != 0) return;
-    nll /= seg_tokens; ce /= seg_tokens;
-    out[seg] = nll + gripper_alpha * ce; out[gridDim.x + seg] = nll; out[2 * gridDim.x + seg] = ce;
+    mix_loss_segment(partial, blockIdx.x, gridDim.x, blocks_per_seg, seg_tokens, gripper_alpha, out);
 }
 
 __global__ __launch_bounds__(256) void mix_loss_bwd_kernel(MixP p, int seg_tokens, const float* __restrict__ gout, float* __restrict__ dy, long ld_dy) {
@@ -161,17 +179,44 @@
     return v;
 }
 
+struct KlFin { unsigned* ctr; int NG_seg, B_seg, nseg; float beta; const float* beta_dev; float* out; };
+
+__device__ void cat_kl_sum_tail(const float* kl, const KlFin& f, float* sh) {
+    const float beta = f.beta_dev ? *f.beta_dev : f.beta;
+    const int lane = threadIdx.x & 63, wave = threadIdx.x >> 6, nw = blockDim.x >> 6;
+    for (int seg = 0; seg < f.nseg; ++seg) {
+        const float* kg = kl + (long)seg * f.NG_seg;
+        __syncthreads();
+        for (int v = wave; v < 16; v += nw) {
+            float acc = 0.f;
+            for (int g = v * 64 + lane; g < f.NG_seg; g += 1024) acc += fin_load(kg + g);
+            acc = wave_sum(acc);
+            if (lane == 0) sh[v] = acc;
+        }
+        __syncthreads();
+        if (threadIdx.x == 0) {
+            float t = 0.f;
+            for (int w = 0; w < 16; ++w) t += sh[w];
+            f.out[seg] = beta * t / f.B_seg;
+        }
+    }
+}
+
 __global__ __launch_bounds__(256) void cat_kl_group_kernel(const float* __restrict__ pp, const float* __restrict__ pr, int NG,
-                                                           float* __restrict__ kl_group) {
+                                                           float* __restrict__ kl_group, KlFin fin) {
+    __shared__ float sh[16];
+    __shared__ int s_last;
     const int lane = threadIdx.x & 31;
     const int g = blockIdx.x * (blockDim.x >> 5) + (threadIdx.x >> 5);
-    if (g >= NG) return;
-    const float a = pr[(long)g * 32 + lane], b = pp[(long)g * 32 + lane];
-    const float ma = sub32_max(a), mb = sub32_max(b);
-    const float lp = a - (ma + logf(sub32_sum(expf(a - ma))));
-    const float lq = b - (mb + logf(sub32_sum(expf(b - mb))));
-    const float kl = sub32_sum(expf(lp) * (lp - lq));
-    if (lane == 0) kl_group[g] = kl;
+    if (g < NG) {
+        const float a = pr[(long)g * 32 + lane], b = pp[(long)g * 32 + lane];
+        const float ma = sub32_max(a), mb = sub32_max(b);
+        const float lp = a - (ma + logf(sub32_sum(expf(a - ma))));
+        const float lq = b - (mb + logf(sub32_sum(expf(b - mb))));
+        const float kl = sub32_sum(expf(lp) * (lp - lq));
+        if (lane == 0) { if (fin.ctr) fin_store(kl_group + g, kl); else kl_group[g] = kl; }
+    }
+    if (fin.ctr && fin_last_arriver(fin.ctr, gridDim.x, &s_last)) cat_kl_sum_tail(kl_group, fin, sh);
 }
 __global__ __launch_bounds__(1024) void cat_kl_sum_kernel(const float* __restrict__ kl_group, int NG_seg, int B_seg, float beta,
                                                           const float* __restrict__ beta_dev, float* __restrict__ out) {
@@ -245,6 +290,36 @@
     dlogits[i] = accumulate ? dlogits[i] + v : v;
 }
 
+__global__ __launch_bounds__(256) void cat_kl_sample_bwd_kernel(const float* __restrict__ pp, const float* __restrict__ pr,
+                                                                const float* __restrict__ kl_group, int B, int G, float beta,
+                                                                const float* __restrict__ beta_dev, float mix, const float* __restrict__ gout,
+                                                                int nseg, const float* __restrict__ dplan, float* __restrict__ dpp,
+                                                                float* __restrict__ dpr) {
+    const int lane = threadIdx.x & 31;
+    const int g = blockIdx.x * (blockDim.x >> 5) + (threadIdx.x >> 5);
+    if (g >= B * G) return;
+    if (beta_dev) beta = *beta_dev;
+    const int Bs = B / nseg;
+    gout += (g / G) / Bs;
+    B = Bs;
+    const long i = (long)g * 32 + lane;
+    const float a = pr[i], b = pp[i];
+    const float ma = sub32_max(a), mb = sub32_max(b);
+    const float lp = a - (ma + logf(sub32_sum(expf(a - ma))));
+    const float lq = b - (mb + logf(sub32_sum(expf(b - mb))));
+    const float p = expf(lp), q = expf(lq);
+    const float s = gout[0] * beta / B;
+    dpp[i] = s * mix * (q - p);
+    float dkl = s * (1.f - mix) * p * (lp - lq - kl_group[g]);
+    const float e = expf(a - ma);
+    const float ps = e / sub32_sum(e);
+    const float gd = dplan[i];
+    const float dot = sub32_sum(ps * gd);
+    float v = ps * (gd - dot);
+    asm volatile("" : "+v"(dkl), "+v"(v));
+    dpr[i] = dkl + v;
+}
+
 HULC_DEVICE float softplus_grad(float r) { return r > 20.f ? 1.f : sigmoid_f(r); }
 HULC_DEVICE void gauss_pair(uint64_t seed, uint64_t pair, float& z0, float& z1) {
     const float u1 = hulc_uniform01(seed, 2 * pair), u2 = hulc_uniform01(seed, 2 * pair + 1);
@@ -257,8 +332,10 @@
 __global__ __launch_bounds__(128) void gauss_plan_row_kernel(const float* __restrict__ pp, const float* __restrict__ pr,
                                                              const float* __restrict__ eps_in, unsigned long long seed,
                                                              const unsigned long long* __restrict__ seed_dev, int P, float min_std,
-                                                             float* __restrict__ plan, float* __restrict__ eps_out, float* __restrict__ kl_row) {
+                                                             float* __restrict__ plan, float* __restrict__ eps_out, float* __restrict__ kl_row,
+                                                             KlFin fin) {
     __shared__ float sh[16];
+    __shared__ int s_last;
     const int b = blockIdx.x, NP = (P + 1) >> 1;
     if (seed_dev) seed ^= seed_dev[0];
     const float* q = pr + (long)b * 2 * P;
@@ -287,7 +364,8 @@
     }
     if (kl_row) {
         acc = block_sum(acc, sh);
-        if (threadIdx.x == 0) kl_row[b] = acc;
+        if (threadIdx.x == 0) { if (fin.ctr) fin_store(kl_row + b, acc); else kl_row[b] = acc; }
+        if (fin.ctr && fin_last_arriver(fin.ctr, gridDim.x, &s_last)) cat_kl_sum_tail(kl_row, fin, sh);
     }
 }
 
@@ -554,8 +632,10 @@
     int rc = mix_check(d, "fwd"); if (rc) return rc;
     const int seg_tokens = d->T / d->nseg, bps = (seg_tokens * (d->A + 1) + 15) / 16;
     hipStream_t s = (hipStream_t)stream;
-    mix_loss_partial_kernel<<<d->nseg * bps, 256, 0, s>>>(make_mix(d, y, act), seg_tokens, bps, (float*)ws);
-    mix_loss_final_kernel<<<d->nseg, 64, 0, s>>>((const float*)ws, bps, seg_tokens, d->gripper_alpha, out);
+    unsigned* ctr = nullptr;
+    if ((long)d->nseg * bps <= FIN_MAX_ARRIVALS && !(ctr = hulc_finish_counters(1, s, "hulc_mix_loss_fwd"))) return -100;
+    mix_loss_partial_kernel<<<d->nseg * bps, 256, 0, s>>>(make_mix(d, y, act), seg_tokens, bps, (float*)ws, d->nseg, ctr, out);
+    if (!ctr) mix_loss_final_kernel<<<d->nseg, 64, 0, s>>>((const float*)ws, bps, seg_tokens, d->gripper_alpha, out);
     return hulc_check_launch("hulc_mix_loss_fwd");
 }
 extern "C" int hulc_mix_loss_bwd(const hulc_mix_desc* d, const float* y, const float* act, const float* gout, float* dy, long ld_dy,
@@ -582,8 +662,10 @@
     if (!pp || !pr || !out || !kl_group) return fail_named(-1, name, "null pointer");
     if (CLS != 32) return fail_named(-2, name, "class_size must be 32 (one 32-lane sub-wave per category)");
     if (nseg < 1 || B % nseg) return fail_named(-2, name, "the batch must split evenly into nseg segments");
-    cat_kl_group_kernel<<<(B * G + 7) / 8, 256, 0, (hipStream_t)stream>>>(pp, pr, B * G, kl_group);
-    cat_kl_sum_kernel<<<nseg, 1024, 0, (hipStream_t)stream>>>(kl_group, B / nseg * G, B / nseg, beta, beta_dev, out);
+    KlFin fin = {nullptr, B / nseg * G, B / nseg, nseg, beta, beta_dev, out};
+    if (((long)B * G + 7) / 8 <= FIN_MAX_ARRIVALS && !(fin.ctr = hulc_finish_counters(1, (hipStream_t)stream, name))) return -100;
+    cat_kl_group_kernel<<<(B * G + 7) / 8, 256, 0, (hipStream_t)stream>>>(pp, pr, B * G, kl_group, fin);
+    if (!fin.ctr) cat_kl_sum_kernel<<<nseg, 1024, 0, (hipStream_t)stream>>>(kl_group, B / nseg * G, B / nseg, beta, beta_dev, out);
     return hulc_check_launch(name);
 }
 static int cat_kl_bwd_impl(const char* name, const float* pp, const float* pr, const float* kl_group, int B, int G, int CLS, float beta,
@@ -594,6 +676,17 @@
     cat_kl_bwd_kernel<<<(B * G + 7) / 8, 256, 0, (hipStream_t)stream>>>(pp, pr, kl_group, B, G, beta, beta_dev, mix, gout, nseg, dpp, dpr);
     return hulc_check_launch(name);
 }
+extern "C" int hulc_cat_kl_sample_bwd(const float* pp, const float* pr, const float* kl_group, int B, int G, int CLS, float beta, float mix,
+                                      const float* gout, int nseg, const float* dplan, float* dpp, float* dpr, const float* beta_dev,
+                                      void* stream) {
+    if (!pp || !pr || !kl_group || !gout || !dplan || !dpp || !dpr) return hulc_fail(-1, "hulc_cat_kl_sample_bwd: null pointer");
+    if (CLS != 32) return hulc_fail(-2, "hulc_cat_kl_sample_bwd: class_size must be 32");
+    if (nseg < 1 || B % nseg) return hulc_fail(-2, "hulc_cat_kl_sample_bwd: the batch must split evenly into nseg segments");
+    if (beta_dev && (uintptr_t)beta_dev % 4) return hulc_fail(-4, "hulc_cat_kl_sample_bwd: beta_dev must be 4-byte aligned");
+    cat_kl_sample_bwd_kernel<<<(B * G + 7) / 8, 256, 0, (hipStream_t)stream>>>(pp, pr, kl_group, B, G, beta, beta_dev, mix, gout, nseg, dplan, dpp,
+                                                                               dpr);
+    return hulc_check_launch("hulc_cat_kl_sample_bwd");
+}
 extern "C" int hulc_cat_kl_fwd(const float* pp, const float* pr, int B, int G, int CLS, float beta, int nseg, float* out, float* kl_group, void* stream) {
     return cat_kl_fwd_impl("hulc_cat_kl_fwd", pp, pr, B, G, CLS, beta, nullptr, nseg, out, kl_group, stream);
 }
@@ -634,8 +727,13 @@
     if (!pr || (out && (!pp || !kl_row))) return fail_named(-1, name, "null pointer");
     if (B < 1 || P < 1) return fail_named(-2, name, "needs B >= 1 and plan_features >= 1");
     if (out && (nseg < 1 || B % nseg)) return fail_named(-2, name, "the batch must split evenly into nseg segments");
-    gauss_plan_row_kernel<<<B, 128, 0, (hipStream_t)stream>>>(pp, pr, eps_in, seed, seed_dev, P, min_std, plan, eps_out, out ? kl_row : nullptr);
-    if (out) cat_kl_sum_kernel<<<nseg, 1024, 0, (hipStream_t)stream>>>(kl_row, B / nseg, B / nseg, beta, beta_dev, out);
+    KlFin fin = {nullptr, 0, 0, 0, 0.f, nullptr, nullptr};
+    if (out) {
+        fin = KlFin{nullptr, B / nseg, B / nseg, nseg, beta, beta_dev, out};
+        if (B <= FIN_MAX_ARRIVALS && !(fin.ctr = hulc_finish_counters(1, (hipStream_t)stream, name))) return -100;
+    }
+    gauss_plan_row_kernel<<<B, 128, 0, (hipStream_t)stream>>>(pp, pr, eps_in, seed, seed_dev, P, min_std, plan, eps_out, out ? kl_row : nullptr, fin);
+    if (out && !fin.ctr) cat_kl_sum_kernel<<<nseg, 1024, 0, (hipStream_t)stream>>>(kl_row, B / nseg, B / nseg, beta, beta_dev, out);
     return hulc_check_launch(name);
 }
 static int gauss_plan_bwd_impl(const char* name, const float* pp, const float* pr, const float* eps_in, unsigned long long seed,
diff --git a/hulc2_amd/csrc/pointwise.hip b/hulc2_amd/csrc/pointwise.hip
--- a/hulc2_amd/csrc/pointwise.hip
+++ b/hulc2_amd/csrc/pointwise.hip
@@ -220,16 +220,11 @@
 }
 
 
-__global__ __launch_bounds__(256) void layernorm_fwd_kernel(const float* __restrict__ x, const float* __restrict__ o, float drop_p,
-                                                            unsigned long long seed, const unsigned long long* __restrict__ seed_dev,
-                                                            const float* __restrict__ gamma,
-                                                            const float* __restrict__ beta, float eps, int R, int D,
-                                                            float* __restrict__ pre_out, float* __restrict__ y,
-                                                            float* __restrict__ mean_out, float* __restrict__ rstd_out,
-                                                            int n_o = 1, long o_stride = 0, long ld_y = 0) {
+HULC_DEVICE void layernorm_fwd_row(int r, const float* __restrict__ x, const float* __restrict__ o, float drop_p, unsigned long long seed,
+                                   const unsigned long long* __restrict__ seed_dev, const float* __restrict__ gamma,
+                                   const float* __restrict__ beta, float eps, int D, float* __restrict__ pre_out, float* __restrict__ y,
+                                   float* __restrict__ mean_out, float* __restrict__ rstd_out, int n_o, long o_stride, long ld_y) {
     const int lane = threadIdx.x & 63;
-    const int r = blockIdx.x * 4 + (threadIdx.x >> 6);
-    if (r >= R) return;
     if (seed_dev) seed ^= seed_dev[0];
     float v[4];
     float s = 0.f;
@@ -274,14 +269,57 @@
     }
     if (lane == 0) { mean_out[r] = mean; rstd_out[r] = rstd; }
 }
-
-__global__ __launch_bounds__(256) void layernorm_bwd_kernel(const float* __restrict__ dy, const float* __restrict__ pre,
-                                                            const float* __restrict__ mean_in, const float* __restrict__ rstd_in,
-                                                            const float* __restrict__ gamma, int R, int D, int rows_per_block,
-                                                            float* __restrict__ dpre, float* __restrict__ do_out, float drop_p,
+__global__ __launch_bounds__(256) void layernorm_fwd_kernel(const float* __restrict__ x, const float* __restrict__ o, float drop_p,
                                                             unsigned long long seed, const unsigned long long* __restrict__ seed_dev,
-                                                            float* __restrict__ partial, long ld_dy = 0) {
-    __shared__ float red[4][2][256];
+                                                            const float* __restrict__ gamma,
+                                                            const float* __restrict__ beta, float eps, int R, int D,
+                                                            float* __restrict__ pre_out, float* __restrict__ y,
+                                                            float* __restrict__ mean_out, float* __restrict__ rstd_out,
+                                                            int n_o = 1, long o_stride = 0, long ld_y = 0) {
+    const int r = blockIdx.x * 4 + (threadIdx.x >> 6);
+    if (r >= R) return;
+    layernorm_fwd_row(r, x, o, drop_p, seed, seed_dev, gamma, beta, eps, D, pre_out, y, mean_out, rstd_out, n_o, o_stride, ld_y);
+}
+constexpr int LN_MULTI_MAX = 4;
+struct LnFwdMultiP { const float* x[LN_MULTI_MAX]; const float* gamma[LN_MULTI_MAX]; const float* beta[LN_MULTI_MAX]; float* y[LN_MULTI_MAX];
+                     float* mean[LN_MULTI_MAX]; float* rstd[LN_MULTI_MAX]; int R[LN_MULTI_MAX]; int D[LN_MULTI_MAX]; };
+__global__ __launch_bounds__(256) void layernorm_fwd_multi_kernel(LnFwdMultiP t, float eps, long ld_y) {
+    const int w = blockIdx.y;
+    const int r = blockIdx.x * 4 + (threadIdx.x >> 6);
+    if (r >= t.R[w]) return;
+    layernorm_fwd_row(r, t.x[w], nullptr, 0.f, 0ull, nullptr, t.gamma[w], t.beta[w], eps, t.D[w], nullptr, t.y[w], t.mean[w], t.rstd[w], 1, 0, ld_y);
+}
+
+HULC_DEVICE void reduce_rows_wide_tail(const float* partial, int P, long ld, int accumulate, float* __restrict__ out, int R,
+                                      float* __restrict__ out1 = nullptr, int R1 = 0) {
+    const int per = (P + 15) / 16;
+    for (int c = threadIdx.x; c < R + R1; c += blockDim.x) {
+        const float* col = partial + c;
+        float t = 0.f, s = 0.f;
+        for (int q0 = 0; q0 < P; q0 += 16) {
+            float v[16];
+#pragma unroll
+            for (int i = 0; i < 16; ++i) v[i] = fin_load(col + (long)(q0 + i < P ? q0 + i : P - 1) * ld);
+#pragma unroll
+            for (int i = 0; i < 16; ++i) {
+                const int q = q0 + i;
+                if (q < P) {
+                    s += v[i];
+                    if ((q + 1) % per == 0 || q == P - 1) { t += s; s = 0.f; }
+                }
+            }
+        }
+        if (c < R) out[c] = accumulate ? out[c] + t : t;
+        else out1[c - R] = accumulate ? out1[c - R] + t : t;
+    }
+}
+
+HULC_DEVICE void layernorm_bwd_block(const float* __restrict__ dy, const float* __restrict__ pre, const float* __restrict__ mean_in,
+                                     const float* __restrict__ rstd_in, const float* __restrict__ gamma, int R, int D, int rows_per_block,
+                                     float* __restrict__ dpre, float* __restrict__ do_out, float drop_p, unsigned long long seed,
+                                     const unsigned long long* __restrict__ seed_dev, float* __restrict__ partial, long ld_dy,
+                                     unsigned* fin_ctr, float* __restrict__ dgamma, float* __restrict__ dbeta, int accumulate,
+                                     float (*red)[2][256], int* s_last) {
     if (seed_dev) seed ^= seed_dev[0];
     const int lane = threadIdx.x & 63, wave = threadIdx.x >> 6;
     float dg[4] = {0.f, 0.f, 0.f, 0.f}, db[4] = {0.f, 0.f, 0.f, 0.f};
@@ -320,9 +358,37 @@
     for (int c = threadIdx.x; c < D; c += 256) {
         float a = 0.f, b = 0.f;
         for (int w = 0; w < 4; ++w) { a += red[w][0][c]; b += red[w][1][c]; }
-        partial[(long)blockIdx.x * 2 * D + c] = a;
-        partial[(long)blockIdx.x * 2 * D + D + c] = b;
-    }
+        float* dst = partial + (long)blockIdx.x * 2 * D + c;
+        if (fin_ctr) { fin_store(dst, a); fin_store(dst + D, b); }
+        else { dst[0] = a; dst[D] = b; }
+    }
+    if (!fin_ctr || !fin_last_arriver(fin_ctr, gridDim.x, s_last)) return;
+    reduce_rows_wide_tail(partial, (int)gridDim.x, 2 * D, accumulate, dgamma, D, dbeta, D);
+}
+__global__ __launch_bounds__(256) void layernorm_bwd_kernel(const float* __restrict__ dy, const float* __restrict__ pre,
+                                                            const float* __restrict__ mean_in, const float* __restrict__ rstd_in,
+                                                            const float* __restrict__ gamma, int R, int D, int rows_per_block,
+                                                            float* __restrict__ dpre, float* __restrict__ do_out, float drop_p,
+                                                            unsigned long long seed, const unsigned long long* __restrict__ seed_dev,
+                                                            float* __restrict__ partial, long ld_dy = 0, unsigned* fin_ctr = nullptr,
+                                                            float* __restrict__ dgamma = nullptr, float* __restrict__ dbeta = nullptr,
+                                                            int accumulate = 0) {
+    __shared__ float red[4][2][256];
+    __shared__ int s_last;
+    layernorm_bwd_block(dy, pre, mean_in, rstd_in, gamma, R, D, rows_per_block, dpre, do_out, drop_p, seed, seed_dev, partial, ld_dy, fin_ctr, dgamma,
+                        dbeta, accumulate, red, &s_last);
+}
+struct LnBwdMultiP { const float* dy[LN_MULTI_MAX]; const float* pre[LN_MULTI_MAX]; const float* mean[LN_MULTI_MAX]; const float* rstd[LN_MULTI_MAX];
+                     const float* gamma[LN_MULTI_MAX]; float* dpre[LN_MULTI_MAX]; float* dgamma[LN_MULTI_MAX]; float* dbeta[LN_MULTI_MAX];
+                     int accumulate[LN_MULTI_MAX]; };
+__global__ __launch_bounds__(256) void layernorm_bwd_multi_kernel(LnBwdMultiP t, long ld_dy, int R, int D, int rows_per_block,
+                                                                  float* __restrict__ partial, unsigned* fin_ctr) {
+    __shared__ float red[4][2][256];
+    __shared__ int s_last;
+    const int w = blockIdx.y;
+    layernorm_bwd_block(t.dy[w], t.pre[w], t.mean[w], t.rstd[w], t.gamma[w], R, D, rows_per_block, t.dpre[w], nullptr, 0.f, 0ull, nullptr,
+                        partial + (long)w * gridDim.x * 2 * D, ld_dy, fin_ctr ? fin_ctr + w : nullptr, t.dgamma[w], t.dbeta[w], t.accumulate[w],
+                        red, &s_last);
 }
 
 __device__ inline float4 load4(const void* x, int dt, long off) {
@@ -331,8 +397,10 @@
     return make_float4(__uint_as_float(v.x << 16), __uint_as_float(v.x & 0xffff0000u), __uint_as_float(v.y << 16), __uint_as_float(v.y & 0xffff0000u));
 }
 __global__ __launch_bounds__(256) void colsum_kernel(const void* __restrict__ x, int x_dtype, long M, int N, long ld, long rows_per_block,
-                                                     float* __restrict__ partial, float* __restrict__ direct_out, int accumulate, int vec) {
+                                                     float* __restrict__ partial, float* __restrict__ direct_out, int accumulate, int vec,
+                                                     unsigned* fin_ctr = nullptr, float* __restrict__ fin_out = nullptr) {
     __shared__ float4 red[4][64];
+    __shared__ int s_last;
     const int lane = threadIdx.x & 63, wave = threadIdx.x >> 6;
     const int n = (blockIdx.x * 64 + lane) * 4;
     const long r0 = (long)blockIdx.y * rows_per_block;
@@ -368,9 +436,13 @@
         for (int j = 0; j < 4; ++j) {
             if (n + j >= N) break;
             if (direct_out) direct_out[n + j] = accumulate ? direct_out[n + j] + v[j] : v[j];
+            else if (fin_ctr) fin_store(partial + (long)blockIdx.y * N + n + j, v[j]);
             else partial[(long)blockIdx.y * N + n + j] = v[j];
         }
     }
+    if (!fin_ctr || !fin_last_arriver(fin_ctr + blockIdx.x, gridDim.y, &s_last)) return;
+    const int c0 = blockIdx.x * 256;
+    reduce_rows_wide_tail(partial + c0, (int)gridDim.y, N, accumulate, fin_out + c0, N - c0 < 256 ? N - c0 : 256);
 }
 __global__ __launch_bounds__(1024) void reduce_rows_wide_kernel(const float* __restrict__ partial, float* __restrict__ out, int P, long R, long ld,
                                                                 int accumulate, long off1 = 0, float* __restrict__ out1 = nullptr) {
@@ -690,8 +762,11 @@
     if (D > 256 || D <= 0) return hulc_fail(-2, "hulc_layernorm_bwd: D must be in 1..256");
     const int rpb = ln_bwd_rows_per_block(R), nb = (R + rpb - 1) / rpb;
     hipStream_t s = (hipStream_t)stream;
-    layernorm_bwd_kernel<<<nb, 256, 0, s>>>(dy, pre, mean, rstd, gamma, R, D, rpb, dpre, do_out, drop_p, seed, seed_dev, (float*)ws);
-    reduce_rows_wide_kernel<<<dim3((D + 63) / 64, 2), 1024, 0, s>>>((const float*)ws, dgamma, nb, D, 2 * D, accumulate_params, (long)D, dbeta);
+    unsigned* ctr = nullptr;
+    if (nb <= FIN_MAX_ARRIVALS && !(ctr = hulc_finish_counters(1, s, "hulc_layernorm_bwd"))) return -100;
+    layernorm_bwd_kernel<<<nb, 256, 0, s>>>(dy, pre, mean, rstd, gamma, R, D, rpb, dpre, do_out, drop_p, seed, seed_dev, (float*)ws, 0, ctr, dgamma,
+                                            dbeta, accumulate_params);
+    if (!ctr) reduce_rows_wide_kernel<<<dim3((D + 63) / 64, 2), 1024, 0, s>>>((const float*)ws, dgamma, nb, D, 2 * D, accumulate_params, (long)D, dbeta);
     return hulc_check_launch("hulc_layernorm_bwd");
 }
 
@@ -701,8 +776,11 @@
     if (D > 256 || D <= 0 || ld_dy < D) return hulc_fail(-2, "hulc_layernorm_bwd_ld: D must be in 1..256, ld_dy >= D");
     const int rpb = ln_bwd_rows_per_block(R), nb = (R + rpb - 1) / rpb;
     hipStream_t s = (hipStream_t)stream;
-    layernorm_bwd_kernel<<<nb, 256, 0, s>>>(dy, pre, mean, rstd, gamma, R, D, rpb, dpre, nullptr, 0.f, 0ull, nullptr, (float*)ws, ld_dy);
-    reduce_rows_wide_kernel<<<dim3((D + 63) / 64, 2), 1024, 0, s>>>((const float*)ws, dgamma, nb, D, 2 * D, accumulate_params, (long)D, dbeta);
+    unsigned* ctr = nullptr;
+    if (nb <= FIN_MAX_ARRIVALS && !(ctr = hulc_finish_counters(1, s, "hulc_layernorm_bwd_ld"))) return -100;
+    layernorm_bwd_kernel<<<nb, 256, 0, s>>>(dy, pre, mean, rstd, gamma, R, D, rpb, dpre, nullptr, 0.f, 0ull, nullptr, (float*)ws, ld_dy, ctr, dgamma,
+                                            dbeta, accumulate_params);
+    if (!ctr) reduce_rows_wide_kernel<<<dim3((D + 63) / 64, 2), 1024, 0, s>>>((const float*)ws, dgamma, nb, D, 2 * D, accumulate_params, (long)D, dbeta);
     return hulc_check_launch("hulc_layernorm_bwd_ld");
 }
 
@@ -797,6 +875,48 @@
     return hulc_check_launch("hulc_ln_partial_reduce_multi");
 }
 
+extern "C" int hulc_layernorm_fwd_ld_multi(int n, const float* const* x, const float* const* gamma, const float* const* beta, float eps, const int* R,
+                                           const int* D, float* const* y, long ld_y, float* const* mean, float* const* rstd, void* stream) {
+    if (!x || !gamma || !beta || !R || !D || !y || !mean || !rstd) return hulc_fail(-1, "hulc_layernorm_fwd_ld_multi: null pointer");
+    if (n < 1 || n > LN_MULTI_MAX) return hulc_fail(-2, "hulc_layernorm_fwd_ld_multi: 1..4 LayerNorms");
+    LnFwdMultiP t = {};
+    int rmax = 0;
+    for (int i = 0; i < n; ++i) {
+        if (!x[i] || !gamma[i] || !beta[i] || !y[i] || !mean[i] || !rstd[i]) return hulc_fail(-1, "hulc_layernorm_fwd_ld_multi: null pointer");
+        if (D[i] > 256 || D[i] <= 0 || ld_y < D[i] || R[i] < 1) return hulc_fail(-2, "hulc_layernorm_fwd_ld_multi: D must be in 1..256, ld_y >= D, R >= 1");
+        t.x[i] = x[i]; t.gamma[i] = gamma[i]; t.beta[i] = beta[i]; t.y[i] = y[i]; t.mean[i] = mean[i]; t.rstd[i] = rstd[i]; t.R[i] = R[i]; t.D[i] = D[i];
+        if (R[i] > rmax) rmax = R[i];
+    }
+    layernorm_fwd_multi_kernel<<<dim3((rmax + 3) / 4, n), 256, 0, (hipStream_t)stream>>>(t, eps, ld_y);
+    return hulc_check_launch("hulc_layernorm_fwd_ld_multi");
+}
+
+extern "C" long hulc_layernorm_bwd_ld_multi_workspace(int n, int R, int D) { return n * hulc_layernorm_bwd_workspace(R, D); }
+
+extern "C" int hulc_layernorm_bwd_ld_multi(int n, const float* const* dy, long ld_dy, const float* const* pre, const float* const* mean,
+                                           const float* const* rstd, const float* const* gamma, int R, int D, float* const* dpre,
+                                           float* const* dgamma, float* const* dbeta, const int* accumulate_params, void* ws, void* stream) {
+    if (!dy || !pre || !mean || !rstd || !gamma || !dpre || !dgamma || !dbeta || !accumulate_params || !ws)
+        return hulc_fail(-1, "hulc_layernorm_bwd_ld_multi: null pointer");
+    if (n < 1 || n > LN_MULTI_MAX) return hulc_fail(-2, "hulc_layernorm_bwd_ld_multi: 1..4 LayerNorms");
+    if (D > 256 || D <= 0 || ld_dy < D || R < 1) return hulc_fail(-2, "hulc_layernorm_bwd_ld_multi: D must be in 1..256, ld_dy >= D, R >= 1");
+    LnBwdMultiP t = {};
+    LnMultiP red = {};
+    for (int i = 0; i < n; ++i) {
+        if (!dy[i] || !pre[i] || !mean[i] || !rstd[i] || !gamma[i] || !dpre[i] || !dgamma[i] || !dbeta[i])
+            return hulc_fail(-1, "hulc_layernorm_bwd_ld_multi: null pointer");
+        t.dy[i] = dy[i]; t.pre[i] = pre[i]; t.mean[i] = mean[i]; t.rstd[i] = rstd[i]; t.gamma[i] = gamma[i]; t.dpre[i] = dpre[i];
+        t.dgamma[i] = red.dg[i] = dgamma[i]; t.dbeta[i] = red.db[i] = dbeta[i]; t.accumulate[i] = red.acc[i] = accumulate_params[i];
+    }
+    const int rpb = ln_bwd_rows_per_block(R), nb = (R + rpb - 1) / rpb;
+    hipStream_t s = (hipStream_t)stream;
+    unsigned* ctr = nullptr;
+    if (nb <= FIN_MAX_ARRIVALS && !(ctr = hulc_finish_counters(n, s, "hulc_layernorm_bwd_ld_multi"))) return -100;
+    layernorm_bwd_multi_kernel<<<dim3(nb, n), 256, 0, s>>>(t, ld_dy, R, D, rpb, (float*)ws, ctr);
+    if (!ctr) ln_partial_multi_kernel<<<dim3((D + 63) / 64, 2, n), 1024, 0, s>>>((const float*)ws, nb, D, red);
+    return hulc_check_launch("hulc_layernorm_bwd_ld_multi");
+}
+
 static long colsum_row_blocks(long M, int N) {
     const long gx = (N + 255) / 256;
     long rb = (1024 + gx - 1) / gx;
@@ -817,8 +937,10 @@
     const int vec = (N % 4 == 0) && (ld % 4 == 0) && (((uintptr_t)x) % (4 * esz) == 0);
     hipStream_t s = (hipStream_t)stream;
     dim3 grid((N + 255) / 256, (unsigned)rb);
-    colsum_kernel<<<grid, 256, 0, s>>>(x, x_dtype, M, N, ld, rpb, (float*)ws, rb == 1 ? out : nullptr, accumulate, vec);
-    if (rb > 1) reduce_rows_wide_kernel<<<(N + 63) / 64, 1024, 0, s>>>((const float*)ws, out, (int)rb, N, N, accumulate);
+    unsigned* ctr = nullptr;
+    if (rb > 1 && rb <= FIN_MAX_ARRIVALS && grid.x <= HULC_FINISH_MAX && !(ctr = hulc_finish_counters(grid.x, s, "hulc_colsum"))) return -100;
+    colsum_kernel<<<grid, 256, 0, s>>>(x, x_dtype, M, N, ld, rpb, (float*)ws, rb == 1 ? out : nullptr, accumulate, vec, ctr, out);
+    if (rb > 1 && !ctr) reduce_rows_wide_kernel<<<(N + 63) / 64, 1024, 0, s>>>((const float*)ws, out, (int)rb, N, N, accumulate);
     return hulc_check_launch("hulc_colsum");
 }
 
diff --git a/hulc2_amd/functional.py b/hulc2_amd/functional.py
--- a/hulc2_amd/functional.py
+++ b/hulc2_amd/functional.py
@@ -591,11 +591,15 @@
         y = _f32(R, D, like=xs[0])
         flat = y.view(-1)
         stats = []
-        for i, x in enumerate(xs):
-            r, d = x.shape
-            mean, rstd = _f32(r, like=x), _f32(r, like=x)
-            kn.layernorm_fwd_ld(x, params[2 * i], params[2 * i + 1], eps, r, d, flat[offs[i]:], ld, mean, rstd)
-            stats += [mean, rstd]
+        for x in xs:
+            stats += [_f32(x.shape[0], like=x), _f32(x.shape[0], like=x)]
+        if 1 < n <= 4:
+            kn.layernorm_fwd_ld_multi(xs, params[0::2], params[1::2], eps, [x.shape[0] for x in xs], [x.shape[1] for x in xs],
+                                      [flat[o:] for o in offs], ld, stats[0::2], stats[1::2])
+        else:
+            for i, x in enumerate(xs):
+                r, d = x.shape
+                kn.layernorm_fwd_ld(x, params[2 * i], params[2 * i + 1], eps, r, d, flat[offs[i]:], ld, stats[2 * i], stats[2 * i + 1])
         ctx.save_for_backward(*xs, *stats, *[params[2 * i] for i in range(n)])
         ctx.betas = [params[2 * i + 1] for i in range(n)]
         ctx.meta = (n, offs, ld, [tuple(a.shape) for a in args[:n]])
@@ -608,6 +612,16 @@
         xs, stats, gammas = sv[:n], sv[n:3 * n], sv[3 * n:]
         dyf = _c(dy).view(-1)
         dxs, dps = [], []
+        if 1 < n <= 4 and all(x.shape == xs[0].shape for x in xs):
+            r, d = xs[0].shape
+            dgs, dbs, accs = [], [], []
+            for i in range(n):
+                (dg, db), acc, rets = gradsink.joint((gammas[i], ctx.betas[i]), None, dyf)
+                dgs.append(dg); dbs.append(db); accs.append(acc)
+                dps += rets
+                dxs.append(_f32(r, d, like=dyf))
+            kn.layernorm_bwd_ld_multi([dyf[o:] for o in offs], ld, xs, stats[0::2], stats[1::2], gammas, r, d, dxs, dgs, dbs, accs)
+            return (None, None, None, *[dx.reshape(s) for dx, s in zip(dxs, shapes)], *dps)
         for i in range(n):
             x, gamma, beta = xs[i], gammas[i], ctx.betas[i]
             r, d = x.shape
@@ -649,15 +663,15 @@
         pp, pr, klg = ctx.saved_tensors
         B, G, CLS, beta, beta_dev, mix, nseg = ctx.meta
         dpp = dpr = None
-        if gkl is not None:
+        if gkl is not None and dplan is not None:
+            dpp, dpr = torch.empty_like(pp), torch.empty_like(pr)
+            kn.cat_kl_sample_bwd(pp, pr, klg, B, G, CLS, beta, mix, _c(gkl.reshape(nseg)), _c(dplan), dpp, dpr, nseg, beta_dev=beta_dev)
+        elif gkl is not None:
             dpp, dpr = torch.empty_like(pp), torch.empty_like(pr)
             kn.cat_kl_bwd(pp, pr, klg, B, G, CLS, beta, mix, _c(gkl.reshape(nseg)), dpp, dpr, nseg, beta_dev=beta_dev)
-        if dplan is not None:
-            if dpr is None:
-                dpr = torch.empty_like(pr)
-                kn.plan_sample_bwd(pr, _c(dplan), B * G, CLS, dpr)
-            else:
-                kn.plan_sample_bwd(pr, _c(dplan), B * G, CLS, dpr, accumulate=True)
+        elif dplan is not None:
+            dpr = torch.empty_like(pr)
+            kn.plan_sample_bwd(pr, _c(dplan), B * G, CLS, dpr)
         return dpp, dpr, None, None, None, None, None, None, None
 
 
diff --git a/hulc2_amd/kernels.py b/hulc2_amd/kernels.py
--- a/hulc2_amd/kernels.py
+++ b/hulc2_amd/kernels.py
@@ -1139,6 +1139,12 @@
           idx_out, plan)
 
 
+def cat_kl_sample_bwd(pp, pr, kl_group, B, G, CLS, beta, mix, gout, dplan, dpp, dpr, nseg=1, beta_dev=None):
+    if beta_dev is not None:
+        _beta_dev_ok("cat_kl_sample_bwd", beta_dev, _first_device(pp, pr, dpp))
+    _call("hulc_cat_kl_sample_bwd", pp, pr, kl_group, B, G, CLS, beta, mix, gout, nseg, dplan, dpp, dpr, beta_dev)
+
+
 def plan_sample_bwd(logits, dplan, NG, CLS, dlogits, accumulate=False):
     _call("hulc_plan_sample_bwd", logits, dplan, NG, CLS, dlogits, accumulate)
 
@@ -1213,6 +1219,24 @@
 def layernorm_bwd_ld(dy, ld_dy, pre, mean, rstd, gamma, R, D, dpre, dgamma, dbeta, accumulate_params=False):
     ws = _ws(_L.load().hulc_layernorm_bwd_workspace(R, D), dy.device)
     _call("hulc_layernorm_bwd_ld", dy, ld_dy, pre, mean, rstd, gamma, R, D, dpre, dgamma, dbeta, accumulate_params, ws)
+
+
+def _ptrs(ts):
+    _require_cuda(*ts)
+    return (_c.c_void_p * len(ts))(*[t.data_ptr() for t in ts])
+
+
+def layernorm_fwd_ld_multi(xs, gammas, betas, eps, Rs, Ds, ys, ld_y, means, rstds):
+    n = len(xs)
+    _call("hulc_layernorm_fwd_ld_multi", n, _ptrs(xs), _ptrs(gammas), _ptrs(betas), eps, (_c.c_int * n)(*Rs), (_c.c_int * n)(*Ds), _ptrs(ys), ld_y,
+          _ptrs(means), _ptrs(rstds))
+
+
+def layernorm_bwd_ld_multi(dys, ld_dy, pres, means, rstds, gammas, R, D, dpres, dgammas, dbetas, accumulates):
+    n = len(dys)
+    ws = _ws(_L.load().hulc_layernorm_bwd_ld_multi_workspace(n, R, D), dys[0].device)
+    _call("hulc_layernorm_bwd_ld_multi", n, _ptrs(dys), ld_dy, _ptrs(pres), _ptrs(means), _ptrs(rstds), _ptrs(gammas), R, D, _ptrs(dpres),
+          _ptrs(dgammas), _ptrs(dbetas), (_c.c_int * n)(*[int(bool(a)) for a in accumulates]), ws)
 
 
 def world_to_tcp(act, robot_obs, n, obs_dim, out):
diff --git a/include/hulc2_amd.h b/include/hulc2_amd.h
--- a/include/hulc2_amd.h
+++ b/include/hulc2_amd.h
@@ -74,6 +74,12 @@
                           float* rstd, void* stream);
 int hulc_layernorm_bwd_ld(const float* dy, long ld_dy, const float* pre, const float* mean, const float* rstd, const float* gamma, int R, int D,
                           float* dpre, float* dgamma, float* dbeta, int accumulate_params, void* ws, void* stream);
+int hulc_layernorm_fwd_ld_multi(int n, const float* const* x, const float* const* gamma, const float* const* beta, float eps, const int* R,
+                                const int* D, float* const* y, long ld_y, float* const* mean, float* const* rstd, void* stream);
+long hulc_layernorm_bwd_ld_multi_workspace(int n, int R, int D);
+int hulc_layernorm_bwd_ld_multi(int n, const float* const* dy, long ld_dy, const float* const* pre, const float* const* mean,
+                                const float* const* rstd, const float* const* gamma, int R, int D, float* const* dpre, float* const* dgamma,
+                                float* const* dbeta, const int* accumulate_params, void* ws, void* stream);
 long hulc_layernorm_bwd_workspace(int R, int D);
 int hulc_layernorm_bwd(const float* dy, const float* pre, const float* mean, const float* rstd, const float* gamma, int R, int D,
                        float* dpre, float* do_out, float drop_p, unsigned long long seed, const unsigned long long* seed_dev,
@@ -126,6 +132,8 @@
 int hulc_gauss_plan_bwd_sched(const float* pp, const float* pr, const float* eps_in, unsigned long long seed,
                               const unsigned long long* seed_dev, int B, int P, float min_std, float beta, float mix, int nseg,
                               const float* dplan, const float* gout, float* dpp, float* dpr, const float* beta_dev, void* stream);
+int hulc_cat_kl_sample_bwd(const float* pp, const float* pr, const float* kl_group, int B, int G, int CLS, float beta, float mix,
+                           const float* gout, int nseg, const float* dplan, float* dpp, float* dpr, const float* beta_dev, void* stream);
 int hulc_clip_loss_fwd(const float* im, const float* tx, const unsigned char* use, int row0, const float* logit_scale, int M, int D,
                        float* out, void* stream);
 int hulc_clip_loss_bwd(const float* im, const float* tx, const unsigned char* use, int row0, const float* logit_scale, int M, int D,
```

Result: no change. 20870 play-sequences/s (median of 6 runs) (+0.6%).
